# bioscan-ml/clibd

Hardware: AMD Instinct MI355X
Metric: paired samples/sec/step (I+D contrastive), global batch 2048 (higher is better)
Workload: dtype bf16

## Files before the change

clibd_amd/csrc/common.h:

```cpp
#pragma once
#include <hip/hip_runtime.h>
#include <stdint.h>

namespace clibd {

typedef __attribute__((ext_vector_type(8))) short bf16x8;
typedef __attribute__((ext_vector_type(4))) short bf16x4;
typedef __attribute__((ext_vector_type(4))) float f32x4;
typedef __attribute__((ext_vector_type(16))) float f32x16;
typedef __attribute__((address_space(3))) void lds_void;
typedef __attribute__((address_space(1))) const void gbl_cvoid;

__device__ __forceinline__ unsigned short f2bf(float x) {
    __bf16 h = (__bf16)x;
    return __builtin_bit_cast(unsigned short, h);
}
__device__ __forceinline__ float bf2f(unsigned short h) {
    return __builtin_bit_cast(float, ((unsigned)h) << 16);
}
__device__ __forceinline__ unsigned pack2bf(float lo, float hi) {
    typedef __bf16 bf16x2_t __attribute__((ext_vector_type(2)));
    typedef float f32x2_t __attribute__((ext_vector_type(2)));
    const bf16x2_t r = __builtin_convertvector((f32x2_t){lo, hi}, bf16x2_t);
    return __builtin_bit_cast(unsigned, r);
}
__device__ __forceinline__ float bfround(float x) { return bf2f(f2bf(x)); }

__device__ __forceinline__ unsigned pack4fp8(float a, float b, float c, float d) {
    a = __builtin_amdgcn_fmed3f(a, -448.f, 448.f); b = __builtin_amdgcn_fmed3f(b, -448.f, 448.f);
    c = __builtin_amdgcn_fmed3f(c, -448.f, 448.f); d = __builtin_amdgcn_fmed3f(d, -448.f, 448.f);
    int w = __builtin_amdgcn_cvt_pk_fp8_f32(a, b, 0, false);
    w = __builtin_amdgcn_cvt_pk_fp8_f32(c, d, w, true);
    return (unsigned)w;
}
__device__ __forceinline__ uint2 pack8fp8(const float v[8], float s) {
    uint2 o;
    o.x = pack4fp8(v[0] * s, v[1] * s, v[2] * s, v[3] * s);
    o.y = pack4fp8(v[4] * s, v[5] * s, v[6] * s, v[7] * s);
    return o;
}

__device__ __forceinline__ void glds16(const void* gsrc, void* lds_wave_base) {
    __builtin_amdgcn_global_load_lds((gbl_cvoid*)gsrc, (lds_void*)lds_wave_base, 16, 0, 0);
}

__device__ __forceinline__ void store16_stream(void* p, uint4 v) {
#ifdef CLIBD_NT_STORES
    typedef unsigned u32x4_t __attribute__((ext_vector_type(4)));
    __builtin_nontemporal_store((u32x4_t){v.x, v.y, v.z, v.w}, (u32x4_t*)p);
#else
    *(uint4*)p = v;
#endif
}

__device__ __forceinline__ unsigned drop_hash(unsigned seed, unsigned pair) {
    unsigned x = pair ^ seed;
    x ^= x >> 16; x *= 0x7feb352du; x ^= x >> 15; x *= 0x846ca68bu; x ^= x >> 16;
    return x;
}
__device__ __forceinline__ void drop_pair(unsigned seed, unsigned idx_even, unsigned thr16, float scale, float& f0, float& f1) {
    const unsigned h = drop_hash(seed, idx_even >> 1);
    f0 = (h & 0xffffu) >= thr16 ? scale : 0.f;
    f1 = (h >> 16) >= thr16 ? scale : 0.f;
}
__device__ __forceinline__ float drop_one(unsigned seed, unsigned idx, unsigned thr16, float scale) {
    const unsigned h = drop_hash(seed, idx >> 1);
    return (((idx & 1u) ? (h >> 16) : (h & 0xffffu)) >= thr16) ? scale : 0.f;
}

template <int CTRL>
__device__ __forceinline__ float dpp_mov(float v) {
    return __builtin_bit_cast(float, __builtin_amdgcn_update_dpp(0, __builtin_bit_cast(int, v), CTRL, 0xF, 0xF, false));
}
constexpr int DPP_QUAD_XOR1 = 0xB1, DPP_QUAD_XOR2 = 0x4E, DPP_ROW_HALF_MIRROR = 0x141, DPP_ROW_MIRROR = 0x140, DPP_ROW_ROR8 = 0x128;
__device__ __forceinline__ void permlane32_swap(float& a, float& b) {
    asm volatile("s_nop 1\n\tv_permlane32_swap_b32 %0, %1\n\ts_nop 1" : "+v"(a), "+v"(b));
}
__device__ __forceinline__ void permlane16_swap(float& a, float& b) {
    asm volatile("s_nop 1\n\tv_permlane16_swap_b32 %0, %1\n\ts_nop 1" : "+v"(a), "+v"(b));
}
__device__ __forceinline__ float rows4_sum(float v) {
    float a = v, b = v;
    permlane16_swap(a, b);
    v = a + b;
    a = v; b = v;
    permlane32_swap(a, b);
    return a + b;
}
__device__ __forceinline__ float rows4_max(float v) {
    float a = v, b = v;
    permlane16_swap(a, b);
    v = fmaxf(a, b);
    a = v; b = v;
    permlane32_swap(a, b);
    return fmaxf(a, b);
}
__device__ __forceinline__ float wave_sum(float v) {
    v += dpp_mov<DPP_QUAD_XOR1>(v);
    v += dpp_mov<DPP_QUAD_XOR2>(v);
    v += dpp_mov<DPP_ROW_HALF_MIRROR>(v);
    v += dpp_mov<DPP_ROW_MIRROR>(v);
    return rows4_sum(v);
}
__device__ __forceinline__ float wave_max(float v) {
    v = fmaxf(v, dpp_mov<DPP_QUAD_XOR1>(v));
    v = fmaxf(v, dpp_mov<DPP_QUAD_XOR2>(v));
    v = fmaxf(v, dpp_mov<DPP_ROW_HALF_MIRROR>(v));
    v = fmaxf(v, dpp_mov<DPP_ROW_MIRROR>(v));
    return rows4_max(v);
}

__device__ __forceinline__ float fast_erf(float x) {
    float ax = fabsf(x);
    float t = __builtin_amdgcn_rcpf(1.0f + 0.3275911f * ax);
    float y = ((((1.061405429f * t - 1.453152027f) * t + 1.421413741f) * t - 0.284496736f) * t + 0.254829592f) * t;
    float e = __expf(-ax * ax);
    float r = 1.0f - y * e;
    return copysignf(r, x);
}
__device__ __forceinline__ float gelu_f(float x) {
    return 0.5f * x * (1.0f + fast_erf(x * 0.70710678118654752f));
}
__device__ __forceinline__ void gelu_and_grad_f(float x, float& y, float& dy) {
    const float ax = fabsf(x) * 0.70710678118654752f;
    const float t = __builtin_amdgcn_rcpf(1.0f + 0.3275911f * ax);
    const float poly = ((((1.061405429f * t - 1.453152027f) * t + 1.421413741f) * t - 0.284496736f) * t + 0.254829592f) * t;
    const float e = __expf(-ax * ax);
    const float erfv = copysignf(1.0f - poly * e, x);
    const float cdf = 0.5f * (1.0f + erfv);
    y = x * cdf;
    dy = cdf + x * (0.3989422804014327f * e);
}
typedef float f32x2 __attribute__((ext_vector_type(2)));
__device__ __forceinline__ void gelu_and_grad_x2(f32x2 x, f32x2& y, f32x2& dy) {
    constexpr float K = 0.84932180028801907f;
    constexpr float P = 0.3275911f * 0.70710678118654752f / K;
    f32x2 ax = {fabsf(x[0]), fabsf(x[1])};
    ax = ax * K;
    const f32x2 d = ax * P + 1.0f;
    const f32x2 t = {__builtin_amdgcn_rcpf(d[0]), __builtin_amdgcn_rcpf(d[1])};
    const f32x2 poly = ((((0.5307027145f * t - 0.7265760135f) * t + 0.7107068705f) * t - 0.142248368f) * t + 0.127414796f) * t;
    const f32x2 s = ax * ax;
    const f32x2 e = {__builtin_amdgcn_exp2f(-s[0]), __builtin_amdgcn_exp2f(-s[1])};
    const f32x2 h = 0.5f - poly * e;
    const f32x2 hs = {copysignf(h[0], x[0]), copysignf(h[1], x[1])};
    const f32x2 cdf = hs + 0.5f;
    y = x * cdf;
    dy = (x * e) * 0.3989422804014327f + cdf;
}
__device__ __forceinline__ f32x2 bfround2(float a, float b) {
    const unsigned pk = pack2bf(a, b);
    return (f32x2){__builtin_bit_cast(float, pk << 16), __builtin_bit_cast(float, pk & 0xffff0000u)};
}
template <int N>
__device__ __forceinline__ void gelu_and_grad_rows(float* v, float* dg) {
#pragma unroll
    for (int e = 0; e < N; e += 2) {
        f32x2 y, d;
        gelu_and_grad_x2(bfround2(v[e], v[e + 1]), y, d);
        v[e] = y[0]; v[e + 1] = y[1];
        dg[e] = d[0]; dg[e + 1] = d[1];
    }
}
template <int N>
__device__ __forceinline__ void gelu_rows(float* v) {
#pragma unroll
    for (int e = 0; e < N; e += 2) {
        f32x2 y, d;
        gelu_and_grad_x2((f32x2){v[e], v[e + 1]}, y, d);
        v[e] = y[0]; v[e + 1] = y[1];
    }
}
constexpr float GELUQ_LO = -0.1328125f;
constexpr float GELUQ_STEP = 1.265625f / 255.0f;
constexpr float GELUQ_INV = 255.0f / 1.265625f;
__device__ __forceinline__ unsigned geluq_pack4(float a, float b, float c, float d) {
    unsigned w = 0;
    w = __builtin_amdgcn_cvt_pk_u8_f32(fmaf(a, GELUQ_INV, -GELUQ_LO * GELUQ_INV), 0, w);
    w = __builtin_amdgcn_cvt_pk_u8_f32(fmaf(b, GELUQ_INV, -GELUQ_LO * GELUQ_INV), 1, w);
    w = __builtin_amdgcn_cvt_pk_u8_f32(fmaf(c, GELUQ_INV, -GELUQ_LO * GELUQ_INV), 2, w);
    w = __builtin_amdgcn_cvt_pk_u8_f32(fmaf(d, GELUQ_INV, -GELUQ_LO * GELUQ_INV), 3, w);
    return w;
}
__device__ __forceinline__ void geluq_unpack4(unsigned w, float out[4]) {
    out[0] = fmaf((float)(w & 0xffu), GELUQ_STEP, GELUQ_LO);
    out[1] = fmaf((float)((w >> 8) & 0xffu), GELUQ_STEP, GELUQ_LO);
    out[2] = fmaf((float)((w >> 16) & 0xffu), GELUQ_STEP, GELUQ_LO);
    out[3] = fmaf((float)(w >> 24), GELUQ_STEP, GELUQ_LO);
}

__device__ __forceinline__ unsigned gelu12_code_bits(unsigned b) {
    const unsigned t = b & 0x7fffu;
    unsigned u = t >= (113u << 7) ? t - (112u << 7) : 0u;
    u = u > 0x7ffu ? 0x7ffu : u;
    return ((b >> 4) & 0x800u) | u;
}
__device__ __forceinline__ float gelu12_val(unsigned c) {
    const unsigned u = c & 0x7ffu;
    const unsigned t = u ? u + (112u << 7) : 0u;
    return __uint_as_float((((c & 0x800u) << 4) | t) << 16);
}
struct __attribute__((packed, aligned(4))) gelu12_row8 { unsigned w0, w1, w2; };
__device__ __forceinline__ gelu12_row8 gelu12_pack8(const float* g) {
    unsigned c[8];
#pragma unroll
    for (int e = 0; e < 8; e += 2) {
        const unsigned pk = pack2bf(g[e], g[e + 1]);
        c[e] = gelu12_code_bits(pk & 0xffffu);
        c[e + 1] = gelu12_code_bits(pk >> 16);
    }
    gelu12_row8 r;
    r.w0 = c[0] | (c[1] << 12) | (c[2] << 24);
    r.w1 = (c[2] >> 8) | (c[3] << 4) | (c[4] << 16) | (c[5] << 28);
    r.w2 = (c[5] >> 4) | (c[6] << 8) | (c[7] << 20);
    return r;
}
__device__ __forceinline__ void gelu12_unpack8(unsigned w0, unsigned w1, unsigned w2, float* g) {
    g[0] = gelu12_val(w0 & 0xfffu);
    g[1] = gelu12_val((w0 >> 12) & 0xfffu);
    g[2] = gelu12_val((w0 >> 24) | ((w1 & 0xfu) << 8));
// ... 15 lines not shown
```

clibd_amd/csrc/gemm.hip:

```cpp
#include <stdlib.h>

#include <cmath>

#include "gemm_common.h"
#include "host_util.h"

namespace clibd {

constexpr int BM = 128, BN = 128, BK = 64;
constexpr int TILE_BYTES = BM * BK * 2;
constexpr int GEMM_THREADS = 256;

__device__ __forceinline__ int w_row_perm(int r) {
    const int r6 = r & 63;
    return (r & 64) + w_col_of(r6 >> 4, r6 & 15);
}

__global__ __launch_bounds__(GEMM_THREADS, 2) void gemm_bf16_nt_kernel(GemmParams p) {
    extern __shared__ __attribute__((aligned(16))) char smem[];
    const int tid = threadIdx.x;
    const int lane = tid & 63;
    const int wave = __builtin_amdgcn_readfirstlane(tid >> 6);
    const int wm = wave >> 1, wn = wave & 1;

    const int ntiles = p.tiles_m * p.tiles_n;
    int bid = blockIdx.x;
    const int split = bid / ntiles;
    bid -= split * ntiles;
    int tile_m, tile_n;
    tile_coords(bid, p.tiles_m, p.tiles_n, 8, tile_m, tile_n);
    const int m0 = tile_m * BM, n0 = tile_n * BN;

    const int kt0 = split * p.ktiles_per_split;
    const int nk = min(p.ktiles_per_split, p.K / BK - p.hole_nkt - kt0);

    const int prow = lane >> 3;
    const int chunk = (lane & 7) ^ prow;
    const char* a_src[4];
    const char* w_src[4];
#pragma unroll
    for (int j = 0; j < 4; ++j) {
        const int r = (wave * 4 + j) * 8 + prow;
        const int gm = min(m0 + r, p.M - 1);
        const int gn = min(n0 + w_row_perm(r), p.N - 1);
        a_src[j] = (const char*)(p.A + (size_t)gm * p.lda) + chunk * 16;
        w_src[j] = (const char*)(p.W + (size_t)gn * p.ldw) + chunk * 16;
    }

    f32x4 acc[4][4];
#pragma unroll
    for (int i = 0; i < 4; ++i)
#pragma unroll
        for (int j = 0; j < 4; ++j) acc[i][j] = (f32x4){0.f, 0.f, 0.f, 0.f};

    const int frow = lane & 15, fch = lane >> 4;
    int a_off[4], w_off[4];
#pragma unroll
    for (int t = 0; t < 4; ++t) {
        const int ra = wm * 64 + t * 16 + frow;
        const int rw = wn * 64 + t * 16 + frow;
        a_off[t] = ra * 128 + ((fch ^ (ra & 7)) << 4);
        w_off[t] = rw * 128 + ((fch ^ (rw & 7)) << 4);
    }

    auto stage = [&](int kt, int buf) {
        char* base = smem + buf * (2 * TILE_BYTES);
        int kta = kt0 + kt;
        if (kta >= p.hole_kt) kta += p.hole_nkt;
        const size_t koff = (size_t)kta * (BK * 2);
#pragma unroll
        for (int j = 0; j < 4; ++j) {
            glds16(a_src[j] + koff, base + (wave * 4 + j) * 1024);
            glds16(w_src[j] + koff, base + TILE_BYTES + (wave * 4 + j) * 1024);
        }
    };

    if (nk > 0) stage(0, 0);
    for (int kt = 0; kt < nk; ++kt) {
        __syncthreads();
        if (kt + 1 < nk) stage(kt + 1, (kt + 1) & 1);
        const char* ab = smem + (kt & 1) * (2 * TILE_BYTES);
        const char* wb = ab + TILE_BYTES;
#pragma unroll
        for (int kk = 0; kk < 2; ++kk) {
            bf16x8 af[4], wf[4];
#pragma unroll
            for (int t = 0; t < 4; ++t) {
                af[t] = *(const bf16x8*)(ab + (a_off[t] ^ (kk << 6)));
                wf[t] = *(const bf16x8*)(wb + (w_off[t] ^ (kk << 6)));
            }
#pragma unroll
            for (int i = 0; i < 4; ++i)
#pragma unroll
                for (int j = 0; j < 4; ++j)
                    acc[i][j] = __builtin_amdgcn_mfma_f32_16x16x32_bf16(wf[j], af[i], acc[i][j], 0, 0, 0);
        }
    }

    const clibd_gemm_epilogue& ep = p.ep;
    if (ep.rank_u != nullptr && split == 0) {
        bf16x8 uf[4], vf[4];
#pragma unroll
        for (int t = 0; t < 4; ++t) {
            uf[t] = (bf16x8){0, 0, 0, 0, 0, 0, 0, 0};
            vf[t] = (bf16x8){0, 0, 0, 0, 0, 0, 0, 0};
            if (fch == 0) {
                const int gm = min(m0 + wm * 64 + t * 16 + frow, p.M - 1);
                const int gn = min(n0 + w_row_perm(wn * 64 + t * 16 + frow), p.N - 1);
                uf[t] = *(const bf16x8*)((const unsigned short*)ep.rank_u + (size_t)gm * ep.ld_rank_u);
                vf[t] = *(const bf16x8*)((const unsigned short*)ep.rank_v + (size_t)gn * 8);
            }
        }
#pragma unroll
        for (int i = 0; i < 4; ++i)
#pragma unroll
            for (int j = 0; j < 4; ++j)
                acc[i][j] = __builtin_amdgcn_mfma_f32_16x16x32_bf16(vf[j], uf[i], acc[i][j], 0, 0, 0);
    }

    const int nb = n0 + wn * 64 + 16 * fch;
    if (nb >= p.N) return;
    float bias[16];
    load_bias16(ep, nb, split == 0, bias);
#pragma unroll
    for (int i = 0; i < 4; ++i) {
        const int m = m0 + wm * 64 + 16 * i + frow;
        if (m >= p.M) continue;
        float v[16];
#pragma unroll
        for (int j = 0; j < 4; ++j)
#pragma unroll
            for (int r = 0; r < 4; ++r) v[4 * j + r] = acc[i][j][r] + bias[4 * j + r];
        store_row16(ep, m, nb, v);
    }
}

__global__ __launch_bounds__(256) void transpose_bf16_kernel(const unsigned short* in, int ld_in, int R, int C,
                                                             unsigned short* out, int ld_out) {
    __shared__ unsigned short tile[64][66];
    const int r0 = blockIdx.y * 64, c0 = blockIdx.x * 64;
    const int tx = threadIdx.x & 63, ty = threadIdx.x >> 6;
    for (int i = ty; i < 64; i += 4) {
        const int r = r0 + i, c = c0 + tx;
        tile[i][tx] = (r < R && c < C) ? in[(size_t)r * ld_in + c] : (unsigned short)0;
    }
    __syncthreads();
    for (int i = ty; i < 64; i += 4) {
        const int c = c0 + i, r = r0 + tx;
        if (c < C && r < ld_out) out[(size_t)c * ld_out + r] = tile[tx][i];
    }
}

__global__ __launch_bounds__(256) void transpose_fp8_bf16_kernel(const unsigned char* __restrict__ in, int ld_in, int R, int C, float scale,
                                                                 unsigned short* __restrict__ out, int ld_out) {
    __shared__ unsigned short tile[64][66];
    const int r0 = blockIdx.y * 64, c0 = blockIdx.x * 64;
    const int tx = threadIdx.x & 63, ty = threadIdx.x >> 6;
    for (int i = ty; i < 64; i += 4) {
        const int r = r0 + i, c = c0 + tx;
        unsigned short v = 0;
        if (r < R && c < C) v = f2bf(__builtin_amdgcn_cvt_f32_fp8((int)in[(size_t)r * ld_in + c], 0) * scale);
        tile[i][tx] = v;
    }
    __syncthreads();
    for (int i = ty; i < 64; i += 4) {
        const int c = c0 + i, r = r0 + tx;
        if (c < C && r < ld_out) out[(size_t)c * ld_out + r] = tile[tx][i];
    }
}

template <int RB>
__global__ __launch_bounds__(256) void transpose_colsum_bf16_kernel(const unsigned short* __restrict__ in, int ld_in, int R, int C,
                                                                    unsigned short* __restrict__ out, int ld_out,
                                                                    float* __restrict__ colsum, float* __restrict__ partials) {
    __shared__ __attribute__((aligned(16))) unsigned short tile[64 * RB * 66];
    const int r0 = blockIdx.y * (64 * RB), c0 = blockIdx.x * 64;
    const int t = threadIdx.x;
    uint4 v[2 * RB];
#pragma unroll
    for (int k = 0; k < 2 * RB; ++k) {
        const int row = (t >> 3) + 32 * k, ch = t & 7;
        v[k] = make_uint4(0u, 0u, 0u, 0u);
        if (r0 + row < R && c0 + 8 * ch < C) v[k] = *(const uint4*)(in + (size_t)(r0 + row) * ld_in + c0 + 8 * ch);
    }
#pragma unroll
    for (int k = 0; k < 2 * RB; ++k) {
        const int row = (t >> 3) + 32 * k, ch = t & 7;
        unsigned* d = (unsigned*)(tile + row * 66 + 8 * ch);
        d[0] = v[k].x; d[1] = v[k].y; d[2] = v[k].z; d[3] = v[k].w;
    }
    __syncthreads();
#pragma unroll
    for (int k = 0; k < 2; ++k) {
        const int c = (t >> 3) + 32 * k, rch = t & 7;
        float sum = 0.f;
#pragma unroll
        for (int rb = 0; rb < RB; ++rb) {
            unsigned short e[8];
#pragma unroll
            for (int j = 0; j < 8; ++j) e[j] = tile[(64 * rb + 8 * rch + j) * 66 + c];
            if (c0 + c < C && r0 + 64 * rb + 8 * rch < ld_out) {
                uint4 o;
                o.x = (unsigned)e[0] | ((unsigned)e[1] << 16); o.y = (unsigned)e[2] | ((unsigned)e[3] << 16);
                o.z = (unsigned)e[4] | ((unsigned)e[5] << 16); o.w = (unsigned)e[6] | ((unsigned)e[7] << 16);
                *(uint4*)(out + (size_t)(c0 + c) * ld_out + r0 + 64 * rb + 8 * rch) = o;
            }
            if (colsum != nullptr) {
#pragma unroll
                for (int j = 0; j < 8; ++j) sum += bf2f(e[j]);
            }
        }
        if (colsum != nullptr) {
            sum += dpp_mov<DPP_QUAD_XOR1>(sum);
            sum += dpp_mov<DPP_QUAD_XOR2>(sum);
            sum += dpp_mov<DPP_ROW_HALF_MIRROR>(sum);
            if (rch == 0 && c0 + c < C) {
                if (partials != nullptr) partials[(size_t)blockIdx.y * C + c0 + c] = sum;
                else atomicAdd(colsum + c0 + c, sum);
            }
        }
    }
}

__global__ __launch_bounds__(256) void colsum_partials_kernel(const float* __restrict__ partials, int nblk, int C, float* __restrict__ colsum) {
    const int c = blockIdx.x * 256 + threadIdx.x;
    if (c >= C) return;
    float s0 = 0.f, s1 = 0.f, s2 = 0.f, s3 = 0.f;
    int b = 0;
    for (; b + 3 < nblk; b += 4) {
        s0 += partials[(size_t)b * C + c];
        s1 += partials[(size_t)(b + 1) * C + c];
        s2 += partials[(size_t)(b + 2) * C + c];
        s3 += partials[(size_t)(b + 3) * C + c];
    }
    for (; b < nblk; ++b) s0 += partials[(size_t)b * C + c];
    colsum[c] += (s0 + s1) + (s2 + s3);
}

__global__ __launch_bounds__(1024) void ordered_colsum_kernel(const float* __restrict__ partials, int nblk, int C, float* __restrict__ out, int split,
                                                              float* __restrict__ out_b) {
    __shared__ float part[16][64];
    const int lane = threadIdx.x & 63, w = threadIdx.x >> 6, G = blockDim.x >> 6;
    const int c = blockIdx.x * 64 + lane;
    const int per = (nblk + G - 1) / G;
    const int b1 = min((w + 1) * per, nblk);
    float s = 0.f;
    if (c < C) {
        int b = w * per;
        for (; b + 8 <= b1; b += 8) {
            float v[8];
#pragma unroll
            for (int k = 0; k < 8; ++k) v[k] = partials[(size_t)(b + k) * C + c];
#pragma unroll
            for (int k = 0; k < 8; ++k) s += v[k];
        }
        for (; b < b1; ++b) s += partials[(size_t)b * C + c];
    }
    part[w][lane] = s;
    __syncthreads();
    if (w == 0 && c < C) {
        float t = part[0][lane];
        for (int k = 1; k < G; ++k) t += part[k][lane];
        if (c < split) out[c] += t;
        else out_b[c - split] += t;
    }
}

int ordered_colsum_launch(const float* partials, int nblk, int C, float* out, int split, float* out_b, hipStream_t stream) {
    if (nblk <= 0 || C <= 0) return CLIBD_OK;
    const int G = nblk < 16 ? nblk : 16;
    hipLaunchKernelGGL(ordered_colsum_kernel, dim3((unsigned)((C + 63) / 64)), dim3(64 * G), 0, stream, partials, nblk, C, out, split, out_b);
    return check_launch("ordered_colsum");
}

__global__ __launch_bounds__(256) void cast_f32_bf16_kernel(const float* in, unsigned short* out, size_t n) {
    size_t i = ((size_t)blockIdx.x * blockDim.x + threadIdx.x) * 4;
    const size_t stride = (size_t)gridDim.x * blockDim.x * 4;
    for (; i + 3 < n; i += stride) {
        const f32x4 v = *(const f32x4*)(in + i);
        uint2 o;
        o.x = pack2bf(v[0], v[1]);
        o.y = pack2bf(v[2], v[3]);
        *(uint2*)(out + i) = o;
    }
    if (blockIdx.x == 0 && threadIdx.x == 0)
        for (size_t j = n & ~(size_t)3; j < n; ++j) out[j] = f2bf(in[j]);
}

__global__ __launch_bounds__(256) void cast_transpose_f32_bf16_kernel(const float* in, int R, int C,
                                                                      unsigned short* out) {
    __shared__ float tile[64][65];
    const int r0 = blockIdx.y * 64, c0 = blockIdx.x * 64;
    const int tx = threadIdx.x & 63, ty = threadIdx.x >> 6;
    for (int i = ty; i < 64; i += 4) {
        const int r = r0 + i, c = c0 + tx;
        tile[i][tx] = (r < R && c < C) ? in[(size_t)r * C + c] : 0.f;
    }
    __syncthreads();
    for (int i = ty; i < 64; i += 4) {
        const int c = c0 + i, r = r0 + tx;
        if (c < C && r < R) out[(size_t)c * R + r] = f2bf(tile[tx][i]);
    }
}

}

using namespace clibd;

static int gemm_impl(const void* A, int lda, const void* W, int ldw, int M, int N, int K, int hole_k0, int hole_len,
                     const clibd_gemm_epilogue* ep, void* stream, void* tail_ws = nullptr, size_t tail_ws_bytes = 0) {
    if (!A || !W || !ep) return set_error(CLIBD_EINVAL, "gemm: null pointer");
    if (hole_len < 0 || hole_k0 < 0 || hole_k0 % BK || hole_len % BK || hole_k0 + hole_len > K || (hole_len > 0 && hole_len >= K))
        return set_error(CLIBD_EINVAL, "gemm: bad K hole (multiples of 64 inside [0, K))");
    if (M <= 0 || N <= 0 || K <= 0) return set_error(CLIBD_EINVAL, "gemm: non-positive shape");
    if (K % BK != 0) return set_error(CLIBD_EINVAL, "gemm: K must be a multiple of 64");
    if (N % 16 != 0) return set_error(CLIBD_EINVAL, "gemm: N must be a multiple of 16");
    if (lda % 8 != 0 || ldw % 8 != 0 || lda < K || ldw < K) return set_error(CLIBD_EINVAL, "gemm: bad lda/ldw");
    if (!aligned16(A) || !aligned16(W)) return set_error(CLIBD_EINVAL, "gemm: operands must be 16-byte aligned");
    if (!ep->out_bf16 && !ep->out_f32 && !ep->out_pre_bf16) return set_error(CLIBD_EINVAL, "gemm: no output");
    if ((ep->rank_u == nullptr) != (ep->rank_v == nullptr)) return set_error(CLIBD_EINVAL, "gemm: rank_u/rank_v");
    if (ep->rank_u && (ep->ld_rank_u < 8 || ep->ld_rank_u % 8)) return set_error(CLIBD_EINVAL, "gemm: ld_rank_u");
    if ((ep->act == CLIBD_ACT_GELU_GRAD || ep->act == CLIBD_ACT_MUL_AUX || ep->act == CLIBD_ACT_ADD_AUX) &&
        (!ep->aux_bf16 || ep->ld_aux % 8 || ep->ld_aux < N))
        return set_error(CLIBD_EINVAL, "gemm: GELU_GRAD / MUL_AUX / ADD_AUX need aux_bf16 with ld_aux >= N, % 8");
    if (ep->act == CLIBD_ACT_MUL_AUX_U8 && (!ep->aux_bf16 || ep->ld_aux % 16 || ep->ld_aux < N))
        return set_error(CLIBD_EINVAL, "gemm: MUL_AUX_U8 needs aux (one byte per element) with ld_aux >= N, % 16");
    const bool e12 = ep->act == CLIBD_ACT_GELU_SAVE_GRAD_E12 || ep->act == CLIBD_ACT_MUL_AUX_E12;
    if (e12 && (N % 8 != 0)) return set_error(CLIBD_EINVAL, "gemm: the e4m7 gelu' forms need N % 8 == 0");
    if (ep->act == CLIBD_ACT_MUL_AUX_E12 && (!ep->aux_bf16 || ep->ld_aux % 4 || ep->ld_aux < 3 * (N / 2)))
        return set_error(CLIBD_EINVAL, "gemm: MUL_AUX_E12 needs aux (1.5 bytes per element) with ld_aux >= 3N/2 bytes, % 4");
    if (ep->act == CLIBD_ACT_GELU_SAVE_GRAD_E12 && (!ep->out_pre_bf16 || ep->ld_pre % 4 || ep->ld_pre < 3 * (N / 2)))
        return set_error(CLIBD_EINVAL, "gemm: GELU_SAVE_GRAD_E12 needs out_pre (1.5 bytes per element) with ld_pre >= 3N/2 bytes, % 4");
    if ((ep->act == CLIBD_ACT_GELU_SAVE_GRAD || ep->act == CLIBD_ACT_GELU_SAVE_GRAD_U8) && !ep->out_pre_bf16)
        return set_error(CLIBD_EINVAL, "gemm: GELU_SAVE_GRAD needs out_pre_bf16");
    if (ep->act < 0 || ep->act > CLIBD_ACT_MUL_AUX_E12) return set_error(CLIBD_EINVAL, "gemm: bad act");
    if (ep->residual_f32 && (ep->ld_res % 4 || ep->ld_res < N)) return set_error(CLIBD_EINVAL, "gemm: ld_res");
    if (ep->out_pre_bf16 && (ep->ld_pre % (ep->act == CLIBD_ACT_GELU_SAVE_GRAD_U8 ? 16 : 8) || ep->ld_pre < N)) return set_error(CLIBD_EINVAL, "gemm: ld_pre");
    if (ep->out_bf16 && (ep->ld_out_bf16 % 8 || ep->ld_out_bf16 < N)) return set_error(CLIBD_EINVAL, "gemm: ld_out_bf16");
    if (ep->out_f32 && (ep->ld_out_f32 % 4 || ep->ld_out_f32 < N)) return set_error(CLIBD_EINVAL, "gemm: ld_out_f32");
    if (ep->drop_thr16 < 0 || ep->drop_thr16 > 65535 || (ep->drop_thr16 > 0 && (ep->drop_ld < N || (ep->drop_ld & 1) || ep->split_k > 1)))
        return set_error(CLIBD_EINVAL, "gemm: bad dropout parameters");
    const int split = ep->split_k < 1 ? 1 : ep->split_k;
    if (split > 1 && (ep->out_bf16 || ep->out_pre_bf16 || ep->act != CLIBD_ACT_NONE || ep->residual_f32 || !ep->out_f32))
        return set_error(CLIBD_EINVAL, "gemm: split_k > 1 supports only a plain fp32 accumulate output");
    const void* ptrs[] = {ep->bias, ep->rank_u, ep->rank_v, ep->aux_bf16, ep->residual_f32, ep->out_pre_bf16,
                          ep->out_bf16, ep->out_f32};
    for (const void* q : ptrs)
        if (q && !aligned16(q)) return set_error(CLIBD_EINVAL, "gemm: epilogue pointers must be 16-byte aligned");

    GemmParams p{};
    p.A = (const unsigned short*)A; p.W = (const unsigned short*)W;
    p.M = M; p.N = N; p.K = K; p.lda = lda; p.ldw = ldw;
    p.tiles_m = (M + BM - 1) / BM;
    p.tiles_n = (N + BN - 1) / BN;
    const int ktiles = (K - hole_len) / BK;
    p.ktiles_per_split = (ktiles + split - 1) / split;
    p.ep = *ep;
    p.ep.split_k = split;
    p.splits = 1; p.nk_split = 0; p.split_stride = 0;
    p.hole_kt = hole_len > 0 ? hole_k0 / BK : 0x7fffffff;
    p.hole_nkt = hole_len / BK;
    if (tail_ws != nullptr) {
        const size_t need = gemm256_tail_workspace_bytes(M, N, K);
        if (need > 0) {
            if (tail_ws_bytes < need || !aligned16(tail_ws)) return set_error(CLIBD_EINVAL, "gemm: tail workspace too small or misaligned (clibd_gemm_tail_workspace_bytes)");
            p.sk_flags = (unsigned*)tail_ws;
            p.sk_ws = (float*)((char*)tail_ws + 1024);
        }
    }
    static const int forced = [] { const char* e = getenv("CLIBD_GEMM_KERNEL"); return e ? atoi(e) : 0; }();
    const bool fold_epi = ep->row_sums != nullptr || ep->row_stats != nullptr;
    if (fold_epi) {
        if (epilogue_kind(p.ep) < 0)
            return set_error(CLIBD_EINVAL, "gemm: LN-fold epilogue: row_sums needs bias + residual_f32 + out_f32 + out_bf16 (act NONE); row_stats needs "
                                           "col_sum_w + bias + GELU_SAVE_GRAD with out_pre_bf16 + out_bf16; no rank update, dropout or split-K");
        if ((ep->row_sums && !aligned16(ep->row_sums)) || (ep->row_stats && !aligned16(ep->row_stats)) || (ep->col_sum_w && !aligned16(ep->col_sum_w)))
            return set_error(CLIBD_EINVAL, "gemm: LN-fold epilogue pointers must be 16-byte aligned");
        if (forced == 1 || hole_len != 0 || !gemm256_try_launch(p, (hipStream_t)stream))
            return set_error(CLIBD_EINVAL, "gemm: the LN-fold epilogues exist in the 256x256 kernel only (M >= 1024, N % 256 == 0, K % 128 == 0, >= 128 tiles)");
        return check_launch("gemm256_bf16_nt");
    }
    if (forced != 1 && hole_len == 0 && gemm256_try_launch(p, (hipStream_t)stream)) return check_launch("gemm256_bf16_nt");
    const long long nblocks = (long long)p.tiles_m * p.tiles_n * split;
    if (nblocks > 0x7fffffffLL) return set_error(CLIBD_EINVAL, "gemm: grid too large");
    static const bool attr_ok = [] {
        return hipFuncSetAttribute((const void*)gemm_bf16_nt_kernel, hipFuncAttributeMaxDynamicSharedMemorySize,
                                   4 * TILE_BYTES) == hipSuccess;
    }();
    (void)attr_ok;
    hipLaunchKernelGGL(gemm_bf16_nt_kernel, dim3((unsigned)nblocks), dim3(GEMM_THREADS), 4 * TILE_BYTES,
                       (hipStream_t)stream, p);
    return check_launch("gemm_bf16_nt");
}

extern "C" int clibd_gemm_bf16_nt(const void* A, int lda, const void* W, int ldw, int M, int N, int K,
                                  const clibd_gemm_epilogue* ep, void* stream) {
    return gemm_impl(A, lda, W, ldw, M, N, K, 0, 0, ep, stream);
}

extern "C" size_t clibd_gemm_tail_workspace_bytes(int M, int N, int K) { return gemm256_tail_workspace_bytes(M, N, K); }

extern "C" int clibd_gemm_bf16_nt_ws(const void* A, int lda, const void* W, int ldw, int M, int N, int K,
                                     const clibd_gemm_epilogue* ep, void* workspace, size_t workspace_bytes, void* stream) {
    return gemm_impl(A, lda, W, ldw, M, N, K, 0, 0, ep, stream, workspace, workspace_bytes);
}

extern "C" int clibd_gemm_bf16_nt_khole(const void* A, int lda, const void* W, int ldw, int M, int N, int K, int hole_k0, int hole_len,
                                        const clibd_gemm_epilogue* ep, void* stream) {
    return gemm_impl(A, lda, W, ldw, M, N, K, hole_k0, hole_len, ep, stream);
}

extern "C" int clibd_gemm_fp8_nt(const void* A, int lda, const void* W, int ldw, int M, int N, int K, const float* col_scale,
                                 float out_fp8_scale, const clibd_gemm_epilogue* ep, void* stream) {
    if (!A || !W || !ep || !col_scale) return set_error(CLIBD_EINVAL, "gemm_fp8: null pointer");
    if (M <= 0 || N <= 0 || K <= 0 || lda < K || ldw < K) return set_error(CLIBD_EINVAL, "gemm_fp8: bad shape");
    if ((lda & 15) || (ldw & 15) || !aligned16(A) || !aligned16(W) || !aligned16(col_scale)) return set_error(CLIBD_EINVAL, "gemm_fp8: alignment (lda, ldw % 16)");
    if (ep->ld_out_bf16 & 7 || ep->ld_out_f32 & 3 || ep->ld_res & 3 || ep->ld_pre & 7 || ep->ld_rank_u & 7)
        return set_error(CLIBD_EINVAL, "gemm_fp8: leading dimensions");
    if ((ep->out_bf16 && !aligned16(ep->out_bf16)) || (ep->out_f32 && !aligned16(ep->out_f32)) || (ep->out_pre_bf16 && !aligned16(ep->out_pre_bf16)) ||
        (ep->residual_f32 && !aligned16(ep->residual_f32)) || (ep->rank_u && !aligned16(ep->rank_u)) || (ep->rank_v && !aligned16(ep->rank_v)) ||
        (ep->bias && !aligned16(ep->bias)))
        return set_error(CLIBD_EINVAL, "gemm_fp8: pointer alignment");
    if ((ep->rank_u == nullptr) != (ep->rank_v == nullptr)) return set_error(CLIBD_EINVAL, "gemm_fp8: rank_u / rank_v must come together");
    GemmParams p{};
    p.A = (const unsigned short*)A; p.W = (const unsigned short*)W;
    p.M = M; p.N = N; p.K = K; p.lda = lda; p.ldw = ldw;
    p.ep = *ep;
    if (p.ep.split_k < 1) p.ep.split_k = 1;
    p.fp8 = 1; p.col_scale = col_scale; p.out_fp8_scale = out_fp8_scale;
    if (!gemm256_fp8_launch(p, (hipStream_t)stream))
        return set_error(CLIBD_EINVAL, "gemm_fp8: shape / epilogue not supported (N % 256, K % 256, K >= 512, bias required; forms: "
                                       "[lora] bias->bf16 | bias->gelu->fp8 + gelu' | bias[->dropout]+residual->f32)");
    return check_launch("gemm256_fp8_nt");
}

extern "C" int clibd_gemm_fp8_dgrad_nt(const void* A, int lda, const void* W, int ldw, int M, int N, int K, const float* col_scale,
                                       const float* a_row_dequant, float out_fp8_scale, const clibd_gemm_epilogue* ep, void* stream) {
    if (!A || !W || !ep || !col_scale) return set_error(CLIBD_EINVAL, "gemm_fp8_dgrad: null pointer");
    if (M <= 0 || N <= 0 || K <= 0 || lda < K || ldw < K) return set_error(CLIBD_EINVAL, "gemm_fp8_dgrad: bad shape");
    if ((lda & 15) || (ldw & 15) || !aligned16(A) || !aligned16(W) || !aligned16(col_scale) || (a_row_dequant && !aligned16(a_row_dequant)))
        return set_error(CLIBD_EINVAL, "gemm_fp8_dgrad: alignment (lda, ldw % 16)");
    if (ep->ld_out_bf16 & 7 || ep->ld_aux & 7) return set_error(CLIBD_EINVAL, "gemm_fp8_dgrad: leading dimensions");
    if (ep->act == CLIBD_ACT_MUL_AUX_U8 && (!ep->aux_bf16 || ep->ld_aux % 16 || ep->ld_aux < N))
        return set_error(CLIBD_EINVAL, "gemm_fp8_dgrad: MUL_AUX_U8 needs aux (one byte per element) with ld_aux >= N, % 16");
    if (!ep->out_bf16 || !aligned16(ep->out_bf16) || (ep->aux_bf16 && !aligned16(ep->aux_bf16))) return set_error(CLIBD_EINVAL, "gemm_fp8_dgrad: out_bf16 / aux alignment");
    if (ep->out_f32 || ep->residual_f32 || ep->bias || ep->rank_u || ep->rank_v || ep->row_sums || ep->row_stats || ep->col_sum_w)
        return set_error(CLIBD_EINVAL, "gemm_fp8_dgrad: only out_bf16 [+ aux_bf16] epilogues");
    const bool mul_form = ep->act == CLIBD_ACT_MUL_AUX || ep->act == CLIBD_ACT_MUL_AUX_U8 || ep->act == CLIBD_ACT_MUL_AUX_E12;
    if (ep->act == CLIBD_ACT_MUL_AUX_E12 && (!ep->aux_bf16 || ep->ld_aux % 4 || ep->ld_aux < 3 * (N / 2)))
        return set_error(CLIBD_EINVAL, "gemm_fp8_dgrad: MUL_AUX_E12 needs aux (1.5 bytes per element) with ld_aux >= 3N/2 bytes, % 4");
    if (ep->out_pre_bf16 && (!mul_form || !a_row_dequant || !aligned16(ep->out_pre_bf16) || (ep->ld_pre & 7) || ep->ld_pre < N))
        return set_error(CLIBD_EINVAL, "gemm_fp8_dgrad: out_pre_bf16 (bf16 copy) comes with MUL_AUX[_U8] and a_row_dequant only; ld_pre >= N, % 8; 16-byte aligned");
    GemmParams p{};
    p.A = (const unsigned short*)A; p.W = (const unsigned short*)W;
    p.M = M; p.N = N; p.K = K; p.lda = lda; p.ldw = ldw;
    p.ep = *ep;
    if (p.ep.split_k < 1) p.ep.split_k = 1;
    p.fp8 = 1; p.col_scale = col_scale; p.out_fp8_scale = out_fp8_scale; p.a_row_dequant = a_row_dequant;
    p.dual_bf16 = (unsigned short*)p.ep.out_pre_bf16; p.ld_dual = p.ep.ld_pre;
    p.ep.out_pre_bf16 = nullptr; p.ep.ld_pre = 0;
    if (!gemm256_fp8_dgrad_launch(p, (hipStream_t)stream))
        return set_error(CLIBD_EINVAL, "gemm_fp8_dgrad: shape / epilogue not supported (M % 4, N % 256, K % 256, K >= 512; forms: -> bf16 | + aux_bf16 -> bf16 "
                                       "(both need a_row_dequant) | x aux (bf16 gelu' or its one-byte code) -> fp8 (needs out_fp8_scale > 0))");
    return check_launch("gemm256_fp8_dgrad_nt");
}

namespace clibd {
__global__ __launch_bounds__(256) void reduce_splits_kernel(const float* __restrict__ partials, int splits, size_t n4,
                                                            float* __restrict__ out, int accumulate) {
    for (size_t i = (size_t)blockIdx.x * blockDim.x + threadIdx.x; i < n4; i += (size_t)gridDim.x * blockDim.x) {
        f32x4 s = accumulate ? ((const f32x4*)out)[i] : (f32x4){0.f, 0.f, 0.f, 0.f};
        for (int k = 0; k < splits; ++k) s += ((const f32x4*)partials)[(size_t)k * n4 + i];
        ((f32x4*)out)[i] = s;
    }
}
}

extern "C" size_t clibd_gemm_splitk_workspace_bytes(int M, int N) {
    if (M <= 0 || N <= 0) return 0;
    return (size_t)256 * (size_t)M * (size_t)N * sizeof(float) / (size_t)(((M + 255) / 256) * ((N + 255) / 256));
}

extern "C" int clibd_gemm_bf16_nt_splitk(const void* A, int lda, const void* W, int ldw, int M, int N, int K, float* out_f32, int ld_out,
                                         int accumulate, void* workspace, size_t workspace_bytes, void* stream) {
    if (!A || !W || !out_f32 || !workspace) return set_error(CLIBD_EINVAL, "gemm_splitk: null pointer");
    if (M <= 0 || N <= 0 || K <= 0 || lda < K || ldw < K || ld_out != N) return set_error(CLIBD_EINVAL, "gemm_splitk: bad shape (out must be dense [M,N])");
    if ((lda & 7) || (ldw & 7) || !aligned16(A) || !aligned16(W) || !aligned16(out_f32) || !aligned16(workspace) || (N & 3))
        return set_error(CLIBD_EINVAL, "gemm_splitk: alignment");
    GemmParams p{};
    p.A = (const unsigned short*)A; p.W = (const unsigned short*)W;
    p.M = M; p.N = N; p.K = K; p.lda = lda; p.ldw = ldw;
    const int splits = gemm256_splitk_launch(p, (float*)workspace, workspace_bytes / sizeof(float), (hipStream_t)stream);
    if (splits <= 0) return set_error(CLIBD_EINVAL, "gemm_splitk: shape not supported (need N % 256 == 0, K % 128 == 0, K >= 512, workspace)");
    if (int e = check_launch("gemm256_splitk")) return e;
    const size_t n4 = (size_t)M * N / 4;
    size_t blocks = (n4 + 255) / 256;
    if (blocks > 8192) blocks = 8192;
    hipLaunchKernelGGL(reduce_splits_kernel, dim3((unsigned)blocks), dim3(256), 0, (hipStream_t)stream, (const float*)workspace, splits, n4,
                       out_f32, accumulate);
    return check_launch("reduce_splits");
}

extern "C" int clibd_gemm_bf16_tn_splitk(const void* A, int lda, const void* B, int ldb, int M, int Na, int Nb, float* out_f32, int ld_out,
                                         int accumulate, float* colsum_a, void* workspace, size_t workspace_bytes, void* stream) {
    if (!A || !B || !out_f32 || !workspace) return set_error(CLIBD_EINVAL, "gemm_tn_splitk: null pointer");
    if (M <= 0 || Na <= 0 || Nb <= 0 || lda < Na || ldb < Nb || ld_out != Nb) return set_error(CLIBD_EINVAL, "gemm_tn_splitk: bad shape (out must be dense [Na,Nb])");
    if ((lda & 7) || (ldb & 7) || !aligned16(A) || !aligned16(B) || !aligned16(out_f32) || !aligned16(workspace))
        return set_error(CLIBD_EINVAL, "gemm_tn_splitk: alignment");
    const int splits = gemm256_tn_splitk_launch((const unsigned short*)A, lda, (const unsigned short*)B, ldb, M, Na, Nb, (float*)workspace,
                                                workspace_bytes / sizeof(float), colsum_a, (hipStream_t)stream);
    if (splits <= 0) return set_error(CLIBD_EINVAL, "gemm_tn_splitk: shape not supported (need M % 128 == 0, M >= 256, Na % 256 == 0, Nb % 256 == 0, workspace)");
    if (int e = check_launch("gemm256_tn")) return e;
    const size_t n4 = (size_t)Na * Nb / 4;
    size_t blocks = (n4 + 255) / 256;
    if (blocks > 8192) blocks = 8192;
    hipLaunchKernelGGL(reduce_splits_kernel, dim3((unsigned)blocks), dim3(256), 0, (hipStream_t)stream, (const float*)workspace, splits, n4,
                       out_f32, accumulate);
    return check_launch("reduce_splits");
}

extern "C" size_t clibd_gemm_tn_colsum_workspace_bytes(int M, int Na) {
    if (M <= 0 || Na <= 0) return 0;
    const int slots = M / 256 > 1 ? M / 256 : 1;
    return (size_t)slots * (size_t)Na * sizeof(float);
// ... 147 lines not shown
```

clibd_amd/csrc/gemm256.hip:

```cpp
#include <cstdlib>
#include "gemm_common.h"
#include "host_util.h"

namespace clibd {

constexpr int T_M = 256, T_N = 256, T_K = 64;
constexpr int HALF_BYTES = 128 * T_K * 2;
constexpr int STAGE_BYTES = 4 * HALF_BYTES;
constexpr int G256_THREADS = 512;
constexpr int G256_LDS = 2 * STAGE_BYTES;
constexpr size_t G256_SK_FLAG_BYTES = 1024;
#ifndef CLIBD_WS_MIN_TILES_N
#define CLIBD_WS_MIN_TILES_N 1
#endif
#ifndef CLIBD_WS_GROUP
#define CLIBD_WS_GROUP 6
#endif
constexpr int G256_WS_MIN_TILES_N = CLIBD_WS_MIN_TILES_N, G256_WS_GROUP = CLIBD_WS_GROUP;

#define CLIBD_WAIT_VMCNT(n) asm volatile("s_waitcnt vmcnt(" #n ")" ::: "memory")

typedef int i32x8 __attribute__((ext_vector_type(8)));
typedef int i32x4 __attribute__((ext_vector_type(4)));
__device__ __forceinline__ i32x8 cat_frag(bf16x8 lo, bf16x8 hi) {
// ... 198 lines not shown
    } while (0)
#define PHASE_HEAD(Q8)       \
    do {                                                                                                     \
        constexpr int st_ = ((Q8) >> 2) & 1;                                                                 \
        constexpr int dl_ = (Q8) & 3;                                                                        \
        if (dl_ == 0) { LOAD_W(w0F, st_, 1); LOAD_A(st_, 0); }                                               \
        else if (dl_ == 1) { LOAD_W(w1F, st_, 2); }                                                          \
        else if (dl_ == 2) { LOAD_A(st_, 3); }                                                               \
        if ((Q8) >= 2) {       \
            constexpr int ju_ = ((Q8) + 2) & 3;                                                              \
            constexpr int du_ = ((Q8) + 6) >> 2;                                                             \
            ISSUE(du_, ju_, du_ & 1);                                                                        \
        }                                                                                                    \
        WAIT_HEAD();                                                                                         \
        BARRIER();                                                                                           \
        if (dl_ == 0) { WAIT_FRAGS_W(w0F); WAIT_FRAGS_A(); }                                                 \
        else if (dl_ == 1) { WAIT_FRAGS_W(w1F); }                                                            \
        else if (dl_ == 2) { WAIT_FRAGS_A(); }                                                               \
        if (dl_ == 0) MMA(0, 0, w0F);                                                                        \
        else if (dl_ == 1) MMA(0, 1, w1F);                                                                   \
        else if (dl_ == 2) MMA(1, 1, w1F);                                                                   \
        else MMA(1, 0, w0F);                                                                                 \
        BARRIER();                                                                                           \
    } while (0)
#define PROLOGUE_ISSUE()                                                     \
    do {                                                                     \
         \
        ISSUE(0, 0, 0); __builtin_amdgcn_sched_barrier(0);                   \
        ISSUE(0, 1, 0); __builtin_amdgcn_sched_barrier(0);                   \
        ISSUE(0, 2, 0); __builtin_amdgcn_sched_barrier(0);                   \
        ISSUE(0, 3, 0); __builtin_amdgcn_sched_barrier(0);                   \
        ISSUE(1, 0, 1); __builtin_amdgcn_sched_barrier(0);                   \
        ISSUE(1, 1, 1); __builtin_amdgcn_sched_barrier(0);                   \
        ISSUE(1, 2, 1); __builtin_amdgcn_sched_barrier(0);                   \
        ISSUE(1, 3, 1); __builtin_amdgcn_sched_barrier(0);                   \
    } while (0)

    if (DIAG && skew_ticks > 0) {
        const int cls = (blockIdx.x >> 3) & 3;
        const unsigned long long t0 = __builtin_amdgcn_s_memrealtime();
        while ((long long)(__builtin_amdgcn_s_memrealtime() - t0) < (long long)cls * skew_ticks) __builtin_amdgcn_s_sleep(8);
    }
    set_sources(tile);
    PROLOGUE_ISSUE();
    int allow_case = 0;
    const clibd_gemm_epilogue& ep = p.ep;
    const int stores_case = (ep.out_pre_bf16 ? 1 : 0) + (ep.out_bf16 ? 1 : 0) + (ep.out_f32 ? 2 : 0) + (DG == 2 ? 1 : 0);

    int tile_i = 0;
#define STAMP(k)                                                                                         \
    do {                                                                                                 \
        if (DIAG && stamps != nullptr && tile_i < 16 && (wave == 0 || wave == 4) && lane == 0)                    \
            stamps[(((size_t)blockIdx.x * 16 + tile_i) * 2 + (wave >> 2)) * 8 + (k)] = (long long)__builtin_amdgcn_s_memtime(); \
    } while (0)

    while (true) {
        m0 = nm0;
        n0 = nn0;
        const int nk = nk_issue;
        const int split_cur = split_issue;
        const int part_cur = part_issue, slot_cur = slot_issue;
        const int next = tile + (int)gridDim.x;
        const bool has_next = next < ntiles;
        WAIT_HEAD();
        BARRIER();
        if (wm == 1) BARRIER();
        STAMP(0);
#pragma unroll
        for (int a = 0; a < 2; ++a)
#pragma unroll
            for (int b = 0; b < 4; ++b)
#pragma unroll
                for (int c = 0; c < 2; ++c)
#pragma unroll
                    for (int d = 0; d < 2; ++d) acc[a][b][c][d] = (f32x4){0.f, 0.f, 0.f, 0.f};

        int kt = 0;
        PHASE_HEAD(0); PHASE_HEAD(1); PHASE_HEAD(2); PHASE_HEAD(3);
        STAMP(1);
        PHASE_HEAD(4); PHASE_HEAD(5);
        PHASE(6, true, 8); PHASE(7, true, 8);
        STAMP(2);
        for (kt = 2; kt < nk - 2; kt += 2) {
            PHASE(0, true, 8); PHASE(1, true, 8); PHASE(2, true, 8); PHASE(3, true, 8);
            PHASE(4, true, 8); PHASE(5, true, 8); PHASE(6, true, 8); PHASE(7, true, 8);
        }
        STAMP(3);
        PHASE(0, true, 8); PHASE(1, true, 8);
        if (has_next) set_sources(next);
        PHASE_TAIL(2, 6); PHASE_TAIL(3, 4); PHASE_TAIL(4, 2); PHASE_TAIL(5, 0); PHASE_TAIL(6, 0); PHASE_TAIL(7, 0);
        if (wm == 0) BARRIER();
        if constexpr (FP8) {
#pragma unroll
            for (int hm = 0; hm < 2; ++hm)
                asm volatile("s_nop 15\n\ts_nop 15"
                             : "+v"(acc[hm][0][0][0]), "+v"(acc[hm][0][0][1]), "+v"(acc[hm][0][1][0]), "+v"(acc[hm][0][1][1]),
                               "+v"(acc[hm][1][0][0]), "+v"(acc[hm][1][0][1]), "+v"(acc[hm][1][1][0]), "+v"(acc[hm][1][1][1]),
                               "+v"(acc[hm][2][0][0]), "+v"(acc[hm][2][0][1]), "+v"(acc[hm][2][1][0]), "+v"(acc[hm][2][1][1]),
                               "+v"(acc[hm][3][0][0]), "+v"(acc[hm][3][0][1]), "+v"(acc[hm][3][1][0]), "+v"(acc[hm][3][1][1])
                             :: "memory");
        }
        STAMP(4);
        if constexpr (SK) {
            if (slot_cur >= 0) {
                const int srow = 64 * wn + 4 * fch, scol = 128 * wm + 8 * frow;
                if (part_cur > 0) {
                    float* outp = p.sk_ws + ((size_t)(part_cur - 1) * (size_t)p.sk_tail + (size_t)slot_cur) * (size_t)(T_M * T_N);
#pragma unroll
                    for (int hn = 0; hn < 2; ++hn)
#pragma unroll
                        for (int n = 0; n < 2; ++n)
#pragma unroll
                            for (int r = 0; r < 4; ++r) {
                                float* o = outp + (size_t)(srow + 32 * hn + 16 * n + r) * T_N + scol;
                                const f32x4 v0 = (f32x4){acc[0][0][hn][n][r], acc[0][1][hn][n][r], acc[0][2][hn][n][r], acc[0][3][hn][n][r]};
                                const f32x4 v1 = (f32x4){acc[1][0][hn][n][r], acc[1][1][hn][n][r], acc[1][2][hn][n][r], acc[1][3][hn][n][r]};
                                asm volatile("global_store_dwordx4 %0, %1, off sc0 sc1\n\tglobal_store_dwordx4 %0, %2, off offset:16 sc0 sc1" :: "v"(o), "v"(v0), "v"(v1) : "memory");
                            }
                    asm volatile("s_waitcnt vmcnt(0)" ::: "memory");
                    BARRIER();
                    if (tid == 0) __hip_atomic_fetch_add(p.sk_flags + slot_cur, 1u, __ATOMIC_RELAXED, __HIP_MEMORY_SCOPE_AGENT);
                    break;
                }
                if (tid == 0) {
                    while (__hip_atomic_load(p.sk_flags + slot_cur, __ATOMIC_RELAXED, __HIP_MEMORY_SCOPE_AGENT) < (unsigned)(p.sk_parts - 1)) __builtin_amdgcn_s_sleep(16);
                    __hip_atomic_store(p.sk_flags + slot_cur, 0u, __ATOMIC_RELAXED, __HIP_MEMORY_SCOPE_AGENT);
                }
                BARRIER();
                for (int q = 1; q < p.sk_parts; ++q) {
                    const float* inp = p.sk_ws + ((size_t)(q - 1) * (size_t)p.sk_tail + (size_t)slot_cur) * (size_t)(T_M * T_N);
#pragma unroll
                    for (int hn = 0; hn < 2; ++hn)
#pragma unroll
                        for (int n = 0; n < 2; ++n) {
                            f32x4 t0[4], t1[4];
#pragma unroll
                            for (int r = 0; r < 4; ++r) {
                                const float* o = inp + (size_t)(srow + 32 * hn + 16 * n + r) * T_N + scol;
                                asm volatile("global_load_dwordx4 %0, %2, off sc0 sc1\n\tglobal_load_dwordx4 %1, %2, off offset:16 sc0 sc1" : "=&v"(t0[r]), "=&v"(t1[r]) : "v"(o) : "memory");
                            }
                            asm volatile("s_waitcnt vmcnt(0)" : "+v"(t0[0]), "+v"(t0[1]), "+v"(t0[2]), "+v"(t0[3]), "+v"(t1[0]), "+v"(t1[1]), "+v"(t1[2]), "+v"(t1[3]));
#pragma unroll
                            for (int r = 0; r < 4; ++r)
#pragma unroll
                                for (int t = 0; t < 4; ++t) { acc[0][t][hn][n][r] += t0[r][t]; acc[1][t][hn][n][r] += t1[r][t]; }
                        }
                }
            }
        }
        int erow = frow, egrp = fch;
        asm volatile("" : "+v"(erow), "+v"(egrp));
        int nb = n0 + 128 * wm + 8 * erow;
        int mb = m0 + 64 * wn + 4 * egrp;
        constexpr bool RES_KIND = (KIND == EPI_RES_F32 || KIND == EPI_RES_F32_DROP || KIND == EPI_RES_F32_COPY);
        constexpr bool TWO_PASS = (epi_aux_kind(KIND) || RES_KIND || KIND == EPI_ROWNORM_GELU);
        constexpr bool PRELOAD_ROWS = TWO_PASS && !LORA && !FP8;
        f32x4 bias_q[2];
        uint4 in_aux[8];
        f32x4 in_res[8][2];
        float2 in_st[8];
        f32x4 col_s[2];
#define GLOAD128(dst, ptr) asm volatile("global_load_dwordx4 %0, %1, off ; EPI_OPERAND_LOAD" : "=&v"(dst) : "v"(ptr) : "memory")
        constexpr bool BIAS_ASM = BIAS && !FP8;
        if constexpr (BIAS_ASM) {
            const float* bp = ep.bias + nb;
            GLOAD128(bias_q[0], bp);
            GLOAD128(bias_q[1], bp + 4);
        }
        if constexpr (PRELOAD_ROWS) {
#pragma unroll
            for (int n = 0; n < 2; ++n)
#pragma unroll
                for (int r = 0; r < 4; ++r) {
                    const int mc = min(mb + 16 * n + r, p.M - 1);
                    if constexpr (KIND == EPI_ROWNORM_GELU) {
                        in_st[4 * n + r] = *(const float2*)(ep.row_stats + (size_t)mc * 2);
                    } else if constexpr (KIND == EPI_MUL_AUX_U8) {
                        const uint2 c8 = *(const uint2*)((const unsigned char*)ep.aux_bf16 + (size_t)mc * ep.ld_aux + nb);
                        in_aux[4 * n + r] = make_uint4(c8.x, c8.y, 0u, 0u);
                    } else if constexpr (KIND == EPI_MUL_AUX_12) {
                        in_aux[4 * n + r] = load_aux12((const unsigned char*)ep.aux_bf16 + (size_t)mc * ep.ld_aux + (nb >> 1) * 3);
                    } else if constexpr (epi_aux_kind(KIND)) {
                        in_aux[4 * n + r] = load_aux16<epi_aux_nt(KIND)>((const unsigned short*)ep.aux_bf16 + (size_t)mc * ep.ld_aux + nb);
                    } else {
                        const f32x4* rs = (const f32x4*)(ep.residual_f32 + (size_t)mc * ep.ld_res + nb);
                        in_res[4 * n + r][0] = rs[0];
                        in_res[4 * n + r][1] = rs[1];
                    }
                }
        }
        if constexpr (KIND == EPI_ROWNORM_GELU) {
            col_s[0] = *(const f32x4*)(ep.col_sum_w + nb);
            col_s[1] = *(const f32x4*)(ep.col_sum_w + nb + 4);
        }
        if (has_next) {
            ISSUE(1, 2, 1); __builtin_amdgcn_sched_barrier(0);
            ISSUE(1, 3, 1); __builtin_amdgcn_sched_barrier(0);
        }
        erow = frow; egrp = fch;
        asm volatile("" : "+v"(erow), "+v"(egrp));
        nb = n0 + 128 * wm + 8 * erow;
        mb = m0 + 64 * wn + 4 * egrp;
#define EPI_TIED_WAIT(N)                                                                                             \
    do {                                                                                                             \
        if constexpr (BIAS_ASM) asm volatile("s_waitcnt vmcnt(" #N ") ; EPI_OPERAND_WAIT" : "+v"(bias_q[0]), "+v"(bias_q[1])); \
    } while (0)
        if constexpr (KIND == EPI_ROWNORM_GELU) {
            if (!has_next) asm volatile("s_waitcnt vmcnt(10)" ::: "memory");
            EPI_TIED_WAIT(14);
        } else if constexpr (PRELOAD_ROWS && epi_aux_kind(KIND)) {
            if (!has_next) asm volatile("s_waitcnt vmcnt(8)" ::: "memory");
            EPI_TIED_WAIT(12);
        } else if constexpr (PRELOAD_ROWS) {
            if (!has_next) asm volatile("s_waitcnt vmcnt(16)" ::: "memory");
            EPI_TIED_WAIT(20);
        } else {
            if (!has_next) asm volatile("s_waitcnt vmcnt(0)" ::: "memory");
            EPI_TIED_WAIT(4);
        }
#undef EPI_TIED_WAIT
#undef GLOAD128
        unsigned rdexp[2][2];
        if constexpr (FP8) {
            const float* csp = p.col_scale + n0 + 128 * wm + 8 * erow;
            const f32x4 c0 = *(const f32x4*)csp, c1 = *(const f32x4*)(csp + 4);
#pragma unroll
            for (int hm = 0; hm < 2; ++hm)
#pragma unroll
                for (int t = 0; t < 4; ++t) {
                    const float c = hm ? c1[t] : c0[t];
#pragma unroll
                    for (int q = 0; q < 4; ++q) acc[hm][t][q >> 1][q & 1] *= c;
                }
            if constexpr (DG == 2) {
#pragma unroll
                for (int hn = 0; hn < 2; ++hn)
#pragma unroll
                    for (int n = 0; n < 2; ++n) {
                        const f32x4 rd = *(const f32x4*)(p.a_row_dequant + min(mb + 32 * hn + 16 * n, p.M - 4));
                        rdexp[hn][n] = ((__float_as_uint(rd[0]) >> 23) & 0xffu) | (((__float_as_uint(rd[1]) >> 23) & 0xffu) << 8) |
                                       (((__float_as_uint(rd[2]) >> 23) & 0xffu) << 16) | (((__float_as_uint(rd[3]) >> 23) & 0xffu) << 24);
                    }
            }
            if constexpr (DG && !epi_mul_aux_kind(KIND)) {
#pragma unroll
                for (int hn = 0; hn < 2; ++hn)
#pragma unroll
                    for (int n = 0; n < 2; ++n) {
                        const f32x4 rd = *(const f32x4*)(p.a_row_dequant + min(mb + 32 * hn + 16 * n, p.M - 4));
#pragma unroll
                        for (int hm = 0; hm < 2; ++hm)
#pragma unroll
                            for (int t = 0; t < 4; ++t) acc[hm][t][hn][n] *= rd;
                    }
            }
        }
        if (LORA) {
            bf16x8 uf[2][2];
#pragma unroll
            for (int hn = 0; hn < 2; ++hn)
#pragma unroll
                for (int n = 0; n < 2; ++n) {
                    uf[hn][n] = (bf16x8){0, 0, 0, 0, 0, 0, 0, 0};
                    if (egrp == 0) {
                        const int gm = min(m0 + 64 * wn + 32 * hn + 16 * n + erow, p.M - 1);
                        uf[hn][n] = *(const bf16x8*)((const unsigned short*)ep.rank_u + (size_t)gm * ep.ld_rank_u);
                    }
                }
#pragma unroll
            for (int hm = 0; hm < 2; ++hm)
#pragma unroll
                for (int t = 0; t < 4; ++t) {
                    bf16x8 vf = (bf16x8){0, 0, 0, 0, 0, 0, 0, 0};
                    if (egrp == 0) {
                        const int gn = nb + 4 * hm + t;
                        vf = *(const bf16x8*)((const unsigned short*)ep.rank_v + (size_t)gn * 8);
                    }
#pragma unroll
                    for (int n = 0; n < 4; ++n)
                        acc[hm][t][n >> 1][n & 1] = __builtin_amdgcn_mfma_f32_16x16x32_bf16(uf[n >> 1][n & 1], vf, acc[hm][t][n >> 1][n & 1], 0, 0, 0);
                }
            __builtin_amdgcn_sched_barrier(0);
        }

        {
            float bias[8];
            if constexpr (BIAS_ASM) {
#pragma unroll
                for (int e = 0; e < 4; ++e) { bias[e] = bias_q[0][e]; bias[4 + e] = bias_q[1][e]; }
            } else if constexpr (BIAS) {
                load_bias8(ep, nb, bias);
                if constexpr (!TWO_PASS) {
#pragma unroll
                    for (int e = 0; e < 8; ++e) asm volatile("" : "+v"(bias[e]));
                }
            }
#define EPV(hm, t) (BIAS ? acc[hm][t][hn][n][r] + bias[4 * (hm) + (t)] : acc[hm][t][hn][n][r])
#define FOR_ROWS_HN(HN0, HN1, ...)                                                                           \
    _Pragma("unroll") for (int hn = (HN0); hn < (HN1); ++hn)                                                 \
        _Pragma("unroll") for (int n = 0; n < 2; ++n)                                                        \
            _Pragma("unroll") for (int r = 0; r < 4; ++r) {                                                  \
                const int m = mb + 32 * hn + 16 * n + r;                                                     \
                __VA_ARGS__                                                                                  \
            }
#define FOR_ROWS(...) FOR_ROWS_HN(0, 2, __VA_ARGS__)
#define PIN_GROUP(hn_)                                                                                       \
    _Pragma("unroll") for (int hm = 0; hm < 2; ++hm)                                                         \
        _Pragma("unroll") for (int t = 0; t < 4; ++t)                                                        \
            _Pragma("unroll") for (int n2 = 0; n2 < 2; ++n2) asm volatile("" : "+v"(acc[hm][t][hn_][n2]))
            if (KIND == EPI_SPLITK_F32) {
                float* outp = ep.out_f32 + (size_t)split_cur * (size_t)p.split_stride;
                FOR_ROWS({
                    if (m < p.M) {
                        f32x4* o = (f32x4*)(outp + (size_t)m * ep.ld_out_f32 + nb);
                        o[0] = (f32x4){acc[0][0][hn][n][r], acc[0][1][hn][n][r], acc[0][2][hn][n][r], acc[0][3][hn][n][r]};
                        o[1] = (f32x4){acc[1][0][hn][n][r], acc[1][1][hn][n][r], acc[1][2][hn][n][r], acc[1][3][hn][n][r]};
                    }
                })
            } else if (TWO_PASS) {
                float cs8[8];
                if constexpr (KIND == EPI_ROWNORM_GELU) {
                    _Pragma("unroll") for (int e = 0; e < 4; ++e) { cs8[e] = col_s[0][e]; cs8[4 + e] = col_s[1][e]; }
                }
                FOR_ROWS_HN(0, 1, {
                    const int mc = min(m, p.M - 1);
                    float v[8];
                    _Pragma("unroll") for (int hm = 0; hm < 2; ++hm)
                        _Pragma("unroll") for (int t = 0; t < 4; ++t) v[4 * hm + t] = (KIND == EPI_ROWNORM_GELU) ? acc[hm][t][hn][n][r] : EPV(hm, t);
                    if constexpr (KIND == EPI_ROWNORM_GELU) fold_rownorm8(v, in_st[4 * n + r].x, in_st[4 * n + r].y, cs8, bias);
                    else if constexpr (PRELOAD_ROWS) fold_row8_in<KIND>(ep, mc, nb, v, in_aux[4 * n + r], in_res[4 * n + r][0], in_res[4 * n + r][1]);
                    else fold_row8<KIND>(ep, mc, nb, v);
                    _Pragma("unroll") for (int hm = 0; hm < 2; ++hm)
                        _Pragma("unroll") for (int t = 0; t < 4; ++t) acc[hm][t][hn][n][r] = v[4 * hm + t];
                })
                PIN_GROUP(0);
                FOR_ROWS_HN(1, 2, {
                    const int mc = min(m, p.M - 1);
                    float v[8];
                    _Pragma("unroll") for (int hm = 0; hm < 2; ++hm)
                        _Pragma("unroll") for (int t = 0; t < 4; ++t) v[4 * hm + t] = (KIND == EPI_ROWNORM_GELU) ? acc[hm][t][hn][n][r] : EPV(hm, t);
                    if constexpr (KIND == EPI_ROWNORM_GELU) {
                        const float2 st = *(const float2*)(ep.row_stats + (size_t)mc * 2);
                        fold_rownorm8(v, st.x, st.y, cs8, bias);
                    } else {
                        fold_row8<KIND>(ep, mc, nb, v);
                    }
                    _Pragma("unroll") for (int hm = 0; hm < 2; ++hm)
                        _Pragma("unroll") for (int t = 0; t < 4; ++t) acc[hm][t][hn][n][r] = v[4 * hm + t];
                })
                PIN_GROUP(1);
                float keep1 = 0.f, keep2 = 0.f;
                FOR_ROWS({
                    if (m < p.M) {
                        float v[8];
                        _Pragma("unroll") for (int hm = 0; hm < 2; ++hm)
                            _Pragma("unroll") for (int t = 0; t < 4; ++t) v[4 * hm + t] = acc[hm][t][hn][n][r];
                        if (KIND == EPI_ROWNORM_GELU) {
                            store_row8<EPI_GELU_SAVE>(ep, m, nb, v);
                        } else if (DG && epi_mul_aux_kind(KIND)) {
                            *(uint2*)((unsigned char*)ep.out_bf16 + (size_t)m * ep.ld_out_bf16 + nb) = pack8fp8(v, p.out_fp8_scale);
                            if constexpr (DG == 2) {
                                const float rdf = __uint_as_float(((rdexp[hn][n] >> (8 * r)) & 0xffu) << 23);
                                float w8[8];
                                _Pragma("unroll") for (int e = 0; e < 8; ++e) w8[e] = v[e] * rdf;
                                *(uint4*)(p.dual_bf16 + (size_t)m * p.ld_dual + nb) = pack8bf(w8);
                            }
                        } else if (epi_aux_kind(KIND)) {
                            *(uint4*)((unsigned short*)ep.out_bf16 + (size_t)m * ep.ld_out_bf16 + nb) = pack8bf(v);
                        } else {
                            f32x4* o = (f32x4*)(ep.out_f32 + (size_t)m * ep.ld_out_f32 + nb);
                            o[0] = (f32x4){v[0], v[1], v[2], v[3]};
                            o[1] = (f32x4){v[4], v[5], v[6], v[7]};
                            if constexpr (KIND == EPI_RES_F32_COPY) {
                                *(uint4*)((unsigned short*)ep.out_bf16 + (size_t)m * ep.ld_out_bf16 + nb) = pack8bf(v);
                                float s1 = ((v[0] + v[1]) + (v[2] + v[3])) + ((v[4] + v[5]) + (v[6] + v[7]));
                                float s2 = 0.f;
                                _Pragma("unroll") for (int e = 0; e < 8; ++e) s2 = fmaf(v[e], v[e], s2);
                                s1 = row16_sum(s1);
                                s2 = row16_sum(s2);
                                if (erow == 8 * hn + 4 * n + r) { keep1 = s1; keep2 = s2; }
                            }
                        }
                    }
                })
                if constexpr (KIND == EPI_RES_F32_COPY) {
                    const int jm = mb + 32 * (erow >> 3) + 16 * ((erow >> 2) & 1) + (erow & 3);
                    const int slice = (n0 >> 7) + wm;
                    if (jm < p.M) *(float2*)(ep.row_sums + ((size_t)slice * (size_t)p.M + (size_t)jm) * 2) = make_float2(keep1, keep2);
                }
            } else {
                FOR_ROWS({
                    if (m < p.M) {
                        float v[8];
                        _Pragma("unroll") for (int hm = 0; hm < 2; ++hm)
                            _Pragma("unroll") for (int t = 0; t < 4; ++t) v[4 * hm + t] = EPV(hm, t);
                        if (FP8 && KIND == EPI_GELU_SAVE) store_row8_gelu_fp8(ep, m, nb, v, p.out_fp8_scale);
                        else store_row8<KIND>(ep, m, nb, v);
                    }
                })
            }
#undef PIN_GROUP
#undef FOR_ROWS_HN
#undef FOR_ROWS
#undef EPV
        }
        STAMP(5);
        if (DIAG) ++tile_i;
        if (!has_next) break;
        allow_case = (m0 + T_M <= p.M) ? stores_case : 0;
        tile = next;
    }
}

template <int KIND, bool LORA, bool BIAS, bool DIAG, bool FP8>
__global__ __launch_bounds__(G256_THREADS) void gemm256_bf16_nt_kernel(GemmParams p, int ntiles, int skew_ticks, long long* stamps) {
    gemm256_body<KIND, LORA, BIAS, DIAG, FP8, 0>(p, ntiles, skew_ticks, stamps);
}
template <int KIND, bool LORA, bool BIAS>
__global__ __launch_bounds__(G256_THREADS) void gemm256_bf16_nt_sk_kernel(GemmParams p, int ntiles, int skew_ticks, long long* stamps) {
    gemm256_body<KIND, LORA, BIAS, false, false, 0, true>(p, ntiles, skew_ticks, stamps);
}
static const void* kernel_ptr_sk(int kind, bool lora, bool bias) {
    switch (kind) {
        case EPI_BF16: return bias ? nullptr : lora ? (const void*)gemm256_bf16_nt_sk_kernel<EPI_BF16, true, false> : (const void*)gemm256_bf16_nt_sk_kernel<EPI_BF16, false, false>;
        case EPI_ADD_AUX: return bias ? nullptr : lora ? (const void*)gemm256_bf16_nt_sk_kernel<EPI_ADD_AUX, true, false> : (const void*)gemm256_bf16_nt_sk_kernel<EPI_ADD_AUX, false, false>;
        case EPI_RES_F32: return (bias && !lora) ? (const void*)gemm256_bf16_nt_sk_kernel<EPI_RES_F32, false, true> : nullptr;
        case EPI_RES_F32_DROP: return (bias && !lora) ? (const void*)gemm256_bf16_nt_sk_kernel<EPI_RES_F32_DROP, false, true> : nullptr;
        default: return nullptr;
    }
}
template <int KIND, int DG = 1>
__global__ __launch_bounds__(G256_THREADS) void gemm256_fp8_dgrad_kernel(GemmParams p, int ntiles, int skew_ticks, long long* stamps) {
    gemm256_body<KIND, false, false, false, true, DG>(p, ntiles, skew_ticks, stamps);
}

#ifdef CLIBD_GEMM_DIAG
static long long* g_stamp_buffer = nullptr;
static int skew_env_value() {
    static const int v = [] { const char* e = getenv("CLIBD_GEMM_SKEW"); return e ? atoi(e) : 0; }();
    return v;
}
static int band_env_value() {
    static const int v = [] { const char* e = getenv("CLIBD_GEMM_BAND"); return e ? atoi(e) : 0; }();
    return v;
}
#define CLIBD_DIAG_KERNEL(KIND) (const void*)gemm256_bf16_nt_kernel<KIND, false, true, true, false>
#else
static constexpr long long* g_stamp_buffer = nullptr;
static int skew_env_value() { return 0; }
static int band_env_value() { return 0; }
#define CLIBD_DIAG_KERNEL(KIND) (const void*)nullptr
#endif

static const void* kernel_ptr(int kind, bool lora, bool bias, bool diag) {
#define K256(KIND)                                                                                                    \
    (diag ? CLIBD_DIAG_KERNEL(KIND)                                                                                   \
          : lora ? (bias ? (const void*)gemm256_bf16_nt_kernel<KIND, true, true, false, false>                        \
                         : (const void*)gemm256_bf16_nt_kernel<KIND, true, false, false, false>)                      \
                 : (bias ? (const void*)gemm256_bf16_nt_kernel<KIND, false, true, false, false>                       \
                         : (const void*)gemm256_bf16_nt_kernel<KIND, false, false, false, false>))
    switch (kind) {
        case EPI_BF16: return K256(EPI_BF16);
        case EPI_GELU_SAVE: return K256(EPI_GELU_SAVE);
        case EPI_GELU: return K256(EPI_GELU);
        case EPI_F32: return K256(EPI_F32);
        case EPI_MUL_AUX: return K256(EPI_MUL_AUX);
        case EPI_ADD_AUX: return K256(EPI_ADD_AUX);
        case EPI_GELU_SAVE_U8: return K256(EPI_GELU_SAVE_U8);
        case EPI_MUL_AUX_U8: return K256(EPI_MUL_AUX_U8);
        case EPI_GELU_SAVE_12: return K256(EPI_GELU_SAVE_12);
        case EPI_MUL_AUX_12: return K256(EPI_MUL_AUX_12);
        case EPI_RES_F32: return K256(EPI_RES_F32);
        case EPI_RES_F32_DROP: return K256(EPI_RES_F32_DROP);
        case EPI_SPLITK_F32: return (const void*)gemm256_bf16_nt_kernel<EPI_SPLITK_F32, false, false, false, false>;
        case EPI_RES_F32_COPY: return (lora || !bias || diag) ? nullptr : (const void*)gemm256_bf16_nt_kernel<EPI_RES_F32_COPY, false, true, false, false>;
        case EPI_ROWNORM_GELU: return (lora || !bias || diag) ? nullptr : (const void*)gemm256_bf16_nt_kernel<EPI_ROWNORM_GELU, false, true, false, false>;
        default: return K256(EPI_GENERIC);
    }
#undef K256
}

static const void* kernel_ptr_fp8(int kind, bool lora) {
    switch (kind) {
        case EPI_BF16: return lora ? (const void*)gemm256_bf16_nt_kernel<EPI_BF16, true, true, false, true>
                                   : (const void*)gemm256_bf16_nt_kernel<EPI_BF16, false, true, false, true>;
        case EPI_GELU_SAVE: return lora ? nullptr : (const void*)gemm256_bf16_nt_kernel<EPI_GELU_SAVE, false, true, false, true>;
        case EPI_RES_F32: return lora ? nullptr : (const void*)gemm256_bf16_nt_kernel<EPI_RES_F32, false, true, false, true>;
        case EPI_RES_F32_DROP: return lora ? nullptr : (const void*)gemm256_bf16_nt_kernel<EPI_RES_F32_DROP, false, true, false, true>;
        default: return nullptr;
    }
}

static int device_cus() {
    static const int num_cus = [] {
        int dev = 0, n = 256;
        if (hipGetDevice(&dev) == hipSuccess) {
            hipDeviceProp_t prop;
            if (hipGetDeviceProperties(&prop, dev) == hipSuccess && prop.multiProcessorCount > 0) n = prop.multiProcessorCount;
        }
        return n;
    }();
    return num_cus;
}

bool gemm256_fp8_launch(const GemmParams& p, hipStream_t stream) {
    const int nk = p.K / 128;
    if (!p.fp8 || p.col_scale == nullptr || p.K % 128 != 0 || nk < 4 || (nk & 1) || p.N % T_N != 0 || p.M < 1 || p.ep.split_k > 1) return false;
    if (p.ep.bias == nullptr) return false;
    if ((unsigned long long)p.M * p.lda >= (1ull << 32) || (unsigned long long)p.N * p.ldw >= (1ull << 32)) return false;
    const int kind = epilogue_kind(p.ep);
    const bool lora = p.ep.rank_u != nullptr;
    const void* fn = kernel_ptr_fp8(kind, lora);
    if (fn == nullptr) return false;
    if ((p.out_fp8_scale > 0.f) != (kind == EPI_GELU_SAVE)) return false;
    static const bool attr_ok = [] {
        bool ok = true;
        for (int k = 0; k < EPI_NUM_KINDS; ++k)
            for (int l = 0; l < 2; ++l) {
                const void* f = kernel_ptr_fp8(k, l != 0);
                if (f != nullptr) ok = ok && hipFuncSetAttribute(f, hipFuncAttributeMaxDynamicSharedMemorySize, G256_LDS) == hipSuccess;
            }
        return ok;
    }();
    if (!attr_ok) return false;
    GemmParams q = p;
    q.tiles_m = (p.M + T_M - 1) / T_M;
    q.tiles_n = p.N / T_N;
    q.splits = 1;
    q.nk_split = nk;
    q.split_stride = 0;
    q.band = q.tiles_n >= G256_WS_MIN_TILES_N ? -G256_WS_GROUP : 4;
    const long long tiles = (long long)q.tiles_m * q.tiles_n;
    const int grid = (int)(tiles < device_cus() ? tiles : device_cus());
    int ntiles_i = (int)tiles, skew = 0;
    long long* stamp = nullptr;
    void* args[] = {(void*)&q, (void*)&ntiles_i, (void*)&skew, (void*)&stamp};
    return hipLaunchKernel(fn, dim3((unsigned)grid), dim3(G256_THREADS), args, G256_LDS, stream) == hipSuccess;
}

bool gemm256_fp8_dgrad_launch(const GemmParams& p, hipStream_t stream) {
    const int nk = p.K / 128;
    if (!p.fp8 || p.col_scale == nullptr || p.K % 128 != 0 || nk < 4 || (nk & 1) || p.N % T_N != 0 || p.M < 4 || (p.M & 3) || p.ep.split_k > 1) return false;
    if (p.ep.bias != nullptr || p.ep.rank_u != nullptr || p.ep.drop_thr16 > 0) return false;
    if ((unsigned long long)p.M * p.lda >= (1ull << 32) || (unsigned long long)p.N * p.ldw >= (1ull << 32)) return false;
    const int kind = epilogue_kind(p.ep);
    const bool dual = p.dual_bf16 != nullptr;
    const void* fn = kind == EPI_BF16 ? (const void*)gemm256_fp8_dgrad_kernel<EPI_BF16>
                   : kind == EPI_MUL_AUX ? (dual ? (const void*)gemm256_fp8_dgrad_kernel<EPI_MUL_AUX, 2> : (const void*)gemm256_fp8_dgrad_kernel<EPI_MUL_AUX>)
                   : kind == EPI_MUL_AUX_U8 ? (dual ? (const void*)gemm256_fp8_dgrad_kernel<EPI_MUL_AUX_U8, 2> : (const void*)gemm256_fp8_dgrad_kernel<EPI_MUL_AUX_U8>)
                   : kind == EPI_MUL_AUX_12 ? (dual ? (const void*)gemm256_fp8_dgrad_kernel<EPI_MUL_AUX_12, 2> : (const void*)gemm256_fp8_dgrad_kernel<EPI_MUL_AUX_12>)
                   : kind == EPI_ADD_AUX ? (const void*)gemm256_fp8_dgrad_kernel<EPI_ADD_AUX> : nullptr;
    if (fn == nullptr) return false;
    const bool mul = epi_mul_aux_kind(kind);
    if ((p.out_fp8_scale > 0.f) != mul) return false;
    if ((!mul || dual) && p.a_row_dequant == nullptr) return false;
    if (dual && (!mul || (p.ld_dual & 7) || p.ld_dual < p.N || ((uintptr_t)p.dual_bf16 & 15))) return false;
    static const bool attr_ok = [] {
        bool ok = hipFuncSetAttribute((const void*)gemm256_fp8_dgrad_kernel<EPI_BF16>, hipFuncAttributeMaxDynamicSharedMemorySize, G256_LDS) == hipSuccess;
        ok = ok && hipFuncSetAttribute((const void*)gemm256_fp8_dgrad_kernel<EPI_MUL_AUX>, hipFuncAttributeMaxDynamicSharedMemorySize, G256_LDS) == hipSuccess;
        ok = ok && hipFuncSetAttribute((const void*)gemm256_fp8_dgrad_kernel<EPI_MUL_AUX_U8>, hipFuncAttributeMaxDynamicSharedMemorySize, G256_LDS) == hipSuccess;
        ok = ok && hipFuncSetAttribute((const void*)gemm256_fp8_dgrad_kernel<EPI_ADD_AUX>, hipFuncAttributeMaxDynamicSharedMemorySize, G256_LDS) == hipSuccess;
        ok = ok && hipFuncSetAttribute((const void*)gemm256_fp8_dgrad_kernel<EPI_MUL_AUX, 2>, hipFuncAttributeMaxDynamicSharedMemorySize, G256_LDS) == hipSuccess;
        ok = ok && hipFuncSetAttribute((const void*)gemm256_fp8_dgrad_kernel<EPI_MUL_AUX_U8, 2>, hipFuncAttributeMaxDynamicSharedMemorySize, G256_LDS) == hipSuccess;
        ok = ok && hipFuncSetAttribute((const void*)gemm256_fp8_dgrad_kernel<EPI_MUL_AUX_12>, hipFuncAttributeMaxDynamicSharedMemorySize, G256_LDS) == hipSuccess;
        ok = ok && hipFuncSetAttribute((const void*)gemm256_fp8_dgrad_kernel<EPI_MUL_AUX_12, 2>, hipFuncAttributeMaxDynamicSharedMemorySize, G256_LDS) == hipSuccess;
        return ok;
    }();
    if (!attr_ok) return false;
    GemmParams q = p;
    q.tiles_m = (p.M + T_M - 1) / T_M;
    q.tiles_n = p.N / T_N;
    q.splits = 1;
    q.nk_split = nk;
    q.split_stride = 0;
    q.band = q.tiles_n >= G256_WS_MIN_TILES_N ? -G256_WS_GROUP : 4;
    const long long tiles = (long long)q.tiles_m * q.tiles_n;
    const int grid = (int)(tiles < device_cus() ? tiles : device_cus());
    int ntiles_i = (int)tiles, skew = 0;
    long long* stamp = nullptr;
    void* args[] = {(void*)&q, (void*)&ntiles_i, (void*)&skew, (void*)&stamp};
    return hipLaunchKernel(fn, dim3((unsigned)grid), dim3(G256_THREADS), args, G256_LDS, stream) == hipSuccess;
}

bool gemm256_try_launch(const GemmParams& p, hipStream_t stream) {
    const int nk = p.K / T_K;
    if (p.K % T_K != 0 || nk < 4 || (nk & 1)) return false;
    if (p.N % T_N != 0) return false;
    if (p.ep.split_k > 1) return false;
    const long long tiles = (long long)((p.M + T_M - 1) / T_M) * (p.N / T_N);
    if (p.M < 1024 || tiles < 128) return false;
    if ((unsigned long long)p.M * p.lda * 2ull >= (1ull << 32) || (unsigned long long)p.N * p.ldw * 2ull >= (1ull << 32)) return false;
    static const bool attr_ok = [] {
        bool ok = true;
        for (int v = 0; v < 5; ++v)
            for (int k = 0; k < EPI_NUM_KINDS; ++k) {
                const void* fn = kernel_ptr(k, (v & 1) != 0, (v & 2) != 0, v == 4);
                if (fn != nullptr) ok = ok && hipFuncSetAttribute(fn, hipFuncAttributeMaxDynamicSharedMemorySize, G256_LDS) == hipSuccess;
            }
        return ok;
    }();
    if (!attr_ok) return false;
    static const int num_cus = [] {
        int dev = 0, n = 256;
        if (hipGetDevice(&dev) == hipSuccess) {
            hipDeviceProp_t prop;
            if (hipGetDeviceProperties(&prop, dev) == hipSuccess && prop.multiProcessorCount > 0) n = prop.multiProcessorCount;
        }
        return n;
    }();
    GemmParams q = p;
    q.tiles_m = (p.M + T_M - 1) / T_M;
    q.tiles_n = p.N / T_N;
    q.splits = 1;
    q.nk_split = nk;
    q.split_stride = 0;
    q.band = band_env_value() != 0 ? band_env_value() : (q.tiles_n >= G256_WS_MIN_TILES_N ? -G256_WS_GROUP : 4);
    int grid = (int)(tiles < num_cus ? tiles : num_cus);
#ifdef CLIBD_BALANCED_GRID
    if (tiles > num_cus) {
        const long long rounds = (tiles + num_cus - 1) / num_cus;
        grid = (int)((tiles + rounds - 1) / rounds);
    }
#endif
    const int kind = epilogue_kind(p.ep);
    int ntiles_i = (int)tiles;
    int skew_arg = skew_env_value();
    long long* stamp_arg = (p.ep.rank_u != nullptr) ? nullptr : g_stamp_buffer;
    const bool lora = p.ep.rank_u != nullptr;
    const bool diag = g_stamp_buffer != nullptr && !lora;
// ... 86 lines not shown
```

clibd_amd/csrc/gemm_common.h:

```cpp
#pragma once
#include "common.h"
#include "../../include/clibd_hip.h"

namespace clibd {

struct GemmParams {
    const unsigned short* A;
    const unsigned short* W;
    int M, N, K, lda, ldw;
    int tiles_m, tiles_n, ktiles_per_split;
    clibd_gemm_epilogue ep;
    int splits, nk_split;
    long long split_stride;
    int band;
    int hole_kt, hole_nkt;
    int fp8;
    const float* col_scale;
    float out_fp8_scale;
    const float* a_row_dequant;
    unsigned short* dual_bf16;
    int ld_dual;
    int sk_parts, sk_tail, sk_first, sk_nk_part;
    float* sk_ws;
    unsigned* sk_flags;
};

struct SkPlan { int parts, tail, first, nk_part; };
inline SkPlan plan_stream_k_tail(long long tiles, int num_cus, int nk) {
    SkPlan s{0, 0, 0, 0};
    if (tiles <= 0 || num_cus <= 0 || nk < 24 || (nk & 1)) return s;
    const long long full = (tiles / num_cus) * num_cus;
    const int tail = (int)(tiles - full);
    if (tail == 0 || 2 * tail > num_cus) return s;
    int P = num_cus / tail;
    if (P > 4) P = 4;
    for (; P >= 2; --P) {
        int nkp = (nk + P - 1) / P;
        nkp += nkp & 1;
        if (nkp < 4) nkp = 4;
        const int parts = (nk + nkp - 1) / nkp;
        const int last = nk - (parts - 1) * nkp;
        if (parts >= 2 && last >= 4 && (long long)parts * tail <= num_cus) { s.parts = parts; s.tail = tail; s.first = (int)full; s.nk_part = nkp; return s; }
    }
    return s;
}

__device__ __forceinline__ int w_col_of(int t, int i) { return 16 * (i >> 2) + 4 * t + (i & 3); }

__device__ __forceinline__ int tile_off(int row, int chunk) { return row * 128 + ((chunk ^ (row & 7)) << 4); }

__device__ __forceinline__ void tile_coords(int bid, int tiles_m, int tiles_n, int band, int& tile_m, int& tile_n) {
    const int ntiles = tiles_m * tiles_n;
    const int q = ntiles >> 3, r = ntiles & 7;
    const int xcd = bid & 7, idx = bid >> 3;
    bid = (xcd < r ? xcd * (q + 1) : r * (q + 1) + (xcd - r) * q) + idx;
    if (band < 0) {
        const int G = -band;
        const int g = bid / (tiles_m * G);
        const int rem = bid - g * tiles_m * G;
        const int gw = min(G, tiles_n - g * G);
        tile_m = rem / gw;
        tile_n = g * G + rem - tile_m * gw;
        return;
    }
    const int band_id = bid / (band * tiles_n);
    const int band_m0 = band_id * band;
    const int band_h = min(band, tiles_m - band_m0);
    const int in_band = bid - band_id * band * tiles_n;
    tile_m = band_m0 + in_band % band_h;
    tile_n = in_band / band_h;
}

__device__ __forceinline__ void load_bias16(const clibd_gemm_epilogue& ep, int nb, bool on, float bias[16]) {
#pragma unroll
    for (int e = 0; e < 16; ++e) bias[e] = 0.f;
    if (ep.bias != nullptr && on) {
#pragma unroll
        for (int q = 0; q < 4; ++q) {
            const f32x4 b4 = *(const f32x4*)(ep.bias + nb + 4 * q);
            bias[4 * q + 0] = b4[0]; bias[4 * q + 1] = b4[1]; bias[4 * q + 2] = b4[2]; bias[4 * q + 3] = b4[3];
        }
    }
}

__device__ __forceinline__ void store_row16(const clibd_gemm_epilogue& ep, int m, int nb, float v[16]) {
    if (ep.split_k > 1) {
        float* o = ep.out_f32 + (size_t)m * ep.ld_out_f32 + nb;
#pragma unroll
        for (int e = 0; e < 16; ++e) atomicAdd(o + e, v[e]);
        return;
    }
    if (ep.drop_thr16 > 0) {
        const unsigned base = (unsigned)m * (unsigned)ep.drop_ld + (unsigned)nb;
#pragma unroll
        for (int e = 0; e < 16; e += 2) {
            float f0, f1;
            drop_pair(ep.drop_seed, base + e, (unsigned)ep.drop_thr16, ep.drop_scale, f0, f1);
            v[e] *= f0;
            v[e + 1] *= f1;
        }
    }
    if (ep.act == CLIBD_ACT_GELU_SAVE_GRAD_E12) {
        float dg[16];
        gelu_and_grad_rows<16>(v, dg);
        gelu12_row8* o = (gelu12_row8*)((unsigned char*)ep.out_pre_bf16 + (size_t)m * ep.ld_pre + (nb >> 1) * 3);
        o[0] = gelu12_pack8(dg);
        o[1] = gelu12_pack8(dg + 8);
    } else if (ep.act == CLIBD_ACT_GELU_SAVE_GRAD_U8) {
        float dg[16];
        gelu_and_grad_rows<16>(v, dg);
        uint4 c;
        c.x = geluq_pack4(dg[0], dg[1], dg[2], dg[3]);   c.y = geluq_pack4(dg[4], dg[5], dg[6], dg[7]);
        c.z = geluq_pack4(dg[8], dg[9], dg[10], dg[11]); c.w = geluq_pack4(dg[12], dg[13], dg[14], dg[15]);
        store16_stream((unsigned char*)ep.out_pre_bf16 + (size_t)m * ep.ld_pre + nb, c);
    } else if (ep.act == CLIBD_ACT_GELU_SAVE_GRAD) {
        float dg[16];
        gelu_and_grad_rows<16>(v, dg);
        uint4 lo, hi;
        lo.x = pack2bf(dg[0], dg[1]);   lo.y = pack2bf(dg[2], dg[3]);   lo.z = pack2bf(dg[4], dg[5]);   lo.w = pack2bf(dg[6], dg[7]);
        hi.x = pack2bf(dg[8], dg[9]);   hi.y = pack2bf(dg[10], dg[11]); hi.z = pack2bf(dg[12], dg[13]); hi.w = pack2bf(dg[14], dg[15]);
        uint4* o = (uint4*)((unsigned short*)ep.out_pre_bf16 + (size_t)m * ep.ld_pre + nb);
        store16_stream(o, lo); store16_stream(o + 1, hi);
    } else if (ep.out_pre_bf16 != nullptr) {
        uint4 lo, hi;
        lo.x = pack2bf(v[0], v[1]);   lo.y = pack2bf(v[2], v[3]);   lo.z = pack2bf(v[4], v[5]);   lo.w = pack2bf(v[6], v[7]);
        hi.x = pack2bf(v[8], v[9]);   hi.y = pack2bf(v[10], v[11]); hi.z = pack2bf(v[12], v[13]); hi.w = pack2bf(v[14], v[15]);
        uint4* o = (uint4*)((unsigned short*)ep.out_pre_bf16 + (size_t)m * ep.ld_pre + nb);
        store16_stream(o, lo); store16_stream(o + 1, hi);
#pragma unroll
        for (int e = 0; e < 16; ++e) v[e] = bfround(v[e]);
    }
    if (ep.act == CLIBD_ACT_GELU) {
        gelu_rows<16>(v);
    } else if (ep.act == CLIBD_ACT_GELU_GRAD) {
        const uint4* ax = (const uint4*)((const unsigned short*)ep.aux_bf16 + (size_t)m * ep.ld_aux + nb);
        const uint4 x0 = ax[0], x1 = ax[1];
        const unsigned xs[8] = {x0.x, x0.y, x0.z, x0.w, x1.x, x1.y, x1.z, x1.w};
#pragma unroll
        for (int e = 0; e < 8; ++e) {
            v[2 * e] *= gelu_grad_f(bf2f((unsigned short)(xs[e] & 0xffffu)));
            v[2 * e + 1] *= gelu_grad_f(bf2f((unsigned short)(xs[e] >> 16)));
        }
    }
    if (ep.act == CLIBD_ACT_MUL_AUX_E12) {
        const gelu12_row8* ax = (const gelu12_row8*)((const unsigned char*)ep.aux_bf16 + (size_t)m * ep.ld_aux + (nb >> 1) * 3);
        const gelu12_row8 a0 = ax[0], a1 = ax[1];
        float d[16];
        gelu12_unpack8(a0.w0, a0.w1, a0.w2, d);
        gelu12_unpack8(a1.w0, a1.w1, a1.w2, d + 8);
#pragma unroll
        for (int e = 0; e < 16; ++e) v[e] *= d[e];
    }
    if (ep.act == CLIBD_ACT_MUL_AUX_U8) {
        const uint4 c = *(const uint4*)((const unsigned char*)ep.aux_bf16 + (size_t)m * ep.ld_aux + nb);
        const unsigned cs[4] = {c.x, c.y, c.z, c.w};
#pragma unroll
        for (int q = 0; q < 4; ++q) {
            float d[4];
            geluq_unpack4(cs[q], d);
            v[4 * q] *= d[0]; v[4 * q + 1] *= d[1]; v[4 * q + 2] *= d[2]; v[4 * q + 3] *= d[3];
        }
    }
    if (ep.act == CLIBD_ACT_MUL_AUX || ep.act == CLIBD_ACT_ADD_AUX) {
        const uint4* ax = (const uint4*)((const unsigned short*)ep.aux_bf16 + (size_t)m * ep.ld_aux + nb);
        const uint4 x0 = ax[0], x1 = ax[1];
        const unsigned xs[8] = {x0.x, x0.y, x0.z, x0.w, x1.x, x1.y, x1.z, x1.w};
#pragma unroll
        for (int e = 0; e < 8; ++e) {
            const float a0 = bf2f((unsigned short)(xs[e] & 0xffffu)), a1 = bf2f((unsigned short)(xs[e] >> 16));
            if (ep.act == CLIBD_ACT_MUL_AUX) { v[2 * e] *= a0; v[2 * e + 1] *= a1; }
            else { v[2 * e] += a0; v[2 * e + 1] += a1; }
        }
    }
    if (ep.residual_f32 != nullptr) {
        const f32x4* rs = (const f32x4*)(ep.residual_f32 + (size_t)m * ep.ld_res + nb);
#pragma unroll
        for (int q = 0; q < 4; ++q) {
            const f32x4 r4 = rs[q];
            v[4 * q + 0] += r4[0]; v[4 * q + 1] += r4[1]; v[4 * q + 2] += r4[2]; v[4 * q + 3] += r4[3];
        }
    }
    if (ep.out_f32 != nullptr) {
        f32x4* o = (f32x4*)(ep.out_f32 + (size_t)m * ep.ld_out_f32 + nb);
#pragma unroll
        for (int q = 0; q < 4; ++q) store16_stream(o + q, __builtin_bit_cast(uint4, (f32x4){v[4 * q], v[4 * q + 1], v[4 * q + 2], v[4 * q + 3]}));
    }
    if (ep.out_bf16 != nullptr) {
        uint4 lo, hi;
        lo.x = pack2bf(v[0], v[1]);   lo.y = pack2bf(v[2], v[3]);   lo.z = pack2bf(v[4], v[5]);   lo.w = pack2bf(v[6], v[7]);
        hi.x = pack2bf(v[8], v[9]);   hi.y = pack2bf(v[10], v[11]); hi.z = pack2bf(v[12], v[13]); hi.w = pack2bf(v[14], v[15]);
        uint4* o = (uint4*)((unsigned short*)ep.out_bf16 + (size_t)m * ep.ld_out_bf16 + nb);
        store16_stream(o, lo); store16_stream(o + 1, hi);
    }
}

__device__ __forceinline__ void load_bias8(const clibd_gemm_epilogue& ep, int nb, float bias[8]) {
#pragma unroll
    for (int e = 0; e < 8; ++e) bias[e] = 0.f;
    if (ep.bias != nullptr) {
        const f32x4 b0 = *(const f32x4*)(ep.bias + nb), b1 = *(const f32x4*)(ep.bias + nb + 4);
        bias[0] = b0[0]; bias[1] = b0[1]; bias[2] = b0[2]; bias[3] = b0[3];
        bias[4] = b1[0]; bias[5] = b1[1]; bias[6] = b1[2]; bias[7] = b1[3];
    }
}

__device__ __forceinline__ uint4 pack8bf(const float v[8]) {
    uint4 o;
    o.x = pack2bf(v[0], v[1]); o.y = pack2bf(v[2], v[3]); o.z = pack2bf(v[4], v[5]); o.w = pack2bf(v[6], v[7]);
    return o;
}

enum : int {
    EPI_GENERIC = 0,
    EPI_BF16 = 1,
    EPI_GELU_SAVE = 2,
    EPI_MUL_AUX = 3,
    EPI_RES_F32 = 4,
    EPI_RES_F32_DROP = 5,
    EPI_SPLITK_F32 = 6,
    EPI_ADD_AUX = 7,
    EPI_GELU_SAVE_U8 = 8,
    EPI_MUL_AUX_U8 = 9,
    EPI_RES_F32_COPY = 10,
    EPI_ROWNORM_GELU = 11,
    EPI_GELU_SAVE_12 = 12,
    EPI_MUL_AUX_12 = 13,
    EPI_GELU = 14,
    EPI_F32 = 15,
    EPI_NUM_KINDS = 16,
};
constexpr bool epi_aux_kind(int kind) { return kind == EPI_MUL_AUX || kind == EPI_ADD_AUX || kind == EPI_MUL_AUX_U8 || kind == EPI_MUL_AUX_12; }
constexpr bool epi_mul_aux_kind(int kind) { return kind == EPI_MUL_AUX || kind == EPI_MUL_AUX_U8 || kind == EPI_MUL_AUX_12; }

__host__ __device__ inline int epilogue_kind(const clibd_gemm_epilogue& ep) {
    if (ep.split_k > 1) return EPI_GENERIC;
    const bool drop = ep.drop_thr16 > 0;
    if (ep.row_sums != nullptr)
        return (ep.act == CLIBD_ACT_NONE && !drop && !ep.out_pre_bf16 && ep.residual_f32 && ep.out_f32 && ep.out_bf16 && !ep.rank_u && ep.bias) ? EPI_RES_F32_COPY : -1;
    if (ep.row_stats != nullptr)
        return (ep.act == CLIBD_ACT_GELU_SAVE_GRAD && !drop && ep.out_pre_bf16 && !ep.residual_f32 && !ep.out_f32 && ep.out_bf16 && !ep.rank_u && ep.bias && ep.col_sum_w) ? EPI_ROWNORM_GELU : -1;
    if (ep.act == CLIBD_ACT_NONE && !drop && !ep.out_pre_bf16 && !ep.residual_f32 && !ep.out_f32 && ep.out_bf16) return EPI_BF16;
    if (ep.act == CLIBD_ACT_GELU_SAVE_GRAD && !drop && ep.out_pre_bf16 && !ep.residual_f32 && !ep.out_f32 && ep.out_bf16) return EPI_GELU_SAVE;
    if (ep.act == CLIBD_ACT_GELU && !drop && !ep.out_pre_bf16 && !ep.residual_f32 && !ep.out_f32 && ep.out_bf16) return EPI_GELU;
    if (ep.act == CLIBD_ACT_MUL_AUX && !drop && !ep.out_pre_bf16 && !ep.residual_f32 && !ep.out_f32 && ep.out_bf16 && ep.aux_bf16) return EPI_MUL_AUX;
    if (ep.act == CLIBD_ACT_ADD_AUX && !drop && !ep.out_pre_bf16 && !ep.residual_f32 && !ep.out_f32 && ep.out_bf16 && ep.aux_bf16) return EPI_ADD_AUX;
    if (ep.act == CLIBD_ACT_GELU_SAVE_GRAD_U8 && !drop && ep.out_pre_bf16 && !ep.residual_f32 && !ep.out_f32 && ep.out_bf16) return EPI_GELU_SAVE_U8;
    if (ep.act == CLIBD_ACT_MUL_AUX_U8 && !drop && !ep.out_pre_bf16 && !ep.residual_f32 && !ep.out_f32 && ep.out_bf16 && ep.aux_bf16) return EPI_MUL_AUX_U8;
    if (ep.act == CLIBD_ACT_GELU_SAVE_GRAD_E12 && !drop && ep.out_pre_bf16 && !ep.residual_f32 && !ep.out_f32 && ep.out_bf16) return EPI_GELU_SAVE_12;
    if (ep.act == CLIBD_ACT_MUL_AUX_E12 && !drop && !ep.out_pre_bf16 && !ep.residual_f32 && !ep.out_f32 && ep.out_bf16 && ep.aux_bf16) return EPI_MUL_AUX_12;
    if (ep.act == CLIBD_ACT_GELU_SAVE_GRAD_E12 || ep.act == CLIBD_ACT_MUL_AUX_E12) return -1;
    if (ep.act == CLIBD_ACT_NONE && !ep.out_pre_bf16 && ep.residual_f32 && ep.out_f32 && !ep.out_bf16) return drop ? EPI_RES_F32_DROP : EPI_RES_F32;
    if (ep.act == CLIBD_ACT_NONE && !drop && !ep.out_pre_bf16 && !ep.residual_f32 && ep.out_f32 && !ep.out_bf16) return EPI_F32;
    return EPI_GENERIC;
}

template <int KIND>
__device__ __forceinline__ void store_row8(const clibd_gemm_epilogue& ep, int m, int nb, float v[8]) {
    if (KIND == EPI_BF16) {
        *(uint4*)((unsigned short*)ep.out_bf16 + (size_t)m * ep.ld_out_bf16 + nb) = pack8bf(v);
        return;
    }
    if (KIND == EPI_F32) {
        f32x4* o = (f32x4*)(ep.out_f32 + (size_t)m * ep.ld_out_f32 + nb);
        o[0] = (f32x4){v[0], v[1], v[2], v[3]};
        o[1] = (f32x4){v[4], v[5], v[6], v[7]};
        return;
    }
    if (KIND == EPI_GELU) {
        gelu_rows<8>(v);
        *(uint4*)((unsigned short*)ep.out_bf16 + (size_t)m * ep.ld_out_bf16 + nb) = pack8bf(v);
        return;
    }
    if (KIND == EPI_GELU_SAVE) {
        float dg[8];
        gelu_and_grad_rows<8>(v, dg);
        *(uint4*)((unsigned short*)ep.out_pre_bf16 + (size_t)m * ep.ld_pre + nb) = pack8bf(dg);
        *(uint4*)((unsigned short*)ep.out_bf16 + (size_t)m * ep.ld_out_bf16 + nb) = pack8bf(v);
        return;
    }
    if (KIND == EPI_GELU_SAVE_U8) {
        float dg[8];
        gelu_and_grad_rows<8>(v, dg);
        *(uint2*)((unsigned char*)ep.out_pre_bf16 + (size_t)m * ep.ld_pre + nb) =
            make_uint2(geluq_pack4(dg[0], dg[1], dg[2], dg[3]), geluq_pack4(dg[4], dg[5], dg[6], dg[7]));
        *(uint4*)((unsigned short*)ep.out_bf16 + (size_t)m * ep.ld_out_bf16 + nb) = pack8bf(v);
        return;
    }
    if (KIND == EPI_MUL_AUX_U8) {
        const uint2 c = *(const uint2*)((const unsigned char*)ep.aux_bf16 + (size_t)m * ep.ld_aux + nb);
        float d0[4], d1[4];
        geluq_unpack4(c.x, d0);
        geluq_unpack4(c.y, d1);
#pragma unroll
        for (int e = 0; e < 4; ++e) { v[e] *= d0[e]; v[4 + e] *= d1[e]; }
        *(uint4*)((unsigned short*)ep.out_bf16 + (size_t)m * ep.ld_out_bf16 + nb) = pack8bf(v);
        return;
    }
    if (KIND == EPI_GELU_SAVE_12) {
        float dg[8];
        gelu_and_grad_rows<8>(v, dg);
        *(gelu12_row8*)((unsigned char*)ep.out_pre_bf16 + (size_t)m * ep.ld_pre + (nb >> 1) * 3) = gelu12_pack8(dg);
        *(uint4*)((unsigned short*)ep.out_bf16 + (size_t)m * ep.ld_out_bf16 + nb) = pack8bf(v);
        return;
    }
    if (KIND == EPI_MUL_AUX_12) {
        const gelu12_row8 a = *(const gelu12_row8*)((const unsigned char*)ep.aux_bf16 + (size_t)m * ep.ld_aux + (nb >> 1) * 3);
        float d[8];
        gelu12_unpack8(a.w0, a.w1, a.w2, d);
#pragma unroll
        for (int e = 0; e < 8; ++e) v[e] *= d[e];
        *(uint4*)((unsigned short*)ep.out_bf16 + (size_t)m * ep.ld_out_bf16 + nb) = pack8bf(v);
        return;
    }
    if (KIND == EPI_MUL_AUX || KIND == EPI_ADD_AUX) {
        const uint4 x0 = *(const uint4*)((const unsigned short*)ep.aux_bf16 + (size_t)m * ep.ld_aux + nb);
        const unsigned xs[4] = {x0.x, x0.y, x0.z, x0.w};
#pragma unroll
        for (int e = 0; e < 4; ++e) {
            const float a0 = bf2f((unsigned short)(xs[e] & 0xffffu)), a1 = bf2f((unsigned short)(xs[e] >> 16));
            if (KIND == EPI_MUL_AUX) { v[2 * e] *= a0; v[2 * e + 1] *= a1; }
            else { v[2 * e] += a0; v[2 * e + 1] += a1; }
        }
        *(uint4*)((unsigned short*)ep.out_bf16 + (size_t)m * ep.ld_out_bf16 + nb) = pack8bf(v);
        return;
    }
    if (KIND == EPI_GENERIC || KIND == EPI_RES_F32_DROP) {
        if (KIND == EPI_RES_F32_DROP || ep.drop_thr16 > 0) {
            const unsigned base = (unsigned)m * (unsigned)ep.drop_ld + (unsigned)nb;
#pragma unroll
            for (int e = 0; e < 8; e += 2) {
                float f0, f1;
                drop_pair(ep.drop_seed, base + e, (unsigned)ep.drop_thr16, ep.drop_scale, f0, f1);
                v[e] *= f0;
                v[e + 1] *= f1;
            }
        }
    }
    if (KIND == EPI_GENERIC) {
        if (ep.act == CLIBD_ACT_GELU_SAVE_GRAD_U8) {
            float dg[8];
            gelu_and_grad_rows<8>(v, dg);
            *(uint2*)((unsigned char*)ep.out_pre_bf16 + (size_t)m * ep.ld_pre + nb) =
                make_uint2(geluq_pack4(dg[0], dg[1], dg[2], dg[3]), geluq_pack4(dg[4], dg[5], dg[6], dg[7]));
        } else if (ep.act == CLIBD_ACT_GELU_SAVE_GRAD) {
            float dg[8];
            gelu_and_grad_rows<8>(v, dg);
            *(uint4*)((unsigned short*)ep.out_pre_bf16 + (size_t)m * ep.ld_pre + nb) = pack8bf(dg);
        } else if (ep.out_pre_bf16 != nullptr) {
            *(uint4*)((unsigned short*)ep.out_pre_bf16 + (size_t)m * ep.ld_pre + nb) = pack8bf(v);
#pragma unroll
            for (int e = 0; e < 8; ++e) v[e] = bfround(v[e]);
        }
        if (ep.act == CLIBD_ACT_GELU) {
            gelu_rows<8>(v);
        } else if (ep.act == CLIBD_ACT_MUL_AUX_U8) {
            const uint2 c = *(const uint2*)((const unsigned char*)ep.aux_bf16 + (size_t)m * ep.ld_aux + nb);
            float d0[4], d1[4];
            geluq_unpack4(c.x, d0);
            geluq_unpack4(c.y, d1);
#pragma unroll
            for (int e = 0; e < 4; ++e) { v[e] *= d0[e]; v[4 + e] *= d1[e]; }
        } else if (ep.act == CLIBD_ACT_GELU_GRAD || ep.act == CLIBD_ACT_MUL_AUX || ep.act == CLIBD_ACT_ADD_AUX) {
            const uint4 x0 = *(const uint4*)((const unsigned short*)ep.aux_bf16 + (size_t)m * ep.ld_aux + nb);
            const unsigned xs[4] = {x0.x, x0.y, x0.z, x0.w};
#pragma unroll
            for (int e = 0; e < 4; ++e) {
                const float a0 = bf2f((unsigned short)(xs[e] & 0xffffu)), a1 = bf2f((unsigned short)(xs[e] >> 16));
                if (ep.act == CLIBD_ACT_GELU_GRAD) {
                    v[2 * e] *= gelu_grad_f(a0);
                    v[2 * e + 1] *= gelu_grad_f(a1);
                } else if (ep.act == CLIBD_ACT_MUL_AUX) {
                    v[2 * e] *= a0;
                    v[2 * e + 1] *= a1;
                } else {
                    v[2 * e] += a0;
                    v[2 * e + 1] += a1;
                }
            }
        }
    }
    if (KIND == EPI_RES_F32 || KIND == EPI_RES_F32_DROP || ep.residual_f32 != nullptr) {
        const f32x4* rs = (const f32x4*)(ep.residual_f32 + (size_t)m * ep.ld_res + nb);
        const f32x4 r0 = rs[0], r1 = rs[1];
        v[0] += r0[0]; v[1] += r0[1]; v[2] += r0[2]; v[3] += r0[3];
        v[4] += r1[0]; v[5] += r1[1]; v[6] += r1[2]; v[7] += r1[3];
    }
    if (KIND == EPI_RES_F32 || KIND == EPI_RES_F32_DROP || ep.out_f32 != nullptr) {
        f32x4* o = (f32x4*)(ep.out_f32 + (size_t)m * ep.ld_out_f32 + nb);
        o[0] = (f32x4){v[0], v[1], v[2], v[3]};
        o[1] = (f32x4){v[4], v[5], v[6], v[7]};
    }
    if (KIND == EPI_GENERIC && ep.out_bf16 != nullptr) *(uint4*)((unsigned short*)ep.out_bf16 + (size_t)m * ep.ld_out_bf16 + nb) = pack8bf(v);
}

__device__ __forceinline__ void store_row8_gelu_fp8(const clibd_gemm_epilogue& ep, int m, int nb, float v[8], float out_scale) {
    float dg[8];
    gelu_and_grad_rows<8>(v, dg);
    *(uint4*)((unsigned short*)ep.out_pre_bf16 + (size_t)m * ep.ld_pre + nb) = pack8bf(dg);
    *(uint2*)((unsigned char*)ep.out_bf16 + (size_t)m * ep.ld_out_bf16 + nb) = pack8fp8(v, out_scale);
}

template <int KIND>
__device__ __forceinline__ void fold_row8_in(const clibd_gemm_epilogue& ep, int m, int nb, float v[8], const uint4& ax, const f32x4& r0,
                                             const f32x4& r1) {
    if (KIND == EPI_MUL_AUX_U8) {
        float d0[4], d1[4];
        geluq_unpack4(ax.x, d0);
        geluq_unpack4(ax.y, d1);
#pragma unroll
        for (int e = 0; e < 4; ++e) { v[e] *= d0[e]; v[4 + e] *= d1[e]; }
    } else if (KIND == EPI_MUL_AUX_12) {
        float d[8];
        gelu12_unpack8(ax.x, ax.y, ax.z, d);
#pragma unroll
        for (int e = 0; e < 8; ++e) v[e] *= d[e];
    } else if (KIND == EPI_MUL_AUX || KIND == EPI_ADD_AUX) {
        const unsigned xs[4] = {ax.x, ax.y, ax.z, ax.w};
#pragma unroll
        for (int e = 0; e < 4; ++e) {
            const float a0 = bf2f((unsigned short)(xs[e] & 0xffffu)), a1 = bf2f((unsigned short)(xs[e] >> 16));
            if (KIND == EPI_MUL_AUX) { v[2 * e] *= a0; v[2 * e + 1] *= a1; }
            else { v[2 * e] += a0; v[2 * e + 1] += a1; }
        }
    } else {
        if (KIND == EPI_RES_F32_DROP) {
            const unsigned base = (unsigned)m * (unsigned)ep.drop_ld + (unsigned)nb;
#pragma unroll
            for (int e = 0; e < 8; e += 2) {
                float f0, f1;
                drop_pair(ep.drop_seed, base + e, (unsigned)ep.drop_thr16, ep.drop_scale, f0, f1);
                v[e] *= f0;
                v[e + 1] *= f1;
            }
        }
        v[0] += r0[0]; v[1] += r0[1]; v[2] += r0[2]; v[3] += r0[3];
        v[4] += r1[0]; v[5] += r1[1]; v[6] += r1[2]; v[7] += r1[3];
    }
}

__device__ __forceinline__ void fold_rownorm8(float v[8], float mean, float rstd, const float s[8], const float b[8]) {
#pragma unroll
    for (int e = 0; e < 8; ++e) v[e] = fmaf(rstd, fmaf(-mean, s[e], v[e]), b[e]);
}

__device__ __forceinline__ float row16_sum(float x) {
    x += dpp_mov<DPP_QUAD_XOR1>(x);
    x += dpp_mov<DPP_QUAD_XOR2>(x);
    x += dpp_mov<DPP_ROW_HALF_MIRROR>(x);
    x += dpp_mov<DPP_ROW_MIRROR>(x);
    return x;
}

template <bool NT>
__device__ __forceinline__ uint4 load_aux16(const void* p) {
    typedef unsigned aux_u32x4 __attribute__((ext_vector_type(4)));
#ifndef CLIBD_PLAIN_AUX_LOADS
    const aux_u32x4 v = NT ? __builtin_nontemporal_load((const aux_u32x4*)p) : *(const aux_u32x4*)p;
#else
    const aux_u32x4 v = *(const aux_u32x4*)p;
#endif
    return make_uint4(v[0], v[1], v[2], v[3]);
}
#ifndef CLIBD_NT_ADD_AUX
#define CLIBD_NT_ADD_AUX 0
#endif
constexpr bool epi_aux_nt(int kind) { return kind != EPI_ADD_AUX || CLIBD_NT_ADD_AUX; }

__device__ __forceinline__ uint4 load_aux12(const void* p) {
    typedef unsigned aux_u32x3 __attribute__((ext_vector_type(3), aligned(4)));
#ifndef CLIBD_PLAIN_AUX_LOADS
    const aux_u32x3 v = __builtin_nontemporal_load((const aux_u32x3*)p);
#else
    const aux_u32x3 v = *(const aux_u32x3*)p;
#endif
    return make_uint4(v[0], v[1], v[2], 0u);
}

template <int KIND>
__device__ __forceinline__ void fold_row8(const clibd_gemm_epilogue& ep, int m, int nb, float v[8]) {
    uint4 ax = make_uint4(0u, 0u, 0u, 0u);
    f32x4 r0 = (f32x4){0.f, 0.f, 0.f, 0.f}, r1 = r0;
    if (KIND == EPI_MUL_AUX_U8) {
        const uint2 c = *(const uint2*)((const unsigned char*)ep.aux_bf16 + (size_t)m * ep.ld_aux + nb);
        ax.x = c.x; ax.y = c.y;
    } else if (KIND == EPI_MUL_AUX_12) {
        ax = load_aux12((const unsigned char*)ep.aux_bf16 + (size_t)m * ep.ld_aux + (nb >> 1) * 3);
    } else if (KIND == EPI_MUL_AUX || KIND == EPI_ADD_AUX) {
        ax = load_aux16<epi_aux_nt(KIND)>((const unsigned short*)ep.aux_bf16 + (size_t)m * ep.ld_aux + nb);
    } else {
        const f32x4* rs = (const f32x4*)(ep.residual_f32 + (size_t)m * ep.ld_res + nb);
        r0 = rs[0];
        r1 = rs[1];
    }
    fold_row8_in<KIND>(ep, m, nb, v, ax, r0, r1);
}

inline int plan_k_slices(int nk, int tiles, int num_cus, int* nks_out) {
    int splits = num_cus / (tiles > 0 ? tiles : 1);
    if (splits < 1) splits = 1;
    if (splits > nk / 4) splits = nk / 4;
    if (splits < 1) splits = 1;
    int nks = (nk + splits - 1) / splits;
    nks += nks & 1;
    if (nks < 4) nks = 4;
    if (nks > nk) nks = nk;
    splits = (nk + nks - 1) / nks;
    while (nk - (splits - 1) * nks < 4 && nks < nk) {
        nks += 2;
        if (nks > nk) nks = nk;
        splits = (nk + nks - 1) / nks;
    }
    *nks_out = nks;
    return splits;
}

bool gemm256_try_launch(const GemmParams& p, hipStream_t stream);
size_t gemm256_tail_workspace_bytes(int M, int N, int K);
bool gemm256_fp8_launch(const GemmParams& p, hipStream_t stream);
bool gemm256_fp8_dgrad_launch(const GemmParams& p, hipStream_t stream);
int gemm256_splitk_launch(const GemmParams& p, float* partials, size_t partials_elems, hipStream_t stream);

int gemm256_tn_splitk_launch(const unsigned short* A, int lda, const unsigned short* B, int ldb, int M, int Na, int Nb, float* partials,
                             size_t partials_elems, float* colsum, hipStream_t stream, float* colsum_partials = nullptr);
int gemm256_tn_fp8b_splitk_launch(const unsigned short* A, int lda, const unsigned char* B8, int ldb, float b_scale, int M, int Na, int Nb,
                                  float* partials, size_t partials_elems, float* colsum, hipStream_t stream, float* colsum_partials = nullptr);

}
```

clibd_amd/csrc/layernorm.hip:

```cpp
#include "common.h"
#include "../../include/clibd_hip.h"
#include "host_util.h"

namespace clibd {

constexpr int LN_MAX_CHUNKS = 4;

__device__ __forceinline__ float wave_reduce8(float v[8], int lane) {
    float w4[4], w2[2];
#pragma unroll
    for (int i = 0; i < 4; ++i) {
        float a = v[i], b = v[i + 4];
        permlane32_swap(a, b);
        w4[i] = a + b;
    }
#pragma unroll
    for (int i = 0; i < 2; ++i) {
        float a = w4[i], b = w4[i + 2];
        permlane16_swap(a, b);
        w2[i] = a + b;
    }
    const bool b3 = lane & 8;
    const float keep = b3 ? w2[1] : w2[0];
    const float send = b3 ? w2[0] : w2[1];
    float w1 = keep + dpp_mov<DPP_ROW_ROR8>(send);
    w1 += dpp_mov<DPP_ROW_HALF_MIRROR>(w1);
    w1 += dpp_mov<DPP_QUAD_XOR1>(w1);
    w1 += dpp_mov<DPP_QUAD_XOR2>(w1);
    return w1;
}

template <int NCH, bool LORA, int ROWS>
__global__ __launch_bounds__(256) void layernorm_fwd_kernel(const float* __restrict__ x, int M, int H,
                                                            const float* __restrict__ gamma,
                                                            const float* __restrict__ beta, float eps,
                                                            unsigned short* __restrict__ y_bf16,
                                                            float* __restrict__ y_f32, float* __restrict__ stats,
                                                            const unsigned short* __restrict__ lora_a,
                                                            unsigned short* __restrict__ t_bf16, unsigned drop_seed,
                                                            int drop_thr16, float drop_scale,
                                                            unsigned char* __restrict__ y_fp8, float fp8_scale) {
    extern __shared__ __attribute__((aligned(16))) float a_lds[];
    const int lane = threadIdx.x & 63;
    const int wave_in_grid = blockIdx.x * 4 + (threadIdx.x >> 6);
    const int nwaves = gridDim.x * 4;
    if (LORA) {
        for (int i = threadIdx.x; i < 8 * H; i += 256) a_lds[i] = bf2f(lora_a[i]);
        __syncthreads();
    }
    f32x4 g[NCH], b[NCH];
    bool act[NCH];
#pragma unroll
    for (int j = 0; j < NCH; ++j) {
        const int c = 4 * (lane + 64 * j);
        act[j] = c < H;
        g[j] = act[j] ? *(const f32x4*)(gamma + c) : (f32x4){0, 0, 0, 0};
        b[j] = act[j] ? *(const f32x4*)(beta + c) : (f32x4){0, 0, 0, 0};
    }
    const float invH = 1.0f / (float)H;
    for (int row0 = wave_in_grid * ROWS; row0 < M; row0 += nwaves * ROWS) {
        f32x4 v[ROWS][NCH];
        float mean[ROWS], rstd[ROWS];
        bool live[ROWS];
#pragma unroll
        for (int rr = 0; rr < ROWS; ++rr) {
            live[rr] = row0 + rr < M;
            const float* xr = x + (size_t)min(row0 + rr, M - 1) * H;
#pragma unroll
            for (int j = 0; j < NCH; ++j) v[rr][j] = act[j] ? *(const f32x4*)(xr + 4 * (lane + 64 * j)) : (f32x4){0, 0, 0, 0};
        }
#pragma unroll
        for (int rr = 0; rr < ROWS; ++rr) {
            float s = 0.f;
#pragma unroll
            for (int j = 0; j < NCH; ++j) s += (v[rr][j][0] + v[rr][j][1]) + (v[rr][j][2] + v[rr][j][3]);
            mean[rr] = wave_sum(s) * invH;
            float q = 0.f;
#pragma unroll
            for (int j = 0; j < NCH; ++j) {
                if (act[j]) {
#pragma unroll
                    for (int e = 0; e < 4; ++e) {
                        const float d = v[rr][j][e] - mean[rr];
                        q += d * d;
                    }
                }
            }
            const float var = wave_sum(q) * invH;
            rstd[rr] = rsqrtf(var + eps);
            if (stats != nullptr && lane == 0 && live[rr]) *(float2*)(stats + 2 * (size_t)(row0 + rr)) = make_float2(mean[rr], rstd[rr]);
        }
        float tp[ROWS][8];
#pragma unroll
        for (int rr = 0; rr < ROWS; ++rr)
#pragma unroll
            for (int r = 0; r < 8; ++r) tp[rr][r] = 0.f;
#pragma unroll
        for (int j = 0; j < NCH; ++j) {
            if (!act[j]) continue;
            const int c = 4 * (lane + 64 * j);
            float yb[ROWS][4];
#pragma unroll
            for (int rr = 0; rr < ROWS; ++rr) {
                const int row = row0 + rr;
                f32x4 y;
#pragma unroll
                for (int e = 0; e < 4; ++e) y[e] = (v[rr][j][e] - mean[rr]) * rstd[rr] * g[j][e] + b[j][e];
                if (drop_thr16 > 0) {
                    const unsigned base = (unsigned)row * (unsigned)H + (unsigned)c;
                    float f0, f1, f2, f3;
                    drop_pair(drop_seed, base, (unsigned)drop_thr16, drop_scale, f0, f1);
                    drop_pair(drop_seed, base + 2, (unsigned)drop_thr16, drop_scale, f2, f3);
                    y[0] *= f0; y[1] *= f1; y[2] *= f2; y[3] *= f3;
                }
                uint2 pk;
                pk.x = pack2bf(y[0], y[1]);
                pk.y = pack2bf(y[2], y[3]);
                if (live[rr]) {
                    if (y_f32 != nullptr) *(f32x4*)(y_f32 + (size_t)row * H + c) = y;
                    if (y_bf16 != nullptr) *(uint2*)(y_bf16 + (size_t)row * H + c) = pk;
                    if (y_fp8 != nullptr)
                        *(unsigned*)(y_fp8 + (size_t)row * H + c) = pack4fp8(y[0] * fp8_scale, y[1] * fp8_scale, y[2] * fp8_scale, y[3] * fp8_scale);
                }
                yb[rr][0] = bf2f((unsigned short)(pk.x & 0xffff)); yb[rr][1] = bf2f((unsigned short)(pk.x >> 16));
                yb[rr][2] = bf2f((unsigned short)(pk.y & 0xffff)); yb[rr][3] = bf2f((unsigned short)(pk.y >> 16));
            }
            if (LORA) {
#pragma unroll
                for (int r = 0; r < 8; ++r) {
                    const f32x4 a = *(const f32x4*)(a_lds + r * H + c);
#pragma unroll
                    for (int rr = 0; rr < ROWS; ++rr)
                        tp[rr][r] += (yb[rr][0] * a[0] + yb[rr][1] * a[1]) + (yb[rr][2] * a[2] + yb[rr][3] * a[3]);
                }
            }
        }
        if (LORA) {
#pragma unroll
            for (int rr = 0; rr < ROWS; ++rr) {
                const float tv = wave_reduce8(tp[rr], lane);
                if ((lane & 7) == 0 && live[rr]) t_bf16[(size_t)(row0 + rr) * 8 + (lane >> 3)] = f2bf(tv);
            }
        }
    }
}

template <int NCH, bool PG, int ROWS, bool F8>
__device__ __forceinline__ void layernorm_bwd_body(const unsigned short* __restrict__ dy_bf16,
                                                   const float* __restrict__ dy_f32,
                                                   const float* __restrict__ x,
                                                   const float* __restrict__ stats,
                                                   const float* __restrict__ gamma, int M, int H,
                                                   const float* __restrict__ dres,
                                                   float* __restrict__ dx_f32,
                                                   unsigned short* __restrict__ dx_bf16, unsigned drop_seed,
                                                   int drop_thr16, float drop_scale, float* __restrict__ dgamma,
                                                   float* __restrict__ dbeta, const unsigned short* __restrict__ dres_b16,
                                                   unsigned short* __restrict__ dx_res_b16, unsigned char* __restrict__ dx_fp8,
                                                   float* __restrict__ row_dequant, float* __restrict__ pg_ws) {
    const int lane = threadIdx.x & 63;
    const int wave_in_grid = blockIdx.x * 4 + (threadIdx.x >> 6);
    const int nwaves = gridDim.x * 4;
    f32x4 g[NCH];
    f32x4 pgam[PG ? NCH : 1], pbet[PG ? NCH : 1];
    bool act[NCH];
#pragma unroll
    for (int j = 0; j < NCH; ++j) {
        const int c = 4 * (lane + 64 * j);
        act[j] = c < H;
        g[j] = act[j] ? *(const f32x4*)(gamma + c) : (f32x4){0, 0, 0, 0};
        if (PG) { pgam[j] = (f32x4){0, 0, 0, 0}; pbet[j] = (f32x4){0, 0, 0, 0}; }
    }
    const float invH = 1.0f / (float)H;
    for (int row0 = wave_in_grid * ROWS; row0 < M; row0 += nwaves * ROWS) {
        constexpr bool RS16 = F8 && ROWS == 2;
        f32x4 gy[ROWS][NCH], xh[ROWS][NCH], rs[RS16 ? 1 : ROWS][RS16 ? 1 : NCH];
        uint2 rsp[RS16 ? ROWS : 1][RS16 ? NCH : 1];
        float rstd[ROWS], m1[ROWS], m2[ROWS];
        bool live[ROWS];
#pragma unroll
        for (int rr = 0; rr < ROWS; ++rr) {
            live[rr] = row0 + rr < M;
            const size_t row = (size_t)min(row0 + rr, M - 1);
            const float mean = stats[2 * row];
            rstd[rr] = stats[2 * row + 1];
#pragma unroll
            for (int j = 0; j < NCH; ++j) {
                gy[rr][j] = (f32x4){0, 0, 0, 0};
                xh[rr][j] = (f32x4){0, 0, 0, 0};
                if constexpr (RS16) rsp[rr][j] = make_uint2(0u, 0u);
                else rs[rr][j] = (f32x4){0, 0, 0, 0};
                if (!act[j]) continue;
                const int c = 4 * (lane + 64 * j);
                f32x4 d;
                if (dy_f32 != nullptr) {
                    d = *(const f32x4*)(dy_f32 + row * H + c);
                } else {
                    const uint2 pk = *(const uint2*)(dy_bf16 + row * H + c);
                    d[0] = bf2f((unsigned short)(pk.x & 0xffff)); d[1] = bf2f((unsigned short)(pk.x >> 16));
                    d[2] = bf2f((unsigned short)(pk.y & 0xffff)); d[3] = bf2f((unsigned short)(pk.y >> 16));
                }
                const f32x4 xv = *(const f32x4*)(x + row * H + c);
                if constexpr (RS16) {
                    if (dres_b16 != nullptr) rsp[rr][j] = *(const uint2*)(dres_b16 + row * H + c);
                } else {
                    if (dres != nullptr) rs[rr][j] = *(const f32x4*)(dres + row * H + c);
                    if (dres_b16 != nullptr) {
                        const uint2 pk = *(const uint2*)(dres_b16 + row * H + c);
                        rs[rr][j][0] += bf2f((unsigned short)(pk.x & 0xffff)); rs[rr][j][1] += bf2f((unsigned short)(pk.x >> 16));
                        rs[rr][j][2] += bf2f((unsigned short)(pk.y & 0xffff)); rs[rr][j][3] += bf2f((unsigned short)(pk.y >> 16));
                    }
                }
#pragma unroll
                for (int e = 0; e < 4; ++e) {
                    gy[rr][j][e] = d[e] * g[j][e];
                    xh[rr][j][e] = (xv[e] - mean) * rstd[rr];
                    if (PG && live[rr]) { pgam[j][e] += d[e] * xh[rr][j][e]; pbet[j][e] += d[e]; }
                }
            }
        }
#pragma unroll
        for (int rr = 0; rr < ROWS; ++rr) {
            float s1 = 0.f, s2 = 0.f;
#pragma unroll
            for (int j = 0; j < NCH; ++j)
#pragma unroll
                for (int e = 0; e < 4; ++e) {
                    s1 += gy[rr][j][e];
                    s2 += gy[rr][j][e] * xh[rr][j][e];
                }
            m1[rr] = wave_sum(s1) * invH;
            m2[rr] = wave_sum(s2) * invH;
        }
#pragma unroll
        for (int rr = 0; rr < ROWS; ++rr) {
            if (!live[rr]) continue;
            const size_t row = (size_t)(row0 + rr);
            float amax = 0.f;
#pragma unroll
            for (int j = 0; j < NCH; ++j) {
                if (!act[j]) continue;
                const int c = 4 * (lane + 64 * j);
                f32x4 o, rv;
                if constexpr (RS16) {
                    const uint2 pk = rsp[rr][j];
                    rv[0] = bf2f((unsigned short)(pk.x & 0xffff)); rv[1] = bf2f((unsigned short)(pk.x >> 16));
                    rv[2] = bf2f((unsigned short)(pk.y & 0xffff)); rv[3] = bf2f((unsigned short)(pk.y >> 16));
                } else {
                    rv = rs[rr][j];
                }
#pragma unroll
                for (int e = 0; e < 4; ++e) o[e] = rstd[rr] * (gy[rr][j][e] - m1[rr] - xh[rr][j][e] * m2[rr]) + rv[e];
                if (dx_f32 != nullptr) *(f32x4*)(dx_f32 + row * H + c) = o;
                if (dx_res_b16 != nullptr) {
                    uint2 pk;
                    pk.x = pack2bf(o[0], o[1]);
                    pk.y = pack2bf(o[2], o[3]);
                    *(uint2*)(dx_res_b16 + row * H + c) = pk;
                }
                if (dx_bf16 != nullptr || F8) {
// ... 218 lines not shown
```

clibd_amd/engine.py:

```python
from __future__ import annotations

import math
import os
from dataclasses import dataclass, field
from typing import List, Optional, Sequence

import torch

from . import ops

BF16, F32 = torch.bfloat16, torch.float32


class NotSupportedYet(NotImplementedError):
    pass


NUMERICS_CHOICES = dict(residual_grad=("bf16", "fp32"), gelu_grad=("bf16", "u8", "e4m7"), attn_bwd=("2phase", "sp"), ln_fold=("off", "on"),
                        dgrad=("bf16", "fp8"))
_NUMERICS_ENV = dict(residual_grad="CLIBD_RESIDUAL_GRAD", gelu_grad="CLIBD_GELU_GRAD", attn_bwd="CLIBD_ATTN_BWD", ln_fold="CLIBD_LN_FOLD",
                     dgrad="CLIBD_DGRAD")


def default_deterministic() -> bool:
    return os.environ.get("CLIBD_DETERMINISTIC", "0") == "1"


def _ordered(on: bool) -> dict:
    return {"ordered": True} if on else {}


def default_numerics() -> dict:
    out = {}
    for k, choices in NUMERICS_CHOICES.items():
        v = os.environ.get(_NUMERICS_ENV[k], choices[0]).lower()
        out[k] = v if v in choices else choices[0]
    return out


def check_numerics(settings: dict) -> dict:
    for k, v in settings.items():
        if k not in NUMERICS_CHOICES:
            raise ValueError(f"unknown numerics switch {k!r} (known: {sorted(NUMERICS_CHOICES)})")
        if v not in NUMERICS_CHOICES[k]:
            raise ValueError(f"numerics switch {k}: {v!r} is not one of {NUMERICS_CHOICES[k]}")
    return settings


def _mul_aux_act(h, FF: int) -> int:
    if h.dtype == torch.uint8:
        return ops.ACT_MUL_AUX_E12 if h.shape[1] == 3 * FF // 2 else ops.ACT_MUL_AUX_U8
    return ops.ACT_MUL_AUX


@dataclass
class LoraParams:
    a_q: torch.nn.Parameter
    b_q: torch.nn.Parameter
    a_v: torch.nn.Parameter
    b_v: torch.nn.Parameter

    def tensors(self):
        return [self.a_q, self.b_q, self.a_v, self.b_v]


@dataclass
class LayerSpec:
    qkv_w: Sequence[torch.Tensor]
    qkv_b: Sequence[torch.Tensor]
    proj_w: torch.Tensor
    proj_b: torch.Tensor
    fc1_w: torch.Tensor
    fc1_b: torch.Tensor
    fc2_w: torch.Tensor
    fc2_b: torch.Tensor
    ln1_w: torch.Tensor
    ln1_b: torch.Tensor
    ln2_w: torch.Tensor
    ln2_b: torch.Tensor
    lora: Optional[LoraParams] = None

    def frozen(self):
        return [*self.qkv_w, *self.qkv_b, self.proj_w, self.proj_b, self.fc1_w, self.fc1_b, self.fc2_w, self.fc2_b, self.ln1_w,
                self.ln1_b, self.ln2_w, self.ln2_b]


class _LayerCache:
    __slots__ = ("wqkv", "wqkv_t", "bqkv", "wo", "wo_t", "bo", "w1", "w1_t", "b1", "w2", "w2_t", "b2", "g1", "be1", "g2", "be2",
                 "v_fwd", "v_bwd", "a_cat", "w_dt", "slot2", "wqkv8", "cs_qkv", "wo8", "cs_o", "w18", "cs_1", "w28", "cs_2",
                 "w1g", "s1", "b1f",
                 "wo_t8", "cs_ot", "w1_t8", "cs_1t", "w2_t8", "cs_2t", "c2")


def _f32c(t: torch.Tensor) -> torch.Tensor:
    t = t.detach()
    return t if (t.dtype == F32 and t.is_contiguous()) else t.to(F32).contiguous()


def _rank_slots(lp: "LoraParams"):
    a_q, a_v, b_q, b_v = _f32c(lp.a_q), _f32c(lp.a_v), _f32c(lp.b_q), _f32c(lp.b_v)
    r, H = a_q.shape

    def slot(lo):
        hi = min(lo + 4, r)
        k = hi - lo
        pa = lambda a: a[lo:hi].contiguous() if k == 4 else torch.cat([a[lo:hi], a.new_zeros((4 - k, H))], dim=0)
        pb = lambda b: (b[:, lo:hi] if k == 4 else torch.cat([b[:, lo:hi], b.new_zeros((H, 4 - k))], dim=1)).contiguous()
        return pa(a_q), pa(a_v), pb(b_q), pb(b_v)

    return [slot(lo) for lo in range(0, r, 4)]


class TransformerStack:

    def __init__(self, layers: List[LayerSpec], hidden: int, heads: int, pre_ln: bool, eps: float):
        if hidden != heads * 64:
            raise NotSupportedYet(f"attention kernel is specialised for head_dim 64 (hidden={hidden}, heads={heads})")
        if hidden % 64 or hidden > 1024:
            raise NotSupportedYet("hidden size must be a multiple of 64 and <= 1024")
        self.layers, self.H, self.heads, self.pre_ln, self.eps = layers, hidden, heads, pre_ln, eps
        self.FF = layers[0].fc1_w.shape[0]
        self._cache: List[_LayerCache] = []
        self._cache_key = None
        self.fp8 = None
        self._calib = None
        self.numerics = default_numerics()
        self.deterministic = default_deterministic()
        self._c2, self._c2_age = None, 0
        self.dgrad8_sites = ("mlp", "proj")

    DGRAD8_C2_EVERY = 64

    def set_numerics(self, **settings):
        before = (self.numerics.get("ln_fold"), self.numerics.get("dgrad"))
        self.numerics.update(check_numerics(settings))
        if (self.numerics.get("ln_fold"), self.numerics.get("dgrad")) != before:
            self._cache_key = None
            self._c2 = None

    def _dgrad8_ok(self) -> bool:
        if self.numerics["dgrad"] != "fp8":
            return False
        if self.numerics["residual_grad"] != "bf16":
            raise NotSupportedYet("dgrad=fp8 needs residual_grad=bf16")
        if self.H % 256 or self.H < 512 or self.FF % 256:
            raise NotSupportedYet("dgrad=fp8 needs hidden % 256 == 0, hidden >= 512, intermediate % 256 == 0")
        return True

    FP8_SITES = ("qkv_in", "proj_in", "fc1_in", "fc2_in")
    FP8_SCALES = dict(qkv_in=8.0, proj_in=32.0, fc1_in=8.0, fc2_in=4.0)

    def enable_fp8(self, scales: Optional[dict] = None, amax: Optional[list] = None, margin: float = 2.0, sites: Optional[Sequence[str]] = None):
        if sites is not None:
            sites = tuple(sites)
            if any(s not in self.FP8_SITES for s in sites):
                raise ValueError(f"enable_fp8: sites must come from {self.FP8_SITES}")
            if set(sites) != set(self.FP8_SITES):
                if set(sites) != {"fc1_in", "fc2_in"}:
                    raise NotSupportedYet("fp8 site selection: only the MLP pair (fc1_in, fc2_in) is built")
        if self.full_mode() and (sites is None or set(sites) != {"fc1_in", "fc2_in"}):
            raise NotSupportedYet("fp8 forward on every site needs frozen base weights (their gradients would need the bf16 GEMM inputs); "
                                  "with trainable base weights the MLP-pair selection (sites=('fc1_in', 'fc2_in')) is built")
        if self.H % 256 or self.H < 512 or self.FF % 256:
            raise NotSupportedYet("fp8 forward needs hidden % 256 == 0, hidden >= 512, intermediate % 256 == 0")
        base = dict(self.FP8_SCALES, **(scales or {}))
        if sites is not None:
            base = {k: v for k, v in base.items() if k in sites}
        per_layer = []
        for i in range(len(self.layers)):
            d = dict(base)
            if amax is not None:
                for site, v in amax[i].items():
                    if site not in d:
                        continue
                    v = float(v)
                    if v > 0.0 and math.isfinite(v):
                        d[site] = 2.0 ** math.floor(math.log2(448.0 / (margin * v)))
            per_layer.append(d)
        self.fp8 = per_layer
        self._cache_key = None

    def disable_fp8(self):
        self.fp8 = None
        self._cache_key = None

    def calibrate(self, on: bool = True):
        if on:
            self._calib = []
            return None
        rec, self._calib = self._calib, None
        return [{k: float(v) for k, v in d.items()} for d in (rec or [])]

    def _key(self):
        k = 0
        for L in self.layers:
            for p in L.frozen():
                k += p._version + (p.data_ptr() & 0xFFFF)
        return (k, self.layers[0].proj_w.device)

    def full_mode(self) -> bool:
        return any(p.requires_grad for L in self.layers for p in L.frozen())

    def base_params(self):
        return [p for L in self.layers for p in L.frozen()]

    def refresh(self):
        key = self._key()
        if key == self._cache_key and not self.full_mode():
            return
        self._cache = []
        with torch.no_grad():
            for L in self.layers:
                c = _LayerCache()
                wqkv = _f32c(L.qkv_w[0]) if len(L.qkv_w) == 1 else torch.cat([_f32c(w) for w in L.qkv_w], dim=0)
                c.wqkv, c.wqkv_t = ops.cast_bf16(wqkv), ops.cast_transpose_bf16(wqkv)
                c.bqkv = _f32c(L.qkv_b[0]).clone() if len(L.qkv_b) == 1 else torch.cat([_f32c(b) for b in L.qkv_b], dim=0)
                c.wo, c.wo_t, c.bo = ops.cast_bf16(_f32c(L.proj_w)), ops.cast_transpose_bf16(_f32c(L.proj_w)), _f32c(L.proj_b)
                c.w1, c.w1_t, c.b1 = ops.cast_bf16(_f32c(L.fc1_w)), ops.cast_transpose_bf16(_f32c(L.fc1_w)), _f32c(L.fc1_b)
                c.w2, c.w2_t, c.b2 = ops.cast_bf16(_f32c(L.fc2_w)), ops.cast_transpose_bf16(_f32c(L.fc2_w)), _f32c(L.fc2_b)
                c.g1, c.be1, c.g2, c.be2 = _f32c(L.ln1_w), _f32c(L.ln1_b), _f32c(L.ln2_w), _f32c(L.ln2_b)
                if self.fp8 is not None:
                    f8 = self.fp8[len(self._cache)]
                    if "qkv_in" in f8:
                        c.wqkv8, c.cs_qkv = ops.quantize_rows_fp8(wqkv.contiguous(), f8["qkv_in"])
                        c.wo8, c.cs_o = ops.quantize_rows_fp8(_f32c(L.proj_w), f8["proj_in"])
                    c.w18, c.cs_1 = ops.quantize_rows_fp8(_f32c(L.fc1_w), f8["fc1_in"])
                    c.w28, c.cs_2 = ops.quantize_rows_fp8(_f32c(L.fc2_w), f8["fc2_in"])
                c.w1g = c.s1 = c.b1f = None
                if self.pre_ln and self.numerics["ln_fold"] == "on" and not self.full_mode():
                    c.w1g, c.s1, c.b1f = ops.ln_fold_weights(_f32c(L.fc1_w), c.g2, c.be2, c.b1)
                c.v_fwd = c.v_bwd = c.a_cat = c.w_dt = c.slot2 = None
                c.wo_t8 = c.cs_ot = c.w1_t8 = c.cs_1t = c.w2_t8 = c.cs_2t = c.c2 = None
                self._cache.append(c)
            if self._dgrad8_ok():
                dev = self._cache[0].w2_t.device
                full = self.full_mode()
                reuse = full and self._c2 is not None and len(self._c2) == len(self._cache) and self._c2_age < self.DGRAD8_C2_EVERY
                l1 = None if reuse else torch.zeros((len(self._cache),), dtype=F32, device=dev)
                for i, c in enumerate(self._cache):
                    c.w2_t8, c.cs_2t = ops.quantize_rows_fp8_bf16(c.w2_t, 1.0, None if reuse else l1[i:i + 1])
                    c.wo_t8, c.cs_ot = ops.quantize_rows_fp8_bf16(c.wo_t, 1.0)
                if reuse:
                    self._c2_age += 1
                else:
                    self._c2 = [2.0 ** (math.floor(math.log2(448.0 / (256.0 * 1.13 * max(v, 1e-30)))) - (1 if full else 0))
                                for v in l1.cpu().tolist()]
                    self._c2_age = 1
                for c, c2 in zip(self._cache, self._c2):
                    c.c2 = c2
                    c.w1_t8, c.cs_1t = ops.quantize_rows_fp8_bf16(c.w1_t, c.c2)
        self._cache_key = key

    def pack_lora(self):
        H = self.H
        for L, c in zip(self.layers, self._cache):
            if L.lora is None:
                continue
            dev = L.proj_w.device
            images = lambda: dict(v_fwd=torch.empty((3 * H, 8), dtype=BF16, device=dev), v_bwd=torch.empty((H, 8), dtype=BF16, device=dev),
                                  a_cat=torch.empty((8, H), dtype=BF16, device=dev), w_dt=torch.empty((16, 3 * H), dtype=BF16, device=dev))
            if c.v_fwd is None:
                im = images()
                c.v_fwd, c.v_bwd, c.a_cat, c.w_dt = im["v_fwd"], im["v_bwd"], im["a_cat"], im["w_dt"]
            slots = _rank_slots(L.lora)
            ops.lora_pack(*slots[0], c.v_fwd, c.v_bwd, c.a_cat, c.w_dt)
            if len(slots) > 1:
                if self.fp8 is not None:
                    raise NotSupportedYet("fp8 forward with LoRA rank > 4")
                if c.slot2 is None or len(c.slot2) != len(slots) - 1:
                    c.slot2 = [images() for _ in slots[1:]]
                for sl, im in zip(slots[1:], c.slot2):
                    ops.lora_pack(*sl, im["v_fwd"], im["v_bwd"], im["a_cat"], im["w_dt"])
            else:
                c.slot2 = None

    def _slot2_addend(self, u, v, N, residual=None):
        M = u.shape[0]
        out = torch.empty((M, N), dtype=F32, device=u.device)
        ops.gemm_nt(torch.zeros((M, 64), dtype=BF16, device=u.device), torch.zeros((N, 64), dtype=BF16, device=u.device), rank_u=u, rank_v=v,
                    residual=residual, out_f32=out)
        return out

    def _slot2_fwd(self, c, x_bf16):
        add32, ts = None, []
        for im in c.slot2:
            tj = ops.lora_down_proj(x_bf16, im["a_cat"])
            add32 = self._slot2_addend(tj, im["v_fwd"], 3 * self.H, residual=add32)
            ts.append(tj)
        return add32, ts

    def _slot2_bwd_addend(self, c, dt2, residual=None):
        add32 = residual
        for im, dtj in zip(c.slot2, dt2):
            add32 = self._slot2_addend(dtj, im["v_bwd"], self.H, residual=add32)
        return add32

    def lora_a(self, i: int):
        if i >= len(self.layers) or self.layers[i].lora is None:
            return None
        return self._cache[i].a_cat

    def forward(self, x_f32, x_bf16, t0, B: int, S: int, key_mask, save: bool, cls_only_last: bool = False, drop=None, full: bool = False,
                x_fp8=None):
        H, FF, M = self.H, self.FF, B * S
        dev = x_f32.device
        saved = []
        new = lambda cols, dt: torch.empty((M, cols), dtype=dt, device=dev)
        keep = save and full
        f8s = self.fp8
        mlp_only = f8s is not None and "qkv_in" not in f8s[0]
        if f8s is not None and full and not mlp_only:
            raise NotSupportedYet("fp8 forward on every site with trainable base weights (the MLP-pair selection is built)")
        cal = self._calib if f8s is None else None
        amax = lambda t_: t_.abs().amax().float()
        f8 = None
        AT = ops.FP8 if f8s is not None else BF16
        o = None if keep else new(H, BF16 if mlp_only else AT)
        a = None if keep else new(FF, AT)
        xn2 = new(H, AT) if (self.pre_ln and not keep) else None
        xn8 = new(H, ops.FP8) if (f8s is not None and not mlp_only) else None
        gg = self.numerics["gelu_grad"]
        if f8s is not None or (self.pre_ln and self.numerics["ln_fold"] == "on"):
            gg = "bf16"
        GG = BF16 if gg == "bf16" else torch.uint8
        HC = 3 * FF // 2 if gg == "e4m7" else FF
        act_save = {"bf16": ops.ACT_GELU_SAVE_GRAD, "u8": ops.ACT_GELU_SAVE_GRAD_U8, "e4m7": ops.ACT_GELU_SAVE_GRAD_E12}[gg]
        h_tmp = new(FF, BF16) if (f8s is not None and not save) else None
        t = t0
        sp_ok = save and key_mask is None and f8s is None and S <= 224 and self.numerics["attn_bwd"] == "sp"
        fold = (self.pre_ln and self.numerics["ln_fold"] == "on" and self._cache[0].w1g is not None and f8s is None and not full and GG == BF16 and H % 256 == 0 and FF % 256 == 0
                and M >= 1024 and ((M + 255) // 256) * (H // 256) >= 128 and H % 128 == 0)
        fold_sums = torch.empty((H // 128, M, 2), dtype=F32, device=dev) if fold else None
        if fold and h_tmp is None and not save:
            h_tmp = new(FF, BF16)
        for i, (L, c) in enumerate(zip(self.layers, self._cache)):
            has_lora = L.lora is not None
            rec = {}
            att_sv = None
            t2 = None
            f8 = f8s[i] if f8s is not None else None
            crec = {} if cal is not None else None
            if keep:
                o, a = new(H, BF16), new(FF, AT)
                xn2 = new(H, AT) if self.pre_ln else None
            if self.pre_ln and cls_only_last and i == len(self.layers) - 1:
                xn = new(H, BF16)
                st1 = torch.empty((M, 2), dtype=F32, device=dev)
                t = torch.empty((M, 8), dtype=BF16, device=dev) if has_lora else None
                qkv = new(3 * H, BF16)
                if f8 is not None and not mlp_only:
                    ops.layernorm_fwd(x_f32, c.g1, c.be1, self.eps, y_bf16=xn, stats=st1, lora_a=c.a_cat if has_lora else None, t_out=t,
                                      y_fp8=xn8, fp8_scale=f8["qkv_in"])
                    ops.gemm_fp8_nt(xn8, c.wqkv8, c.cs_qkv, bias=c.bqkv, rank_u=t, rank_v=c.v_fwd if has_lora else None, out_bf16=qkv)
                else:
                    ops.layernorm_fwd(x_f32, c.g1, c.be1, self.eps, y_bf16=xn, stats=st1, lora_a=c.a_cat if has_lora else None, t_out=t)
                    add32, t2 = self._slot2_fwd(c, xn) if c.slot2 is not None else (None, None)
                    ops.gemm_nt(xn, c.wqkv, bias=c.bqkv, rank_u=t, rank_v=c.v_fwd if has_lora else None, residual=add32, out_bf16=qkv)
                    if crec is not None:
                        crec["qkv_in"] = amax(xn)
                newB = lambda cols, dt: torch.empty((B, cols), dtype=dt, device=dev)
                o_cls = newB(H, BF16)
                ops.attention_fwd(qkv, B, S, self.heads, key_mask, o_cls, nq=1)
                x_cls = ops.gather_rows(x_f32.view(B, S, H))
                x1 = newB(H, F32)
                ops.gemm_nt(o_cls, c.wo, bias=c.bo, residual=x_cls, out_f32=x1)
                st2 = torch.empty((B, 2), dtype=F32, device=dev)
                xn2c = newB(H, BF16)
                ops.layernorm_fwd(x1, c.g2, c.be2, self.eps, y_bf16=xn2c, stats=st2)
                h = newB(HC, GG) if save else None
                ac = newB(FF, BF16)
                ops.gemm_nt(xn2c, c.w1, bias=c.b1, act=act_save if save else ops.ACT_GELU, out_pre=h, out_bf16=ac)
                x2 = newB(H, F32)
                ops.gemm_nt(ac, c.w2, bias=c.b2, residual=x1, out_f32=x2)
                if save:
                    rec = dict(x_in=x_f32, st1=st1, xn=xn, t=t, t2=t2, qkv=qkv, x1=x1, st2=st2, h=h, cls_only=True)
                    if keep:
                        rec.update(o=o_cls, xn2=xn2c, a=ac)
                x_f32 = x2
            elif self.pre_ln:
                xn = new(H, BF16)
                st1 = torch.empty((M, 2), dtype=F32, device=dev)
                t = torch.empty((M, 8), dtype=BF16, device=dev) if has_lora else None
                qkv = new(3 * H, BF16)
                x1 = new(H, F32)
                st2 = torch.empty((M, 2), dtype=F32, device=dev)
                h = new(HC, GG) if save else None
                x2 = new(H, F32)
                if f8 is not None and mlp_only:
                    ops.layernorm_fwd(x_f32, c.g1, c.be1, self.eps, y_bf16=xn, stats=st1, lora_a=c.a_cat if has_lora else None, t_out=t)
                    add32, t2 = self._slot2_fwd(c, xn) if c.slot2 is not None else (None, None)
                    ops.gemm_nt(xn, c.wqkv, bias=c.bqkv, rank_u=t, rank_v=c.v_fwd if has_lora else None, residual=add32, out_bf16=qkv)
                    ops.attention_fwd(qkv, B, S, self.heads, key_mask, o)
                    ops.gemm_nt(o, c.wo, bias=c.bo, residual=x_f32, out_f32=x1)
                    ops.layernorm_fwd(x1, c.g2, c.be2, self.eps, stats=st2, y_fp8=xn2, fp8_scale=f8["fc1_in"])
                    ops.gemm_fp8_nt(xn2, c.w18, c.cs_1, bias=c.b1, gelu_out_fp8=a, gelu_out_scale=f8["fc2_in"], out_pre=h if save else h_tmp)
                    ops.gemm_fp8_nt(a, c.w28, c.cs_2, bias=c.b2, residual=x1, out_f32=x2)
                elif f8 is not None:
                    ops.layernorm_fwd(x_f32, c.g1, c.be1, self.eps, y_bf16=xn, stats=st1, lora_a=c.a_cat if has_lora else None, t_out=t,
                                      y_fp8=xn8, fp8_scale=f8["qkv_in"])
                    ops.gemm_fp8_nt(xn8, c.wqkv8, c.cs_qkv, bias=c.bqkv, rank_u=t, rank_v=c.v_fwd if has_lora else None, out_bf16=qkv)
                    ops.attention_fwd(qkv, B, S, self.heads, key_mask, o, out_fp8_scale=f8["proj_in"])
                    ops.gemm_fp8_nt(o, c.wo8, c.cs_o, bias=c.bo, residual=x_f32, out_f32=x1)
                    ops.layernorm_fwd(x1, c.g2, c.be2, self.eps, stats=st2, y_fp8=xn2, fp8_scale=f8["fc1_in"])
                    ops.gemm_fp8_nt(xn2, c.w18, c.cs_1, bias=c.b1, gelu_out_fp8=a, gelu_out_scale=f8["fc2_in"], out_pre=h if save else h_tmp)
                    ops.gemm_fp8_nt(a, c.w28, c.cs_2, bias=c.b2, residual=x1, out_f32=x2)
                else:
                    ops.layernorm_fwd(x_f32, c.g1, c.be1, self.eps, y_bf16=xn, stats=st1, lora_a=c.a_cat if has_lora else None, t_out=t)
                    add32, t2 = self._slot2_fwd(c, xn) if c.slot2 is not None else (None, None)
                    ops.gemm_nt(xn, c.wqkv, bias=c.bqkv, rank_u=t, rank_v=c.v_fwd if has_lora else None, residual=add32, out_bf16=qkv)
                    if sp_ok:
                        o = o if keep else new(H, BF16)
                        att_sv = dict(o_att=o, o_lo=new(H, BF16), lse=torch.empty((B * self.heads * S,), dtype=F32, device=dev))
                        ops.attention_fwd(qkv, B, S, self.heads, None, o, lse=att_sv["lse"], o_lo=att_sv["o_lo"])
                    else:
                        ops.attention_fwd(qkv, B, S, self.heads, key_mask, o)
                    if fold and cal is None:
                        ops.gemm_nt(o, c.wo, bias=c.bo, residual=x_f32, out_f32=x1, out_bf16=xn2, row_sums=fold_sums)
                        ops.rowsum_finalize(fold_sums, self.eps, st2)
                        ops.gemm_nt(xn2, c.w1g, bias=c.b1f, act=ops.ACT_GELU_SAVE_GRAD, out_pre=h if save else h_tmp, out_bf16=a, row_stats=st2, col_sum_w=c.s1)
                    else:
                        ops.gemm_nt(o, c.wo, bias=c.bo, residual=x_f32, out_f32=x1)
                        ops.layernorm_fwd(x1, c.g2, c.be2, self.eps, y_bf16=xn2, stats=st2)
                        ops.gemm_nt(xn2, c.w1, bias=c.b1, act=act_save if save else ops.ACT_GELU, out_pre=h if save else None, out_bf16=a)
                    ops.gemm_nt(a, c.w2, bias=c.b2, residual=x1, out_f32=x2)
                    if crec is not None:
                        crec.update(qkv_in=amax(xn), proj_in=amax(o), fc1_in=amax(xn2), fc2_in=amax(a))
                if save:
                    rec = dict(x_in=x_f32, st1=st1, xn=xn, t=t, t2=t2, qkv=qkv, x1=x1, st2=st2, h=h)
                    if keep:
                        rec.update(o=o, xn2=xn2, a=a)
                        if f8 is not None:
                            rec.update(xn2_s=f8["fc1_in"], a_s=f8["fc2_in"])
                    if att_sv is not None:
                        rec.update(att_sv)
                x_f32 = x2
            else:
                d_att = d_h1 = d_h2 = None
                if drop is not None:
                    p_h, p_a, base = drop
                    d_att = ops.Drop(p_a, ops.derive_seed(base, i, 0))
                    d_h1 = ops.Drop(p_h, ops.derive_seed(base, i, 1))
                    d_h2 = ops.Drop(p_h, ops.derive_seed(base, i, 2))
                qkv = new(3 * H, BF16)
                s1 = new(H, F32)
                x1_f32 = new(H, F32)
                st1 = torch.empty((M, 2), dtype=F32, device=dev)
                h = new(HC, GG) if save else None
                s2 = new(H, F32)
                x2_f32, x2_bf16 = new(H, F32), new(H, BF16)
                st2 = torch.empty((M, 2), dtype=F32, device=dev)
                nxt = self.lora_a(i + 1)
                t_next = torch.empty((M, 8), dtype=BF16, device=dev) if nxt is not None else None
                ru, rv = (t if has_lora else None), (c.v_fwd if has_lora else None)
                if f8 is not None and mlp_only:
                    x1_bf16 = None
                    x18 = new(H, ops.FP8)
                    ops.gemm_nt(x_bf16, c.wqkv, bias=c.bqkv, rank_u=ru, rank_v=rv, out_bf16=qkv)
                    ops.attention_fwd(qkv, B, S, self.heads, key_mask, o, drop=d_att)
                    ops.gemm_nt(o, c.wo, bias=c.bo, residual=x_f32, out_f32=s1, drop=d_h1)
                    ops.layernorm_fwd(s1, c.g1, c.be1, self.eps, y_f32=x1_f32, stats=st1, y_fp8=x18, fp8_scale=f8["fc1_in"])
                    ops.gemm_fp8_nt(x18, c.w18, c.cs_1, bias=c.b1, gelu_out_fp8=a, gelu_out_scale=f8["fc2_in"], out_pre=h if save else h_tmp)
                    ops.gemm_fp8_nt(a, c.w28, c.cs_2, bias=c.b2, residual=x1_f32, out_f32=s2, drop=d_h2)
                    ops.layernorm_fwd(s2, c.g2, c.be2, self.eps, y_bf16=x2_bf16, y_f32=x2_f32, stats=st2, lora_a=nxt, t_out=t_next)
                elif f8 is not None:
                    if x_fp8 is None:
                        raise ValueError("fp8 forward (post-LN): the caller passes the e4m3 image of x")
                    x1_bf16 = None
                    x18 = xn8
                    ops.gemm_fp8_nt(x_fp8, c.wqkv8, c.cs_qkv, bias=c.bqkv, rank_u=ru, rank_v=rv, out_bf16=qkv)
                    ops.attention_fwd(qkv, B, S, self.heads, key_mask, o, drop=d_att, out_fp8_scale=f8["proj_in"])
                    ops.gemm_fp8_nt(o, c.wo8, c.cs_o, bias=c.bo, residual=x_f32, out_f32=s1, drop=d_h1)
                    ops.layernorm_fwd(s1, c.g1, c.be1, self.eps, y_f32=x1_f32, stats=st1, y_fp8=x18, fp8_scale=f8["fc1_in"])
                    ops.gemm_fp8_nt(x18, c.w18, c.cs_1, bias=c.b1, gelu_out_fp8=a, gelu_out_scale=f8["fc2_in"], out_pre=h if save else h_tmp)
                    ops.gemm_fp8_nt(a, c.w28, c.cs_2, bias=c.b2, residual=x1_f32, out_f32=s2, drop=d_h2)
                    x8_next = new(H, ops.FP8)
                    ops.layernorm_fwd(s2, c.g2, c.be2, self.eps, y_bf16=x2_bf16, y_f32=x2_f32, stats=st2, lora_a=nxt, t_out=t_next,
                                      y_fp8=x8_next, fp8_scale=f8s[min(i + 1, len(f8s) - 1)]["qkv_in"])
                    x_fp8 = x8_next
                else:
                    x1_bf16 = new(H, BF16)
                    add32, t2 = self._slot2_fwd(c, x_bf16) if c.slot2 is not None else (None, None)
                    ops.gemm_nt(x_bf16, c.wqkv, bias=c.bqkv, rank_u=ru, rank_v=rv, residual=add32, out_bf16=qkv)
                    if sp_ok:
                        o = o if keep else new(H, BF16)
                        att_sv = dict(o_att=o, o_lo=new(H, BF16), lse=torch.empty((B * self.heads * S,), dtype=F32, device=dev))
                        ops.attention_fwd(qkv, B, S, self.heads, None, o, drop=d_att, lse=att_sv["lse"], o_lo=att_sv["o_lo"])
                    else:
                        ops.attention_fwd(qkv, B, S, self.heads, key_mask, o, drop=d_att)
                    ops.gemm_nt(o, c.wo, bias=c.bo, residual=x_f32, out_f32=s1, drop=d_h1)
                    ops.layernorm_fwd(s1, c.g1, c.be1, self.eps, y_bf16=x1_bf16, y_f32=x1_f32, stats=st1)
                    ops.gemm_nt(x1_bf16, c.w1, bias=c.b1, act=act_save if save else ops.ACT_GELU, out_pre=h if save else None, out_bf16=a)
                    ops.gemm_nt(a, c.w2, bias=c.b2, residual=x1_f32, out_f32=s2, drop=d_h2)
                    ops.layernorm_fwd(s2, c.g2, c.be2, self.eps, y_bf16=x2_bf16, y_f32=x2_f32, stats=st2, lora_a=nxt, t_out=t_next)
                    if crec is not None:
                        crec.update(qkv_in=amax(x_bf16), proj_in=amax(o), fc1_in=amax(x1_bf16), fc2_in=amax(a))
                if save:
                    rec = dict(x_bf16=x_bf16, t=t if has_lora else None, t2=t2, qkv=qkv, s1=s1, st1=st1, h=h, s2=s2, st2=st2,
                               d_att=d_att, d_h1=d_h1, d_h2=d_h2)
                    if keep:
                        rec.update(o=o, x1_bf16=x1_bf16, a=a)
                        if f8 is not None:
                            rec.update(x1_bf16=x18, x1_s=f8["fc1_in"], a_s=f8["fc2_in"])
                    if att_sv is not None:
                        rec.update(att_sv)
                x_f32, x_bf16, t = x2_f32, x2_bf16, t_next
            saved.append(rec)
            if cal is not None:
                cal.append(crec)
        return x_f32, x_bf16, saved

    def layer_params(self, i: int):
        L = self.layers[i]
        return L.frozen() + (L.lora.tensors() if L.lora is not None else [])

    def backward(self, dx_f32, dx_bf16, saved, B: int, S: int, key_mask, grads: dict, full: bool = False, on_layer_done=None):
        H, FF, M = self.H, self.FF, B * S
        dev = dx_f32.device
        new = lambda cols, dt: torch.empty((M, cols), dtype=dt, device=dev)
        dh = None
        dtmp = new(H, BF16)
        dqkv = new(3 * H, BF16)
        dt = torch.empty((M, 16), dtype=BF16, device=dev)
        first_lora = min((i for i, L in enumerate(self.layers) if L.lora is not None), default=len(self.layers))
        if full:
            first_lora = -1
        r16 = self.numerics["residual_grad"] == "bf16"
        dg8 = self._dgrad8_ok() and self._cache[0].w2_t8 is not None and M % 4 == 0 and M * FF < 2 ** 32
        new8 = lambda cols: (torch.empty((M, cols), dtype=torch.uint8, device=dev).view(ops.FP8), torch.empty((M,), dtype=F32, device=dev))
        f8kw = lambda pair: dict(dx_fp8=pair[0], row_dequant=pair[1])
        dx8 = None
        det = self.deterministic
        pg = lambda w, b: (dict(dgamma=grads[id(w)].view(-1), dbeta=grads[id(b)].view(-1), **_ordered(det))
                           if full and id(w) in grads else {})
        wg = lambda dy, x, ws, bs, xs=None: linear_wgrad(dy, x, ws, bs, grads, x_scale=xs, **_ordered(det)) if full else None
        for i in range(len(self.layers) - 1, -1, -1):
            L, c, rec = self.layers[i], self._cache[i], saved[i]
            has_lora = L.lora is not None
            dt2 = None
            if i < first_lora:
                break
            if self.pre_ln and rec.get("cls_only"):
                newB = lambda cols, dt: torch.empty((B, cols), dtype=dt, device=dev)
                dhc, dtc = newB(FF, BF16), newB(H, BF16)
                wg(dx_bf16, rec.get("a"), [L.fc2_w], [L.fc2_b])
                ops.gemm_nt(dx_bf16, c.w2_t, act=_mul_aux_act(rec["h"], FF), aux=rec["h"], out_bf16=dhc)
                wg(dhc, rec.get("xn2"), [L.fc1_w], [L.fc1_b])
                ops.gemm_nt(dhc, c.w1_t, out_bf16=dtc)
                dx1_f32, dx1_bf16 = newB(H, F32), newB(H, BF16)
                ops.layernorm_bwd(dtc, rec["x1"], rec["st2"], c.g2, dres=dx_f32, dx_f32=dx1_f32, dx_bf16=dx1_bf16, **pg(L.ln2_w, L.ln2_b))
                wg(dx1_bf16, rec.get("o"), [L.proj_w], [L.proj_b])
                ops.gemm_nt(dx1_bf16, c.wo_t, out_bf16=dtc)
                ops.attention_bwd(rec["qkv"], dtc, B, S, self.heads, key_mask, dqkv, nq=1)
                if has_lora:
                    dt2 = self._lora_grads(L, c, dqkv, rec["xn"], rec["t"], dt, grads, rec.get("t2"))
                wg(dqkv, rec["xn"], L.qkv_w, L.qkv_b)
                if i > first_lora:
                    add32 = None if dt2 is None else self._slot2_bwd_addend(c, dt2)
                    ops.gemm_nt(dqkv, c.wqkv_t, rank_u=dt if has_lora else None, rank_v=c.v_bwd if has_lora else None, residual=add32, out_bf16=dtmp)
                    if r16:
                        dres16, _ = ops.scatter_rows(dx1_f32, S, bf16=True, f32=False)
                        ndx_bf16 = new(H, BF16)
                        ndx_f32 = new(H, F32) if (full and i == 0) else None
                        dx8 = new8(H) if (dg8 and "mlp" in self.dgrad8_sites) else None
                        ops.layernorm_bwd(dtmp, rec["x_in"], rec["st1"], c.g1, dres_bf16=dres16, dx_bf16=ndx_bf16, dx_f32=ndx_f32, **pg(L.ln1_w, L.ln1_b),
                                          **(f8kw(dx8) if dx8 is not None else {}))
                        dx_f32, dx_bf16 = ndx_f32, ndx_bf16
                    else:
                        _, dres_full = ops.scatter_rows(dx1_f32, S, bf16=False, f32=True)
                        ndx_f32, ndx_bf16 = new(H, F32), new(H, BF16)
                        ops.layernorm_bwd(dtmp, rec["x_in"], rec["st1"], c.g1, dres=dres_full, dx_f32=ndx_f32, dx_bf16=ndx_bf16, **pg(L.ln1_w, L.ln1_b))
                        dx_f32, dx_bf16 = ndx_f32, ndx_bf16
            elif self.pre_ln:
                wg(dx_bf16, rec.get("a"), [L.fc2_w], [L.fc2_b], rec.get("a_s"))
                if dg8 and dx8 is not None:
                    dh8 = torch.empty((M, FF), dtype=torch.uint8, device=dev).view(ops.FP8)
                    if full:
                        dh = new(FF, BF16) if dh is None else dh
                    ops.gemm_fp8_dgrad_nt(dx8[0], c.w2_t8, c.cs_2t, aux=rec["h"], act=_mul_aux_act(rec["h"], FF), out_fp8=dh8, out_fp8_scale=c.c2,
                                          a_row_dequant=dx8[1] if full else None, out_bf16_dual=dh if full else None)
                    wg(dh, rec.get("xn2"), [L.fc1_w], [L.fc1_b], rec.get("xn2_s"))
                    ops.gemm_fp8_dgrad_nt(dh8, c.w1_t8, c.cs_1t, a_row_dequant=dx8[1], out_bf16=dtmp)
                else:
                    dh = new(FF, BF16) if dh is None else dh
                    ops.gemm_nt(dx_bf16, c.w2_t, act=_mul_aux_act(rec["h"], FF), aux=rec["h"], out_bf16=dh)
                    wg(dh, rec.get("xn2"), [L.fc1_w], [L.fc1_b], rec.get("xn2_s"))
                    ops.gemm_nt(dh, c.w1_t, out_bf16=dtmp)
                dx18 = new8(H) if (dg8 and "proj" in self.dgrad8_sites) else None
                if r16:
                    dx1_f32, dx1_bf16 = None, new(H, BF16)
                    ops.layernorm_bwd(dtmp, rec["x1"], rec["st2"], c.g2, dres_bf16=dx_bf16, dx_bf16=dx1_bf16, **pg(L.ln2_w, L.ln2_b),
                                      **(f8kw(dx18) if dx18 is not None else {}))
                else:
                    dx1_f32, dx1_bf16 = new(H, F32), new(H, BF16)
                    ops.layernorm_bwd(dtmp, rec["x1"], rec["st2"], c.g2, dres=dx_f32, dx_f32=dx1_f32, dx_bf16=dx1_bf16, **pg(L.ln2_w, L.ln2_b))
                wg(dx1_bf16, rec.get("o"), [L.proj_w], [L.proj_b])
                if dx18 is not None:
                    ops.gemm_fp8_dgrad_nt(dx18[0], c.wo_t8, c.cs_ot, a_row_dequant=dx18[1], out_bf16=dtmp)
                else:
                    ops.gemm_nt(dx1_bf16, c.wo_t, out_bf16=dtmp)
                self._attention_bwd(rec, dtmp, B, S, key_mask, dqkv)
                if has_lora:
                    dt2 = self._lora_grads(L, c, dqkv, rec["xn"], rec["t"], dt, grads, rec.get("t2"))
                wg(dqkv, rec["xn"], L.qkv_w, L.qkv_b)
                if i > first_lora:
                    add32 = None if dt2 is None else self._slot2_bwd_addend(c, dt2)
                    ops.gemm_nt(dqkv, c.wqkv_t, rank_u=dt if has_lora else None, rank_v=c.v_bwd if has_lora else None, residual=add32, out_bf16=dtmp)
                    if r16:
                        ndx_f32, ndx_bf16 = (new(H, F32) if (full and i == 0) else None), new(H, BF16)
                        dx8 = new8(H) if (dg8 and "mlp" in self.dgrad8_sites) else None
                        ops.layernorm_bwd(dtmp, rec["x_in"], rec["st1"], c.g1, dres_bf16=dx1_bf16, dx_bf16=ndx_bf16, dx_f32=ndx_f32, **pg(L.ln1_w, L.ln1_b),
                                          **(f8kw(dx8) if dx8 is not None else {}))
                    else:
                        ndx_f32, ndx_bf16 = new(H, F32), new(H, BF16)
                        ops.layernorm_bwd(dtmp, rec["x_in"], rec["st1"], c.g1, dres=dx1_f32, dx_f32=ndx_f32, dx_bf16=ndx_bf16, **pg(L.ln1_w, L.ln1_b))
                    dx_f32, dx_bf16 = ndx_f32, ndx_bf16
            elif r16:
                def ln_back(dy, xs, st, gam, drop_site, pgk):
                    res = new(H, BF16)
                    if dg8 and full:
                        q8 = new8(H)
                        dropped = drop_site is not None and drop_site.thr16 > 0
                        masked = new(H, BF16) if dropped else None
                        ops.layernorm_bwd(dy, xs, st, gam, dx_res_bf16=res, dx_bf16=masked, drop=drop_site, **pgk, **f8kw(q8))
                        return res, (masked if dropped else res), q8
                    if dg8:
                        q8 = new8(H)
                        ops.layernorm_bwd(dy, xs, st, gam, dx_res_bf16=res, drop=drop_site, **f8kw(q8))
                        return res, None, q8
                    if drop_site is not None and drop_site.thr16 > 0:
                        masked = new(H, BF16)
                        ops.layernorm_bwd(dy, xs, st, gam, dx_res_bf16=res, dx_bf16=masked, drop=drop_site, **pgk)
                        return res, masked, None
                    ops.layernorm_bwd(dy, xs, st, gam, dx_res_bf16=res, **pgk)
                    return res, res, None

                ds2_res, ds2_b, ds2_8 = ln_back(dx_f32, rec["s2"], rec["st2"], c.g2, rec["d_h2"], pg(L.ln2_w, L.ln2_b))
                dx1 = new(H, BF16)
                if dg8:
                    dh8 = torch.empty((M, FF), dtype=torch.uint8, device=dev).view(ops.FP8)
                    if full:
                        wg(ds2_b, rec.get("a"), [L.fc2_w], [L.fc2_b], rec.get("a_s"))
                        dh = new(FF, BF16) if dh is None else dh
                    ops.gemm_fp8_dgrad_nt(ds2_8[0], c.w2_t8, c.cs_2t, aux=rec["h"], act=_mul_aux_act(rec["h"], FF), out_fp8=dh8, out_fp8_scale=c.c2,
                                          a_row_dequant=ds2_8[1] if full else None, out_bf16_dual=dh if full else None)
                    wg(dh, rec.get("x1_bf16"), [L.fc1_w], [L.fc1_b], rec.get("x1_s"))
                    ops.gemm_fp8_dgrad_nt(dh8, c.w1_t8, c.cs_1t, a_row_dequant=ds2_8[1], aux=ds2_res, act=ops.ACT_ADD_AUX, out_bf16=dx1)
# ... 204 lines not shown
```

clibd_amd/ops.py:

```python
from __future__ import annotations

import ctypes as C
import math
import os
from typing import Optional

import torch

from . import _lib
from ._lib import GemmEpilogue, check

ACT_NONE, ACT_GELU, ACT_GELU_GRAD, ACT_GELU_SAVE_GRAD, ACT_MUL_AUX, ACT_ADD_AUX, ACT_GELU_SAVE_GRAD_U8, ACT_MUL_AUX_U8 = 0, 1, 2, 3, 4, 5, 6, 7
ACT_GELU_SAVE_GRAD_E12, ACT_MUL_AUX_E12 = 8, 9
BF16, F32, I64, I32 = torch.bfloat16, torch.float32, torch.int64, torch.int32
FP8 = torch.float8_e4m3fn


def _stream() -> int:
    return torch._C._cuda_getCurrentRawStream(torch._C._cuda_getDevice())


def _p(t: Optional[torch.Tensor]) -> Optional[int]:
    return None if t is None else t.data_ptr()


def _chk(t: torch.Tensor, dtype, name: str, contiguous: bool = True) -> None:
    if not t.is_cuda:
        raise ValueError(f"{name}: expected a device tensor (clibd_amd has no CPU compute path)")
    if t.dtype != dtype:
        raise TypeError(f"{name}: expected {dtype}, got {t.dtype}")
    if contiguous and not t.is_contiguous():
        raise ValueError(f"{name}: expected a contiguous tensor")


def _rowmajor(t: torch.Tensor, name: str) -> int:
    if t.dim() != 2 or t.stride(1) != 1:
        raise ValueError(f"{name}: expected a 2-D tensor with unit inner stride")
    return t.stride(0)


class Drop:
    __slots__ = ("seed", "thr16", "scale")

    def __init__(self, p: float, seed: int):
        self.thr16 = int(round(p * 65536.0))
        if not 0 <= self.thr16 < 65536:
            raise ValueError("dropout p must be in [0, 1)")
        self.seed = seed & 0xFFFFFFFF
        self.scale = 1.0 / (1.0 - self.thr16 / 65536.0)


def _drop_args(drop: Optional[Drop]) -> tuple:
    return (drop.seed, drop.thr16, drop.scale) if (drop is not None and drop.thr16 > 0) else (0, 0, 1.0)


def derive_seed(base: int, layer: int, site: int) -> int:
    x = (base ^ ((layer * 8 + site + 1) * 0x9E3779B1)) & 0xFFFFFFFF
    x ^= x >> 16
    x = (x * 0x7FEB352D) & 0xFFFFFFFF
    x ^= x >> 15
    x = (x * 0x846CA68B) & 0xFFFFFFFF
    x ^= x >> 16
    return x


_STREAMK = os.environ.get("CLIBD_GEMM_STREAMK", "0") == "1"
_TAIL_WS_BYTES = 48 * 1024 * 1024 + 1024
_tail_ws: dict = {}

_ordered_ws: dict = {}


def _ordered_workspace(kind: str, nbytes: int, device) -> torch.Tensor:
    key = (kind, device, torch.cuda.current_stream(device).cuda_stream)
    ws = _ordered_ws.get(key)
    if ws is None or ws.numel() < nbytes:
        ws = torch.empty((max(int(nbytes), 16),), dtype=torch.uint8, device=device)
        _ordered_ws[key] = ws
    return ws


def _not_ordered(what: str):
    from .engine import NotSupportedYet

    return NotSupportedYet(f"deterministic mode: {what} has no fixed-order form")


def gemm_nt(
    a: torch.Tensor,
    w: torch.Tensor,
    *,
    bias: Optional[torch.Tensor] = None,
    rank_u: Optional[torch.Tensor] = None,
    rank_v: Optional[torch.Tensor] = None,
    act: int = ACT_NONE,
    aux: Optional[torch.Tensor] = None,
    residual: Optional[torch.Tensor] = None,
    out_pre: Optional[torch.Tensor] = None,
    out_bf16: Optional[torch.Tensor] = None,
    out_f32: Optional[torch.Tensor] = None,
    split_k: int = 1,
    drop: Optional["Drop"] = None,
    k_hole: Optional[tuple] = None,
    row_sums: Optional[torch.Tensor] = None,
    row_stats: Optional[torch.Tensor] = None,
    col_sum_w: Optional[torch.Tensor] = None,
) -> None:
    _chk(a, BF16, "a", contiguous=False)
    _chk(w, BF16, "w", contiguous=False)
    lda, ldw = _rowmajor(a, "a"), _rowmajor(w, "w")
    M, K = a.shape
    N, K2 = w.shape
    if K != K2:
        raise ValueError(f"gemm_nt: K mismatch {K} vs {K2}")
    ep = GemmEpilogue()
    ep.act = act
    ep.split_k = split_k
    if drop is not None and drop.thr16 > 0:
        ep.drop_seed, ep.drop_thr16, ep.drop_scale, ep.drop_ld = drop.seed, drop.thr16, drop.scale, N
    if bias is not None:
        _chk(bias, F32, "bias")
        if bias.numel() != N:
            raise ValueError("gemm_nt: bias must have N elements")
        ep.bias = bias.data_ptr()
    if rank_u is not None or rank_v is not None:
        _chk(rank_u, BF16, "rank_u", contiguous=False)
        _chk(rank_v, BF16, "rank_v")
        if rank_u.shape[0] != M or rank_u.shape[1] < 8 or tuple(rank_v.shape) != (N, 8):
            raise ValueError("gemm_nt: rank_u must be [M,>=8], rank_v [N,8]")
        ep.rank_u, ep.rank_v, ep.ld_rank_u = rank_u.data_ptr(), rank_v.data_ptr(), _rowmajor(rank_u, "rank_u")
    if aux is not None:
        _chk(aux, torch.uint8 if act in (ACT_MUL_AUX_U8, ACT_MUL_AUX_E12) else BF16, "aux", contiguous=False)
        if tuple(aux.shape) != (M, 3 * N // 2 if act == ACT_MUL_AUX_E12 else N):
            raise ValueError("gemm_nt: aux must be [M,N] ([M,3N/2] bytes for the e4m7 form)")
        ep.aux_bf16, ep.ld_aux = aux.data_ptr(), _rowmajor(aux, "aux")
    if residual is not None:
        _chk(residual, F32, "residual", contiguous=False)
        if tuple(residual.shape) != (M, N):
            raise ValueError("gemm_nt: residual must be [M,N]")
        ep.residual_f32, ep.ld_res = residual.data_ptr(), _rowmajor(residual, "residual")
    for name, t, dt in (("out_pre", out_pre, torch.uint8 if act in (ACT_GELU_SAVE_GRAD_U8, ACT_GELU_SAVE_GRAD_E12) else BF16), ("out_bf16", out_bf16, BF16), ("out_f32", out_f32, F32)):
        if t is not None:
            _chk(t, dt, name, contiguous=False)
            if tuple(t.shape) != (M, 3 * N // 2 if (name == "out_pre" and act == ACT_GELU_SAVE_GRAD_E12) else N):
                raise ValueError(f"gemm_nt: {name} must be [M,N] ([M,3N/2] bytes for the e4m7 form)")
    if out_pre is not None:
        ep.out_pre_bf16, ep.ld_pre = out_pre.data_ptr(), _rowmajor(out_pre, "out_pre")
    if out_bf16 is not None:
        ep.out_bf16, ep.ld_out_bf16 = out_bf16.data_ptr(), _rowmajor(out_bf16, "out_bf16")
    if out_f32 is not None:
        ep.out_f32, ep.ld_out_f32 = out_f32.data_ptr(), _rowmajor(out_f32, "out_f32")
    if row_sums is not None:
        _chk(row_sums, F32, "row_sums")
        if N % 128 or tuple(row_sums.shape) != (N // 128, M, 2):
            raise ValueError("gemm_nt: row_sums must be [N/128, M, 2]")
        ep.row_sums = row_sums.data_ptr()
    if row_stats is not None or col_sum_w is not None:
        _chk(row_stats, F32, "row_stats")
        _chk(col_sum_w, F32, "col_sum_w")
        if tuple(row_stats.shape) != (M, 2) or col_sum_w.numel() != N:
            raise ValueError("gemm_nt: row_stats must be [M,2], col_sum_w [N]")
        ep.row_stats, ep.col_sum_w = row_stats.data_ptr(), col_sum_w.data_ptr()
    if k_hole is not None:
        check(_lib.load().clibd_gemm_bf16_nt_khole(a.data_ptr(), lda, w.data_ptr(), ldw, M, N, K, int(k_hole[0]), int(k_hole[1]), C.byref(ep),
                                                   _stream()), "gemm_bf16_nt_khole")
        return
    lib = _lib.load()
    if _STREAMK and split_k == 1 and M >= 1024:
        need = int(lib.clibd_gemm_tail_workspace_bytes(M, N, K))
        if need > 0:
            key = (a.device, torch.cuda.current_stream(a.device).cuda_stream)
            ws = _tail_ws.get(key)
            if ws is None or ws.numel() < need:
                ws = torch.zeros((max(need, _TAIL_WS_BYTES),), dtype=torch.uint8, device=a.device)
                _tail_ws[key] = ws
            check(lib.clibd_gemm_bf16_nt_ws(a.data_ptr(), lda, w.data_ptr(), ldw, M, N, K, C.byref(ep), ws.data_ptr(), ws.numel(), _stream()), "gemm_bf16_nt_ws")
            return
    check(lib.clibd_gemm_bf16_nt(a.data_ptr(), lda, w.data_ptr(), ldw, M, N, K, C.byref(ep), _stream()), "gemm_bf16_nt")


def rowsum_finalize(row_sums: torch.Tensor, eps: float, stats: torch.Tensor) -> None:
    _chk(row_sums, F32, "row_sums")
    _chk(stats, F32, "stats")
    S, M, _ = row_sums.shape
    if tuple(stats.shape) != (M, 2):
        raise ValueError("rowsum_finalize: stats must be [M,2]")
    check(_lib.load().clibd_rowsum_finalize(row_sums.data_ptr(), S, M, 128 * S, float(eps), stats.data_ptr(), _stream()), "rowsum_finalize")


def ln_fold_weights(w: torch.Tensor, gamma: torch.Tensor, beta: torch.Tensor, bias: Optional[torch.Tensor]):
    _chk(w, F32, "w")
    _chk(gamma, F32, "gamma")
    _chk(beta, F32, "beta")
    N, K = w.shape
    wg = torch.empty((N, K), dtype=BF16, device=w.device)
    s = torch.empty((N,), dtype=F32, device=w.device)
    bp = torch.empty((N,), dtype=F32, device=w.device)
    check(_lib.load().clibd_ln_fold_weights(w.data_ptr(), gamma.data_ptr(), beta.data_ptr(), bias.data_ptr() if bias is not None else None, N, K,
                                            wg.data_ptr(), s.data_ptr(), bp.data_ptr(), _stream()), "ln_fold_weights")
    return wg, s, bp


def quantize_rows_fp8(w: torch.Tensor, act_scale: float):
    _chk(w, F32, "w")
    N, K = w.shape
    w8 = torch.empty((N, K), dtype=torch.uint8, device=w.device).view(FP8)
    cs = torch.empty((N,), dtype=F32, device=w.device)
    check(_lib.load().clibd_quantize_rows_fp8(w.data_ptr(), N, K, float(act_scale), w8.data_ptr(), cs.data_ptr(), _stream()), "quantize_rows_fp8")
    return w8, cs


def quantize_rows_fp8_bf16(w: torch.Tensor, act_scale: float = 1.0, l1max: Optional[torch.Tensor] = None):
    _chk(w, BF16, "w")
    N, K = w.shape
    w8 = torch.empty((N, K), dtype=torch.uint8, device=w.device).view(FP8)
    cs = torch.empty((N,), dtype=F32, device=w.device)
    if l1max is not None:
        _chk(l1max, F32, "l1max")
    check(_lib.load().clibd_quantize_rows_fp8_bf16(w.data_ptr(), N, K, float(act_scale), w8.data_ptr(), cs.data_ptr(), _p(l1max), _stream()),
          "quantize_rows_fp8_bf16")
    return w8, cs


def gemm_fp8_dgrad_nt(a: torch.Tensor, w: torch.Tensor, col_scale: torch.Tensor, *, a_row_dequant: Optional[torch.Tensor] = None,
                      aux: Optional[torch.Tensor] = None, act: int = ACT_NONE, out_bf16: Optional[torch.Tensor] = None,
                      out_fp8: Optional[torch.Tensor] = None, out_fp8_scale: float = 0.0, out_bf16_dual: Optional[torch.Tensor] = None) -> None:
    _chk(a, FP8, "a", contiguous=False)
    _chk(w, FP8, "w", contiguous=False)
    _chk(col_scale, F32, "col_scale")
    lda, ldw = _rowmajor(a, "a"), _rowmajor(w, "w")
    M, K = a.shape
    N, K2 = w.shape
    if K != K2 or col_scale.numel() != N:
        raise ValueError("gemm_fp8_dgrad_nt: shape mismatch")
    if act not in (ACT_NONE, ACT_ADD_AUX, ACT_MUL_AUX, ACT_MUL_AUX_U8, ACT_MUL_AUX_E12):
        raise ValueError("gemm_fp8_dgrad_nt: act must be NONE, ADD_AUX, MUL_AUX, MUL_AUX_U8 or MUL_AUX_E12")
    if (act == ACT_NONE) != (aux is None):
        raise ValueError("gemm_fp8_dgrad_nt: aux comes with ADD_AUX / MUL_AUX only")
    ep = GemmEpilogue()
    ep.split_k = 1
    ep.act = act
    if aux is not None:
        _chk(aux, torch.uint8 if act in (ACT_MUL_AUX_U8, ACT_MUL_AUX_E12) else BF16, "aux", contiguous=False)
        if tuple(aux.shape) != (M, 3 * N // 2 if act == ACT_MUL_AUX_E12 else N):
            raise ValueError("gemm_fp8_dgrad_nt: aux must be [M,N] ([M,3N/2] bytes for the e4m7 form)")
        ep.aux_bf16, ep.ld_aux = aux.data_ptr(), _rowmajor(aux, "aux")
    if act in (ACT_MUL_AUX, ACT_MUL_AUX_U8, ACT_MUL_AUX_E12):
        if out_fp8 is None or out_bf16 is not None or not out_fp8_scale > 0:
            raise ValueError("gemm_fp8_dgrad_nt: the MUL_AUX form writes out_fp8 with a positive out_fp8_scale")
        _chk(out_fp8, FP8, "out_fp8", contiguous=False)
        if tuple(out_fp8.shape) != (M, N):
            raise ValueError("gemm_fp8_dgrad_nt: out_fp8 must be [M,N]")
        ep.out_bf16, ep.ld_out_bf16 = out_fp8.data_ptr(), _rowmajor(out_fp8, "out_fp8")
        if out_bf16_dual is not None:
            if a_row_dequant is None:
                raise ValueError("gemm_fp8_dgrad_nt: out_bf16_dual needs a_row_dequant")
            _chk(out_bf16_dual, BF16, "out_bf16_dual", contiguous=False)
            if tuple(out_bf16_dual.shape) != (M, N):
                raise ValueError("gemm_fp8_dgrad_nt: out_bf16_dual must be [M,N]")
            ep.out_pre_bf16, ep.ld_pre = out_bf16_dual.data_ptr(), _rowmajor(out_bf16_dual, "out_bf16_dual")
    else:
        if out_bf16_dual is not None:
            raise ValueError("gemm_fp8_dgrad_nt: out_bf16_dual comes with the MUL_AUX forms only")
        if out_bf16 is None or out_fp8 is not None or a_row_dequant is None:
            raise ValueError("gemm_fp8_dgrad_nt: the bf16-output forms need out_bf16 and a_row_dequant")
        _chk(out_bf16, BF16, "out_bf16", contiguous=False)
        if tuple(out_bf16.shape) != (M, N):
            raise ValueError("gemm_fp8_dgrad_nt: out_bf16 must be [M,N]")
        ep.out_bf16, ep.ld_out_bf16 = out_bf16.data_ptr(), _rowmajor(out_bf16, "out_bf16")
        out_fp8_scale = 0.0
    if a_row_dequant is not None:
        _chk(a_row_dequant, F32, "a_row_dequant")
        if a_row_dequant.numel() != M:
            raise ValueError("gemm_fp8_dgrad_nt: a_row_dequant must have M elements")
    check(_lib.load().clibd_gemm_fp8_dgrad_nt(a.data_ptr(), lda, w.data_ptr(), ldw, M, N, K, col_scale.data_ptr(), _p(a_row_dequant),
                                              float(out_fp8_scale), C.byref(ep), _stream()), "gemm_fp8_dgrad_nt")


def gemm_fp8_nt(
    a: torch.Tensor,
    w: torch.Tensor,
    col_scale: torch.Tensor,
    *,
    bias: torch.Tensor,
    rank_u: Optional[torch.Tensor] = None,
    rank_v: Optional[torch.Tensor] = None,
    gelu_out_fp8: Optional[torch.Tensor] = None,
    gelu_out_scale: float = 0.0,
    out_pre: Optional[torch.Tensor] = None,
    residual: Optional[torch.Tensor] = None,
    out_bf16: Optional[torch.Tensor] = None,
    out_f32: Optional[torch.Tensor] = None,
    drop: Optional["Drop"] = None,
) -> None:
    _chk(a, FP8, "a", contiguous=False)
    _chk(w, FP8, "w", contiguous=False)
    _chk(col_scale, F32, "col_scale")
    _chk(bias, F32, "bias")
    lda, ldw = _rowmajor(a, "a"), _rowmajor(w, "w")
    M, K = a.shape
    N, K2 = w.shape
    if K != K2 or col_scale.numel() != N or bias.numel() != N:
        raise ValueError("gemm_fp8_nt: shape mismatch")
    ep = GemmEpilogue()
    ep.split_k = 1
    ep.bias = bias.data_ptr()
    if drop is not None and drop.thr16 > 0:
        ep.drop_seed, ep.drop_thr16, ep.drop_scale, ep.drop_ld = drop.seed, drop.thr16, drop.scale, N
    if rank_u is not None or rank_v is not None:
        _chk(rank_u, BF16, "rank_u", contiguous=False)
        _chk(rank_v, BF16, "rank_v")
        if rank_u.shape[0] != M or rank_u.shape[1] < 8 or tuple(rank_v.shape) != (N, 8):
            raise ValueError("gemm_fp8_nt: rank_u must be [M,>=8], rank_v [N,8]")
        ep.rank_u, ep.rank_v, ep.ld_rank_u = rank_u.data_ptr(), rank_v.data_ptr(), _rowmajor(rank_u, "rank_u")
    for name, t, dt in (("out_pre", out_pre, BF16), ("out_bf16", out_bf16, BF16), ("out_f32", out_f32, F32), ("residual", residual, F32),
# ... 763 lines not shown
```

Baseline: 7191.

## Recompute post-LN residual inside GEMM epilogue instead of materialising fp32 copy

For post-LN blocks, the fp32 normalised residual (x1_f32, x2_f32) is no longer written by the LayerNorm kernels. The following residual GEMM reads the pre-norm sum, the row mean/rstd and the packed gamma|beta, and applies the LayerNorm affine in its epilogue. This removes an M×H fp32 write and its later read per layer. In exchange the epilogue does more arithmetic and reads a few extra per-row and per-column operands. A new epilogue kind, validation paths and a contract-off ln_affine helper are added so both paths round identically.

```diff
diff --git a/clibd_amd/csrc/common.h b/clibd_amd/csrc/common.h
--- a/clibd_amd/csrc/common.h
+++ b/clibd_amd/csrc/common.h
@@ -66,6 +66,12 @@
 __device__ __forceinline__ float drop_one(unsigned seed, unsigned idx, unsigned thr16, float scale) {
     const unsigned h = drop_hash(seed, idx >> 1);
     return (((idx & 1u) ? (h >> 16) : (h & 0xffffu)) >= thr16) ? scale : 0.f;
+}
+
+__device__ __forceinline__ float ln_affine(float v, float mean, float rstd, float g, float b) {
+#pragma clang fp contract(off)
+    const float xhat = (v - mean) * rstd;
+    return __builtin_fmaf(g, xhat, b);
 }
 
 template <int CTRL>
diff --git a/clibd_amd/csrc/gemm.hip b/clibd_amd/csrc/gemm.hip
--- a/clibd_amd/csrc/gemm.hip
+++ b/clibd_amd/csrc/gemm.hip
@@ -131,7 +131,7 @@
         for (int j = 0; j < 4; ++j)
 #pragma unroll
             for (int r = 0; r < 4; ++r) v[4 * j + r] = acc[i][j][r] + bias[4 * j + r];
-        store_row16(ep, m, nb, v);
+        store_row16(ep, m, nb, p.N, v);
     }
 }
 
@@ -369,7 +369,16 @@
         }
     }
     static const int forced = [] { const char* e = getenv("CLIBD_GEMM_KERNEL"); return e ? atoi(e) : 0; }();
-    const bool fold_epi = ep->row_sums != nullptr || ep->row_stats != nullptr;
+    const bool res_ln = ep->row_sums == nullptr && ep->residual_f32 != nullptr && (ep->row_stats != nullptr || ep->col_sum_w != nullptr);
+    if (res_ln) {
+        if (!ep->row_stats) return set_error(CLIBD_EINVAL, "gemm: normalised residual: col_sum_w (gamma | beta) comes with row_stats (mean, rstd)");
+        if (!ep->col_sum_w) return set_error(CLIBD_EINVAL, "gemm: normalised residual: row_stats (mean, rstd) comes with col_sum_w (gamma | beta, fp32 [2, N])");
+        if (!aligned16(ep->row_stats)) return set_error(CLIBD_EINVAL, "gemm: normalised residual: row_stats must be 16-byte aligned");
+        if (!aligned16(ep->col_sum_w)) return set_error(CLIBD_EINVAL, "gemm: normalised residual: col_sum_w must be 16-byte aligned");
+        if (epilogue_kind(p.ep) < 0)
+            return set_error(CLIBD_EINVAL, "gemm: normalised residual: act NONE with out_f32 only (no out_bf16, no out_pre_bf16, no split-K)");
+    }
+    const bool fold_epi = !res_ln && (ep->row_sums != nullptr || ep->row_stats != nullptr);
     if (fold_epi) {
         if (epilogue_kind(p.ep) < 0)
             return set_error(CLIBD_EINVAL, "gemm: LN-fold epilogue: row_sums needs bias + residual_f32 + out_f32 + out_bf16 (act NONE); row_stats needs "
diff --git a/clibd_amd/csrc/gemm256.hip b/clibd_amd/csrc/gemm256.hip
--- a/clibd_amd/csrc/gemm256.hip
+++ b/clibd_amd/csrc/gemm256.hip
@@ -374,20 +374,31 @@
         asm volatile("" : "+v"(erow), "+v"(egrp));
         int nb = n0 + 128 * wm + 8 * erow;
         int mb = m0 + 64 * wn + 4 * egrp;
-        constexpr bool RES_KIND = (KIND == EPI_RES_F32 || KIND == EPI_RES_F32_DROP || KIND == EPI_RES_F32_COPY);
+        constexpr bool RES_LN = epi_res_ln_kind(KIND);
+        constexpr bool RES_KIND = (KIND == EPI_RES_F32 || KIND == EPI_RES_F32_DROP || KIND == EPI_RES_F32_COPY || RES_LN);
         constexpr bool TWO_PASS = (epi_aux_kind(KIND) || RES_KIND || KIND == EPI_ROWNORM_GELU);
-        constexpr bool PRELOAD_ROWS = TWO_PASS && !LORA && !FP8;
+        constexpr bool PRELOAD_ROWS = TWO_PASS && !LORA && !FP8 && !RES_LN;
         f32x4 bias_q[2];
         uint4 in_aux[8];
         f32x4 in_res[8][2];
         float2 in_st[8];
         f32x4 col_s[2];
+        f32x4 gb_q[4];
+        static_assert(!RES_LN || (BIAS && !FP8 && !LORA), "the on-the-fly LayerNorm residual is instantiated with a bias, bf16 operands and no rank update");
 #define GLOAD128(dst, ptr) asm volatile("global_load_dwordx4 %0, %1, off ; EPI_OPERAND_LOAD" : "=&v"(dst) : "v"(ptr) : "memory")
         constexpr bool BIAS_ASM = BIAS && !FP8;
         if constexpr (BIAS_ASM) {
             const float* bp = ep.bias + nb;
             GLOAD128(bias_q[0], bp);
             GLOAD128(bias_q[1], bp + 4);
+        }
+        if constexpr (RES_LN) {
+            const float* gp = ep.col_sum_w + nb;
+            const float* bp = gp + p.N;
+            GLOAD128(gb_q[0], gp);
+            GLOAD128(gb_q[1], gp + 4);
+            GLOAD128(gb_q[2], bp);
+            GLOAD128(gb_q[3], bp + 4);
         }
         if constexpr (PRELOAD_ROWS) {
 #pragma unroll
@@ -425,11 +436,17 @@
         mb = m0 + 64 * wn + 4 * egrp;
 #define EPI_TIED_WAIT(N)                                                                                             \
     do {                                                                                                             \
-        if constexpr (BIAS_ASM) asm volatile("s_waitcnt vmcnt(" #N ") ; EPI_OPERAND_WAIT" : "+v"(bias_q[0]), "+v"(bias_q[1])); \
+        if constexpr (RES_LN)                                                                                        \
+            asm volatile("s_waitcnt vmcnt(" #N ") ; EPI_OPERAND_WAIT"                                                \
+                         : "+v"(bias_q[0]), "+v"(bias_q[1]), "+v"(gb_q[0]), "+v"(gb_q[1]), "+v"(gb_q[2]), "+v"(gb_q[3]));                \
+        else if constexpr (BIAS_ASM) asm volatile("s_waitcnt vmcnt(" #N ") ; EPI_OPERAND_WAIT" : "+v"(bias_q[0]), "+v"(bias_q[1])); \
     } while (0)
         if constexpr (KIND == EPI_ROWNORM_GELU) {
             if (!has_next) asm volatile("s_waitcnt vmcnt(10)" ::: "memory");
             EPI_TIED_WAIT(14);
+        } else if constexpr (RES_LN) {
+            if (!has_next) asm volatile("s_waitcnt vmcnt(0)" ::: "memory");
+            EPI_TIED_WAIT(4);
         } else if constexpr (PRELOAD_ROWS && epi_aux_kind(KIND)) {
             if (!has_next) asm volatile("s_waitcnt vmcnt(8)" ::: "memory");
             EPI_TIED_WAIT(12);
@@ -544,33 +561,70 @@
                 if constexpr (KIND == EPI_ROWNORM_GELU) {
                     _Pragma("unroll") for (int e = 0; e < 4; ++e) { cs8[e] = col_s[0][e]; cs8[4 + e] = col_s[1][e]; }
                 }
-                FOR_ROWS_HN(0, 1, {
-                    const int mc = min(m, p.M - 1);
-                    float v[8];
-                    _Pragma("unroll") for (int hm = 0; hm < 2; ++hm)
-                        _Pragma("unroll") for (int t = 0; t < 4; ++t) v[4 * hm + t] = (KIND == EPI_ROWNORM_GELU) ? acc[hm][t][hn][n][r] : EPV(hm, t);
-                    if constexpr (KIND == EPI_ROWNORM_GELU) fold_rownorm8(v, in_st[4 * n + r].x, in_st[4 * n + r].y, cs8, bias);
-                    else if constexpr (PRELOAD_ROWS) fold_row8_in<KIND>(ep, mc, nb, v, in_aux[4 * n + r], in_res[4 * n + r][0], in_res[4 * n + r][1]);
-                    else fold_row8<KIND>(ep, mc, nb, v);
-                    _Pragma("unroll") for (int hm = 0; hm < 2; ++hm)
-                        _Pragma("unroll") for (int t = 0; t < 4; ++t) acc[hm][t][hn][n][r] = v[4 * hm + t];
-                })
-                PIN_GROUP(0);
-                FOR_ROWS_HN(1, 2, {
-                    const int mc = min(m, p.M - 1);
-                    float v[8];
-                    _Pragma("unroll") for (int hm = 0; hm < 2; ++hm)
-                        _Pragma("unroll") for (int t = 0; t < 4; ++t) v[4 * hm + t] = (KIND == EPI_ROWNORM_GELU) ? acc[hm][t][hn][n][r] : EPV(hm, t);
-                    if constexpr (KIND == EPI_ROWNORM_GELU) {
-                        const float2 st = *(const float2*)(ep.row_stats + (size_t)mc * 2);
-                        fold_rownorm8(v, st.x, st.y, cs8, bias);
-                    } else {
-                        fold_row8<KIND>(ep, mc, nb, v);
-                    }
-                    _Pragma("unroll") for (int hm = 0; hm < 2; ++hm)
-                        _Pragma("unroll") for (int t = 0; t < 4; ++t) acc[hm][t][hn][n][r] = v[4 * hm + t];
-                })
-                PIN_GROUP(1);
+                float g8[8], b8[8];
+                if constexpr (RES_LN) {
+                    _Pragma("unroll") for (int e = 0; e < 4; ++e) { g8[e] = gb_q[0][e]; g8[4 + e] = gb_q[1][e]; b8[e] = gb_q[2][e]; b8[4 + e] = gb_q[3][e]; }
+                }
+                if constexpr (RES_LN) {
+                    FOR_ROWS({
+                        _Pragma("unroll") for (int hm = 0; hm < 2; ++hm)
+                            _Pragma("unroll") for (int t = 0; t < 4; ++t) acc[hm][t][hn][n][r] = EPV(hm, t);
+                    })
+                    PIN_GROUP(0);
+                    PIN_GROUP(1);
+                    _Pragma("unroll") for (int hn = 0; hn < 2; ++hn)
+                        _Pragma("unroll") for (int n = 0; n < 2; ++n) {
+                            f32x4 rs4[4][2];
+                            float2 st4[4];
+                            _Pragma("unroll") for (int r = 0; r < 4; ++r) {
+                                const int mc = min(mb + 32 * hn + 16 * n + r, p.M - 1);
+                                const f32x4* rs = (const f32x4*)(ep.residual_f32 + (size_t)mc * ep.ld_res + nb);
+                                rs4[r][0] = rs[0];
+                                rs4[r][1] = rs[1];
+                                st4[r] = *(const float2*)(ep.row_stats + (size_t)mc * 2);
+                            }
+                            __builtin_amdgcn_sched_barrier(0);
+                            _Pragma("unroll") for (int r = 0; r < 4; ++r) {
+                                float v[8];
+                                _Pragma("unroll") for (int hm = 0; hm < 2; ++hm)
+                                    _Pragma("unroll") for (int t = 0; t < 4; ++t) v[4 * hm + t] = acc[hm][t][hn][n][r];
+                                fold_row8_ln_in<KIND>(ep, min(mb + 32 * hn + 16 * n + r, p.M - 1), nb, v, rs4[r][0], rs4[r][1], st4[r], g8, b8);
+                                _Pragma("unroll") for (int hm = 0; hm < 2; ++hm)
+                                    _Pragma("unroll") for (int t = 0; t < 4; ++t) acc[hm][t][hn][n][r] = v[4 * hm + t];
+                            }
+                            _Pragma("unroll") for (int hm = 0; hm < 2; ++hm)
+                                _Pragma("unroll") for (int t = 0; t < 4; ++t) asm volatile("" : "+v"(acc[hm][t][hn][n]));
+                            __builtin_amdgcn_sched_barrier(0);
+                        }
+                } else {
+                    FOR_ROWS_HN(0, 1, {
+                        const int mc = min(m, p.M - 1);
+                        float v[8];
+                        _Pragma("unroll") for (int hm = 0; hm < 2; ++hm)
+                            _Pragma("unroll") for (int t = 0; t < 4; ++t) v[4 * hm + t] = (KIND == EPI_ROWNORM_GELU) ? acc[hm][t][hn][n][r] : EPV(hm, t);
+                        if constexpr (KIND == EPI_ROWNORM_GELU) fold_rownorm8(v, in_st[4 * n + r].x, in_st[4 * n + r].y, cs8, bias);
+                        else if constexpr (PRELOAD_ROWS) fold_row8_in<KIND>(ep, mc, nb, v, in_aux[4 * n + r], in_res[4 * n + r][0], in_res[4 * n + r][1]);
+                        else fold_row8<KIND>(ep, mc, nb, v);
+                        _Pragma("unroll") for (int hm = 0; hm < 2; ++hm)
+                            _Pragma("unroll") for (int t = 0; t < 4; ++t) acc[hm][t][hn][n][r] = v[4 * hm + t];
+                    })
+                    PIN_GROUP(0);
+                    FOR_ROWS_HN(1, 2, {
+                        const int mc = min(m, p.M - 1);
+                        float v[8];
+                        _Pragma("unroll") for (int hm = 0; hm < 2; ++hm)
+                            _Pragma("unroll") for (int t = 0; t < 4; ++t) v[4 * hm + t] = (KIND == EPI_ROWNORM_GELU) ? acc[hm][t][hn][n][r] : EPV(hm, t);
+                        if constexpr (KIND == EPI_ROWNORM_GELU) {
+                            const float2 st = *(const float2*)(ep.row_stats + (size_t)mc * 2);
+                            fold_rownorm8(v, st.x, st.y, cs8, bias);
+                        } else {
+                            fold_row8<KIND>(ep, mc, nb, v);
+                        }
+                        _Pragma("unroll") for (int hm = 0; hm < 2; ++hm)
+                            _Pragma("unroll") for (int t = 0; t < 4; ++t) acc[hm][t][hn][n][r] = v[4 * hm + t];
+                    })
+                    PIN_GROUP(1);
+                }
                 float keep1 = 0.f, keep2 = 0.f;
                 FOR_ROWS({
                     if (m < p.M) {
@@ -697,6 +751,8 @@
         case EPI_SPLITK_F32: return (const void*)gemm256_bf16_nt_kernel<EPI_SPLITK_F32, false, false, false, false>;
         case EPI_RES_F32_COPY: return (lora || !bias || diag) ? nullptr : (const void*)gemm256_bf16_nt_kernel<EPI_RES_F32_COPY, false, true, false, false>;
         case EPI_ROWNORM_GELU: return (lora || !bias || diag) ? nullptr : (const void*)gemm256_bf16_nt_kernel<EPI_ROWNORM_GELU, false, true, false, false>;
+        case EPI_RES_LN_F32: return (lora || !bias || diag) ? nullptr : (const void*)gemm256_bf16_nt_kernel<EPI_RES_LN_F32, false, true, false, false>;
+        case EPI_RES_LN_F32_DROP: return (lora || !bias || diag) ? nullptr : (const void*)gemm256_bf16_nt_kernel<EPI_RES_LN_F32_DROP, false, true, false, false>;
         default: return K256(EPI_GENERIC);
     }
 #undef K256
diff --git a/clibd_amd/csrc/gemm_common.h b/clibd_amd/csrc/gemm_common.h
--- a/clibd_amd/csrc/gemm_common.h
+++ b/clibd_amd/csrc/gemm_common.h
@@ -83,7 +83,7 @@
     }
 }
 
-__device__ __forceinline__ void store_row16(const clibd_gemm_epilogue& ep, int m, int nb, float v[16]) {
+__device__ __forceinline__ void store_row16(const clibd_gemm_epilogue& ep, int m, int nb, int N, float v[16]) {
     if (ep.split_k > 1) {
         float* o = ep.out_f32 + (size_t)m * ep.ld_out_f32 + nb;
 #pragma unroll
@@ -174,10 +174,22 @@
     }
     if (ep.residual_f32 != nullptr) {
         const f32x4* rs = (const f32x4*)(ep.residual_f32 + (size_t)m * ep.ld_res + nb);
-#pragma unroll
-        for (int q = 0; q < 4; ++q) {
-            const f32x4 r4 = rs[q];
-            v[4 * q + 0] += r4[0]; v[4 * q + 1] += r4[1]; v[4 * q + 2] += r4[2]; v[4 * q + 3] += r4[3];
+        if (ep.row_stats != nullptr) {
+            const float2 st = *(const float2*)(ep.row_stats + (size_t)m * 2);
+            const f32x4* gs = (const f32x4*)(ep.col_sum_w + nb);
+            const f32x4* bs = (const f32x4*)(ep.col_sum_w + N + nb);
+#pragma unroll
+            for (int q = 0; q < 4; ++q) {
+                const f32x4 r4 = rs[q], g4 = gs[q], b4 = bs[q];
+#pragma unroll
+                for (int e = 0; e < 4; ++e) v[4 * q + e] += ln_affine(r4[e], st.x, st.y, g4[e], b4[e]);
+            }
+        } else {
+#pragma unroll
+            for (int q = 0; q < 4; ++q) {
+                const f32x4 r4 = rs[q];
+                v[4 * q + 0] += r4[0]; v[4 * q + 1] += r4[1]; v[4 * q + 2] += r4[2]; v[4 * q + 3] += r4[3];
+            }
         }
     }
     if (ep.out_f32 != nullptr) {
@@ -227,8 +239,11 @@
     EPI_MUL_AUX_12 = 13,
     EPI_GELU = 14,
     EPI_F32 = 15,
-    EPI_NUM_KINDS = 16,
+    EPI_RES_LN_F32 = 16,
+    EPI_RES_LN_F32_DROP = 17,
+    EPI_NUM_KINDS = 18,
 };
+constexpr bool epi_res_ln_kind(int kind) { return kind == EPI_RES_LN_F32 || kind == EPI_RES_LN_F32_DROP; }
 constexpr bool epi_aux_kind(int kind) { return kind == EPI_MUL_AUX || kind == EPI_ADD_AUX || kind == EPI_MUL_AUX_U8 || kind == EPI_MUL_AUX_12; }
 constexpr bool epi_mul_aux_kind(int kind) { return kind == EPI_MUL_AUX || kind == EPI_MUL_AUX_U8 || kind == EPI_MUL_AUX_12; }
 
@@ -237,6 +252,8 @@
     const bool drop = ep.drop_thr16 > 0;
     if (ep.row_sums != nullptr)
         return (ep.act == CLIBD_ACT_NONE && !drop && !ep.out_pre_bf16 && ep.residual_f32 && ep.out_f32 && ep.out_bf16 && !ep.rank_u && ep.bias) ? EPI_RES_F32_COPY : -1;
+    if (ep.row_stats != nullptr && ep.residual_f32 != nullptr)
+        return (ep.act == CLIBD_ACT_NONE && !ep.out_pre_bf16 && ep.out_f32 && !ep.out_bf16 && ep.col_sum_w) ? (drop ? EPI_RES_LN_F32_DROP : EPI_RES_LN_F32) : -1;
     if (ep.row_stats != nullptr)
         return (ep.act == CLIBD_ACT_GELU_SAVE_GRAD && !drop && ep.out_pre_bf16 && !ep.residual_f32 && !ep.out_f32 && ep.out_bf16 && !ep.rank_u && ep.bias && ep.col_sum_w) ? EPI_ROWNORM_GELU : -1;
     if (ep.act == CLIBD_ACT_NONE && !drop && !ep.out_pre_bf16 && !ep.residual_f32 && !ep.out_f32 && ep.out_bf16) return EPI_BF16;
@@ -438,6 +455,30 @@
     }
 }
 
+template <int KIND>
+__device__ __forceinline__ void fold_row8_ln_in(const clibd_gemm_epilogue& ep, int m, int nb, float v[8], const f32x4& r0, const f32x4& r1, const float2& st,
+                                                const float g[8], const float b[8]) {
+    float y[8];
+#pragma unroll
+    for (int e = 0; e < 4; ++e) {
+        y[e] = ln_affine(r0[e], st.x, st.y, g[e], b[e]);
+        y[4 + e] = ln_affine(r1[e], st.x, st.y, g[4 + e], b[4 + e]);
+    }
+    if (KIND == EPI_RES_LN_F32_DROP) {
+        const unsigned base = (unsigned)m * (unsigned)ep.drop_ld + (unsigned)nb;
+#pragma unroll
+        for (int e = 0; e < 8; e += 2) {
+            float f0, f1;
+            drop_pair(ep.drop_seed, base + e, (unsigned)ep.drop_thr16, ep.drop_scale, f0, f1);
+            v[e] = __builtin_fmaf(v[e], f0, y[e]);
+            v[e + 1] = __builtin_fmaf(v[e + 1], f1, y[e + 1]);
+        }
+    } else {
+#pragma unroll
+        for (int e = 0; e < 8; ++e) v[e] += y[e];
+    }
+}
+
 __device__ __forceinline__ void fold_rownorm8(float v[8], float mean, float rstd, const float s[8], const float b[8]) {
 #pragma unroll
     for (int e = 0; e < 8; ++e) v[e] = fmaf(rstd, fmaf(-mean, s[e], v[e]), b[e]);
diff --git a/clibd_amd/csrc/layernorm.hip b/clibd_amd/csrc/layernorm.hip
--- a/clibd_amd/csrc/layernorm.hip
+++ b/clibd_amd/csrc/layernorm.hip
@@ -105,7 +105,7 @@
                 const int row = row0 + rr;
                 f32x4 y;
 #pragma unroll
-                for (int e = 0; e < 4; ++e) y[e] = (v[rr][j][e] - mean[rr]) * rstd[rr] * g[j][e] + b[j][e];
+                for (int e = 0; e < 4; ++e) y[e] = ln_affine(v[rr][j][e], mean[rr], rstd[rr], g[j][e], b[j][e]);
                 if (drop_thr16 > 0) {
                     const unsigned base = (unsigned)row * (unsigned)H + (unsigned)c;
                     float f0, f1, f2, f3;
diff --git a/clibd_amd/engine.py b/clibd_amd/engine.py
--- a/clibd_amd/engine.py
+++ b/clibd_amd/engine.py
@@ -89,6 +89,7 @@
     __slots__ = ("wqkv", "wqkv_t", "bqkv", "wo", "wo_t", "bo", "w1", "w1_t", "b1", "w2", "w2_t", "b2", "g1", "be1", "g2", "be2",
                  "v_fwd", "v_bwd", "a_cat", "w_dt", "slot2", "wqkv8", "cs_qkv", "wo8", "cs_o", "w18", "cs_1", "w28", "cs_2",
                  "w1g", "s1", "b1f",
+                 "gb1", "gb2",
                  "wo_t8", "cs_ot", "w1_t8", "cs_1t", "w2_t8", "cs_2t", "c2")
 
 
@@ -127,6 +128,7 @@
         self.numerics = default_numerics()
         self.deterministic = default_deterministic()
         self._c2, self._c2_age = None, 0
+        self._ln_residual_materialised = False
         self.dgrad8_sites = ("mlp", "proj")
 
     DGRAD8_C2_EVERY = 64
@@ -219,6 +221,7 @@
                 c.w1, c.w1_t, c.b1 = ops.cast_bf16(_f32c(L.fc1_w)), ops.cast_transpose_bf16(_f32c(L.fc1_w)), _f32c(L.fc1_b)
                 c.w2, c.w2_t, c.b2 = ops.cast_bf16(_f32c(L.fc2_w)), ops.cast_transpose_bf16(_f32c(L.fc2_w)), _f32c(L.fc2_b)
                 c.g1, c.be1, c.g2, c.be2 = _f32c(L.ln1_w), _f32c(L.ln1_b), _f32c(L.ln2_w), _f32c(L.ln2_b)
+                c.gb1, c.gb2 = (None, None) if self.pre_ln else (torch.stack([c.g1.view(-1), c.be1.view(-1)]), torch.stack([c.g2.view(-1), c.be2.view(-1)]))
                 if self.fp8 is not None:
                     f8 = self.fp8[len(self._cache)]
                     if "qkv_in" in f8:
@@ -333,6 +336,8 @@
         fold_sums = torch.empty((H // 128, M, 2), dtype=F32, device=dev) if fold else None
         if fold and h_tmp is None and not save:
             h_tmp = new(FF, BF16)
+        ln_fused = not self.pre_ln and f8s is None and not self._ln_residual_materialised
+        res_ln = None
         for i, (L, c) in enumerate(zip(self.layers, self._cache)):
             has_lora = L.lora is not None
             rec = {}
@@ -443,11 +448,12 @@
                     d_h2 = ops.Drop(p_h, ops.derive_seed(base, i, 2))
                 qkv = new(3 * H, BF16)
                 s1 = new(H, F32)
-                x1_f32 = new(H, F32)
+                x1_f32 = None if ln_fused else new(H, F32)
                 st1 = torch.empty((M, 2), dtype=F32, device=dev)
                 h = new(HC, GG) if save else None
                 s2 = new(H, F32)
-                x2_f32, x2_bf16 = new(H, F32), new(H, BF16)
+                last = i == len(self.layers) - 1
+                x2_f32, x2_bf16 = (None if (ln_fused and not last) else new(H, F32)), new(H, BF16)
                 st2 = torch.empty((M, 2), dtype=F32, device=dev)
                 nxt = self.lora_a(i + 1)
                 t_next = torch.empty((M, 8), dtype=BF16, device=dev) if nxt is not None else None
@@ -487,11 +493,18 @@
                         ops.attention_fwd(qkv, B, S, self.heads, None, o, drop=d_att, lse=att_sv["lse"], o_lo=att_sv["o_lo"])
                     else:
                         ops.attention_fwd(qkv, B, S, self.heads, key_mask, o, drop=d_att)
-                    ops.gemm_nt(o, c.wo, bias=c.bo, residual=x_f32, out_f32=s1, drop=d_h1)
+                    if res_ln is not None:
+                        ops.gemm_nt(o, c.wo, bias=c.bo, residual=res_ln[0], residual_ln=res_ln[1:], out_f32=s1, drop=d_h1)
+                    else:
+                        ops.gemm_nt(o, c.wo, bias=c.bo, residual=x_f32, out_f32=s1, drop=d_h1)
                     ops.layernorm_fwd(s1, c.g1, c.be1, self.eps, y_bf16=x1_bf16, y_f32=x1_f32, stats=st1)
                     ops.gemm_nt(x1_bf16, c.w1, bias=c.b1, act=act_save if save else ops.ACT_GELU, out_pre=h if save else None, out_bf16=a)
-                    ops.gemm_nt(a, c.w2, bias=c.b2, residual=x1_f32, out_f32=s2, drop=d_h2)
+                    if ln_fused:
+                        ops.gemm_nt(a, c.w2, bias=c.b2, residual=s1, residual_ln=(st1, c.gb1), out_f32=s2, drop=d_h2)
+                    else:
+                        ops.gemm_nt(a, c.w2, bias=c.b2, residual=x1_f32, out_f32=s2, drop=d_h2)
                     ops.layernorm_fwd(s2, c.g2, c.be2, self.eps, y_bf16=x2_bf16, y_f32=x2_f32, stats=st2, lora_a=nxt, t_out=t_next)
+                    res_ln = (s2, st2, c.gb2) if x2_f32 is None else None
                     if crec is not None:
                         crec.update(qkv_in=amax(x_bf16), proj_in=amax(o), fc1_in=amax(x1_bf16), fc2_in=amax(a))
                 if save:
diff --git a/clibd_amd/ops.py b/clibd_amd/ops.py
--- a/clibd_amd/ops.py
+++ b/clibd_amd/ops.py
@@ -105,6 +105,7 @@
     row_sums: Optional[torch.Tensor] = None,
     row_stats: Optional[torch.Tensor] = None,
     col_sum_w: Optional[torch.Tensor] = None,
+    residual_ln: Optional[tuple] = None,
 ) -> None:
     _chk(a, BF16, "a", contiguous=False)
     _chk(w, BF16, "w", contiguous=False)
@@ -161,6 +162,17 @@
         if tuple(row_stats.shape) != (M, 2) or col_sum_w.numel() != N:
             raise ValueError("gemm_nt: row_stats must be [M,2], col_sum_w [N]")
         ep.row_stats, ep.col_sum_w = row_stats.data_ptr(), col_sum_w.data_ptr()
+    if residual_ln is not None:
+        if residual is None or row_stats is not None or col_sum_w is not None or row_sums is not None:
+            raise ValueError("gemm_nt: residual_ln needs residual and excludes row_sums / row_stats / col_sum_w")
+        if act != ACT_NONE or out_f32 is None or out_bf16 is not None or out_pre is not None or split_k != 1:
+            raise ValueError("gemm_nt: residual_ln: act NONE with out_f32 only")
+        stats, gamma_beta = residual_ln
+        _chk(stats, F32, "residual_ln stats")
+        _chk(gamma_beta, F32, "residual_ln gamma_beta")
+        if tuple(stats.shape) != (M, 2) or tuple(gamma_beta.shape) != (2, N):
+            raise ValueError("gemm_nt: residual_ln = (stats [M,2], gamma_beta [2,N])")
+        ep.row_stats, ep.col_sum_w = stats.data_ptr(), gamma_beta.data_ptr()
     if k_hole is not None:
         check(_lib.load().clibd_gemm_bf16_nt_khole(a.data_ptr(), lda, w.data_ptr(), ldw, M, N, K, int(k_hole[0]), int(k_hole[1]), C.byref(ep),
                                                    _stream()), "gemm_bf16_nt_khole")
```

Result: no change. 7256 (median of 6 runs) (+0.9%).
